# kondratevakate/mri-epilepsy-diagnosis

Measured on AMD Instinct MI355X. Metric: MRI volumes/sec (fwd+bwd) 3D U-Net @160x192x160, higher is better.
Workload: dtype f32; 1 GPU; unet.UNet(c0=8, 3 enc blocks, BN+PReLU, trilinear) fwd+softmax-Dice+bwd+AdamW, batch 2 x 1x160x192x160 fp32 per GPU (BASELINE configs[1]); global_batch=2, parallelism=dp1, launch=eager

## Files before the change

### include/mri3d.h

```cpp
#ifndef MRI3D_H
#define MRI3D_H

#include <stddef.h>
#include <stdint.h>

#ifdef __cplusplus
extern "C" {
#endif

typedef void* mri3d_stream_t;

enum { MRI3D_OK = 0, MRI3D_EINVAL = -1, MRI3D_ENOTSUP = -2, MRI3D_ELAUNCH = -3, MRI3D_EWORKSPACE = -4 };
enum { MRI3D_F32 = 0, MRI3D_BF16 = 1 };
enum { MRI3D_ACT_NONE = 0, MRI3D_ACT_RELU = 1, MRI3D_ACT_LEAKY = 2, MRI3D_ACT_PRELU = 3 };
enum { MRI3D_UP_NEAREST = 0, MRI3D_UP_TRILINEAR = 1 };
enum { MRI3D_PASS_FWD = 0, MRI3D_PASS_DGRAD = 1, MRI3D_PASS_WGRAD = 2 };

int mri3d_version(void);
const char* mri3d_last_error(void);

typedef struct Mri3dConvGeom {
    int32_t n;
    int32_t di, hi, wi, ci;
    int32_t dout, ho, wo, co;
    int32_t kd, kh, kw;
    int32_t sd, sh, sw;
    int32_t pd, ph, pw;
    int32_t dd, dh, dw;
    int32_t x_ld, y_ld;
    int32_t dtype;
} Mri3dConvGeom;

size_t mri3d_conv3d_workspace_bytes(const Mri3dConvGeom* g, int pass);

int mri3d_conv3d_fwd(const Mri3dConvGeom* g, const void* x, const void* w, const void* bias, void* y,
                     void* workspace, size_t ws_bytes, mri3d_stream_t stream);
int32_t mri3d_conv3d_fwd_stats_blocks(const Mri3dConvGeom* g);
int mri3d_conv3d_fwd_stats(const Mri3dConvGeom* g, const void* x, const void* w, const void* bias, void* y,
                           double* stat_partials, void* workspace, size_t ws_bytes, mri3d_stream_t stream);
int mri3d_conv3d_dgrad(const Mri3dConvGeom* g, const void* dy, const void* w, const void* bias, void* dx,
                       void* workspace, size_t ws_bytes, mri3d_stream_t stream);
int mri3d_conv3d_wgrad(const Mri3dConvGeom* g, const void* x, const void* dy, void* dw, void* dbias,
                       void* workspace, size_t ws_bytes, mri3d_stream_t stream);

int mri3d_conv3d_route(const Mri3dConvGeom* g, int32_t pass, int32_t stats, int32_t bias, int32_t split, int32_t second_ld,
                       int32_t align_x, int32_t align_y, char* name, size_t name_bytes);

int32_t mri3d_conv3d_cat_supported(const Mri3dConvGeom* g, int32_t split, int32_t second_ld, int32_t pass);
int32_t mri3d_conv3d_fwd_cat_stats_blocks(const Mri3dConvGeom* g, int32_t split, int32_t second_ld);
int mri3d_conv3d_fwd_cat(const Mri3dConvGeom* g, const void* x, const void* x2, int32_t split, int32_t x2_ld, const void* w,
                         const void* bias, void* y, double* stat_partials, void* workspace, size_t ws_bytes,
                         mri3d_stream_t stream);
int mri3d_conv3d_dgrad_cat(const Mri3dConvGeom* g, const void* dy, const void* w, void* dx, void* dx2, int32_t split,
                           int32_t dx2_ld, void* workspace, size_t ws_bytes, mri3d_stream_t stream);
int mri3d_conv3d_wgrad_cat(const Mri3dConvGeom* g, const void* x, const void* x2, int32_t split, int32_t x2_ld, const void* dy,
                           void* dw, void* dbias, void* workspace, size_t ws_bytes, mri3d_stream_t stream);

int32_t mri3d_conv3d_march_supported(const Mri3dConvGeom* g, int32_t pass);
int32_t mri3d_conv3d_march_stats_blocks(const Mri3dConvGeom* g);
int mri3d_conv3d_fwd_march(const Mri3dConvGeom* g, const void* x, const void* x2, int32_t split, int32_t x2_ld, const void* w,
                           const void* bias, void* y, double* stat_partials, void* workspace, size_t ws_bytes,
                           mri3d_stream_t stream);
int mri3d_conv3d_dgrad_march(const Mri3dConvGeom* g, const void* dy, const void* w, void* dx, void* dx2, int32_t split,
                             int32_t dx2_ld, void* workspace, size_t ws_bytes, mri3d_stream_t stream);

typedef struct Mri3dMarchPlanInfo {
    int32_t chunks, blocks, wgh, wgw, gch, gcw, nseg, seglen, nbuf, grid, whole_chunks, dispatcher;
    int64_t smem_bytes, wp_bytes;
} Mri3dMarchPlanInfo;
int32_t mri3d_conv3d_march_plan_query(const Mri3dConvGeom* g, int32_t pass, int32_t stats, Mri3dMarchPlanInfo* out);

int32_t mri3d_upconv3d_supported(const Mri3dConvGeom* g, int32_t scale);
size_t mri3d_upconv3d_workspace_bytes(const Mri3dConvGeom* g, int32_t scale);
int mri3d_upconv3d_fwd(const Mri3dConvGeom* g, int32_t scale, const void* x, const float* w, const float* bias, void* y,
                       mri3d_stream_t stream);
int mri3d_upconv3d_dgrad(const Mri3dConvGeom* g, int32_t scale, const void* dy, const float* w, void* dx, mri3d_stream_t stream);
int mri3d_upconv3d_wgrad(const Mri3dConvGeom* g, int32_t scale, const void* x, const void* dy, float* dw, float* dbias,
                         void* workspace, size_t ws_bytes, mri3d_stream_t stream);

int32_t mri3d_convpair_supported(const Mri3dConvGeom* first, const Mri3dConvGeom* second);
size_t mri3d_convpair_workspace_bytes(const Mri3dConvGeom* first, const Mri3dConvGeom* second);
int mri3d_convpair_wgrad_first(const Mri3dConvGeom* first, const Mri3dConvGeom* second, const void* x, const void* dy2, const float* w2,
                               float* dw1, float* dbias1, void* workspace, size_t ws_bytes, mri3d_stream_t stream);

typedef struct Mri3dFusedConvPlanInfo {
    int32_t hch, grid, gtrips, trips, per, passes, chunks;
    int64_t slabs, rows;
} Mri3dFusedConvPlanInfo;
int32_t mri3d_upconv3d_plan_query(const Mri3dConvGeom* g, int32_t scale, int32_t pass, Mri3dFusedConvPlanInfo* out);
int32_t mri3d_convpair_plan_query(const Mri3dConvGeom* first, const Mri3dConvGeom* second, Mri3dFusedConvPlanInfo* out);

typedef struct Mri3dNormGeom {
    int32_t n;
    int64_t vox;
    int32_t c;
    int32_t x_ld;
    int32_t y_ld;
    int32_t instance;
    int32_t act;
    int32_t alpha_n;
    float slope;
    float eps;
    int32_t group_c;
    int32_t dtype;
} Mri3dNormGeom;

size_t mri3d_norm_workspace_bytes(const Mri3dNormGeom* g);

enum { MRI3D_NORM_PASS_STATS = 0, MRI3D_NORM_PASS_FWD = 1, MRI3D_NORM_PASS_BWD = 2 };
typedef struct Mri3dNormPlanInfo {
    int32_t vec, CL, VT, cy, nblk, groups;
    int64_t gvox;
} Mri3dNormPlanInfo;
int32_t mri3d_norm_plan_query(const Mri3dNormGeom* g, int32_t pass, int32_t align, Mri3dNormPlanInfo* out);

int mri3d_norm_stats(const Mri3dNormGeom* g, const void* x, float* mean, float* invstd,
                     float* running_mean, float* running_var, float momentum,
                     void* workspace, size_t ws_bytes, mri3d_stream_t stream);
int mri3d_norm_stats_from_partials(const Mri3dNormGeom* g, const double* partials, int32_t nblk, const float* shift,
                                   float* mean, float* invstd, float* running_mean, float* running_var, float momentum,
                                   mri3d_stream_t stream);
int mri3d_norm_act_fwd(const Mri3dNormGeom* g, const void* x, const float* mean, const float* invstd,
                       const float* gamma, const float* beta, const float* alpha, void* y,
                       mri3d_stream_t stream);
int mri3d_norm_act_bwd(const Mri3dNormGeom* g, int training, const void* x, const void* dy,
                       const float* mean, const float* invstd, const float* gamma, const float* beta,
                       const float* alpha, void* dx, float* dgamma, float* dbeta, float* dalpha,
                       void* workspace, size_t ws_bytes, mri3d_stream_t stream);

int32_t mri3d_norm_act_pw_supported(const Mri3dNormGeom* g, int32_t co);
size_t mri3d_norm_act_pw_workspace_bytes(const Mri3dNormGeom* g, int32_t co);
int mri3d_norm_act_pw_fwd(const Mri3dNormGeom* g, int32_t co, const void* x, const float* mean, const float* invstd,
                          const float* gamma, const float* beta, const float* alpha, const float* w, const float* bias,
                          void* out, mri3d_stream_t stream);
int mri3d_norm_act_pw_bwd(const Mri3dNormGeom* g, int32_t co, int training, const void* x, const void* dout,
                          const float* mean, const float* invstd, const float* gamma, const float* beta, const float* alpha,
                          const float* w, void* dx, float* dgamma, float* dbeta, float* dalpha, float* dw, float* dbias,
                          void* workspace, size_t ws_bytes, mri3d_stream_t stream);

typedef struct Mri3dPoolGeom {
    int32_t n, di, hi, wi, dout, ho, wo, c;
    int32_t kd, kh, kw, sd, sh, sw, pd, ph, pw;
    int32_t x_ld, y_ld;
    int32_t dtype;
} Mri3dPoolGeom;
int mri3d_maxpool3d_fwd(const Mri3dPoolGeom* g, const void* x, void* y, uint8_t* idx, mri3d_stream_t stream);
int mri3d_maxpool3d_bwd(const Mri3dPoolGeom* g, const void* dy, const uint8_t* idx, void* dx, mri3d_stream_t stream);
int mri3d_maxpool3d_bwd_add(const Mri3dPoolGeom* g, const void* dy, const uint8_t* idx, const void* addend,
                            int32_t addend_ld, void* dx, mri3d_stream_t stream);
int mri3d_maxpool3d_route(const Mri3dPoolGeom* g, int32_t pass, int32_t addend_ld, int32_t align_tensors, int32_t align_idx,
                          char* name, size_t name_bytes);

int32_t mri3d_norm_act_pool_supported(const Mri3dNormGeom* g, const Mri3dPoolGeom* pg);
size_t mri3d_norm_act_pool_workspace_bytes(const Mri3dNormGeom* g, const Mri3dPoolGeom* pg);
int mri3d_norm_act_pool_fwd(const Mri3dNormGeom* g, const Mri3dPoolGeom* pg, const void* x, const float* mean,
                            const float* invstd, const float* gamma, const float* beta, const float* alpha, void* skip,
                            void* pooled, uint8_t* idx, mri3d_stream_t stream);
int mri3d_norm_act_pool_bwd(const Mri3dNormGeom* g, const Mri3dPoolGeom* pg, int training, const void* x, const void* dskip,
                            const void* dpool, const uint8_t* idx, const float* mean, const float* invstd, const float* gamma,
                            const float* beta, const float* alpha, void* dx, float* dgamma, float* dbeta, float* dalpha,
                            void* workspace, size_t ws_bytes, mri3d_stream_t stream);

typedef struct Mri3dUpGeom {
    int32_t n, di, hi, wi, dout, ho, wo, c;
    int32_t x_ld, y_ld;
    int32_t mode;
    int32_t align_corners;
    float rd, rh, rw;
    int32_t dtype;
} Mri3dUpGeom;
size_t mri3d_upsample3d_workspace_bytes(const Mri3dUpGeom* g);
int mri3d_upsample3d_fwd(const Mri3dUpGeom* g, const void* x, void* y, mri3d_stream_t stream);
int mri3d_upsample3d_bwd(const Mri3dUpGeom* g, const void* dy, void* dx, void* workspace, size_t ws_bytes,
                         mri3d_stream_t stream);
int mri3d_upsample3d_route(const Mri3dUpGeom* g, int32_t pass, int32_t align, char* name, size_t name_bytes);

typedef struct Mri3dResamplePlanInfo {
    int32_t vec, npv, hch, grid, segs, segl, tiles_h, tiles_w, passes, items, tables;
    int64_t lds_bytes;
} Mri3dResamplePlanInfo;
int32_t mri3d_maxpool3d_plan_query(const Mri3dPoolGeom* g, int32_t pass, int32_t addend_ld, int32_t align_tensors,
                                   int32_t align_idx, Mri3dResamplePlanInfo* out);
int32_t mri3d_upsample3d_plan_query(const Mri3dUpGeom* g, int32_t pass, int32_t align, Mri3dResamplePlanInfo* out);

typedef struct Mri3dDiceGeom {
    int32_t n;
    int64_t vox;
    int32_t c, ct;
    int32_t x_ld, t_ld;
    float eps;
    int32_t dtype;
} Mri3dDiceGeom;
size_t mri3d_softmax_dice_workspace_bytes(const Mri3dDiceGeom* g);
int mri3d_softmax_dice_fwd(const Mri3dDiceGeom* g, const void* logits, const void* target, float* loss,
                           float* stats, void* workspace, size_t ws_bytes, mri3d_stream_t stream);
int mri3d_softmax_dice_bwd(const Mri3dDiceGeom* g, const void* logits, const void* target, const float* stats,
                           const float* dloss, void* dlogits, mri3d_stream_t stream);

int mri3d_argmax_u8(const void* logits, uint8_t* out, int64_t nvox, int32_t c, int32_t ld, int32_t dtype,
                    mri3d_stream_t stream);

size_t mri3d_mask_overlap_workspace_bytes(void);
int mri3d_mask_overlap(const uint8_t* pred, const uint8_t* gt, int64_t nvox, int64_t* counts, void* workspace,
                       size_t ws_bytes, mri3d_stream_t stream);

enum { MRI3D_LABEL_U8 = 0, MRI3D_LABEL_I16 = 1, MRI3D_LABEL_I32 = 2, MRI3D_LABEL_F32 = 3 };

int mri3d_label_remap(const void* in, int32_t in_dtype, void* out, int32_t out_dtype, int64_t n, const uint8_t* lut,
                      int32_t lut_len, int32_t above, int32_t other, mri3d_stream_t stream);

typedef struct Mri3dDiceIndexGeom {
    int32_t n;
    int64_t vox;
    int32_t c;
    int32_t x_ld;
    float eps;
    int32_t dtype;
} Mri3dDiceIndexGeom;
size_t mri3d_softmax_dice_index_workspace_bytes(const Mri3dDiceIndexGeom* g);
int mri3d_softmax_dice_index_fwd(const Mri3dDiceIndexGeom* g, const void* logits, const uint8_t* labels, float* loss,
                                 float* stats, void* workspace, size_t ws_bytes, mri3d_stream_t stream);
int mri3d_softmax_dice_index_bwd(const Mri3dDiceIndexGeom* g, const void* logits, const uint8_t* labels,
                                 const float* stats, const float* dloss, void* dlogits, mri3d_stream_t stream);

size_t mri3d_confusion_workspace_bytes(int32_t c);
int mri3d_confusion_counts(const uint8_t* pred, const uint8_t* gt, int64_t nvox, int32_t c, int64_t* counts,
                           void* workspace, size_t ws_bytes, mri3d_stream_t stream);

size_t mri3d_order_stats_workspace_bytes(void);
int mri3d_order_stats_f32(const float* x, int64_t n, const int64_t* ranks, int32_t nranks, float* out, void* workspace,
                          size_t ws_bytes, mri3d_stream_t stream);
int mri3d_piecewise_linear_f32(const float* x, float* y, int64_t n, const double* edges, const double* slope,
                               const double* intercept, int32_t nseg, mri3d_stream_t stream);
size_t mri3d_znorm_workspace_bytes(void);
int mri3d_znorm_mean_mask_f32(const float* x, float* y, int64_t n, double* stats, void* workspace, size_t ws_bytes,
                              mri3d_stream_t stream);
int mri3d_crop_or_pad_f32(const float* x, float* y, int32_t outer, int32_t di, int32_t hi, int32_t wi, int32_t dout,
                          int32_t ho, int32_t wo, float fill, mri3d_stream_t stream);

size_t mri3d_intensity_workspace_bytes(int64_t n, int32_t batch, int32_t m);
int mri3d_kde_plan(int64_t n, int32_t batch, int32_t m, int32_t out[4]);
int mri3d_intensity_moments_f32(const float* x, const uint8_t* mask, int64_t n, int32_t batch, double* moments,
                                void* workspace, size_t ws_bytes, mri3d_stream_t stream);
int mri3d_kde_f32(const float* x, const uint8_t* mask, int64_t n, int32_t batch, const double* moments, const double* positions,
                  int32_t m, int32_t bw_rule, double bw_scalar, double* positions_out, double* density, void* workspace,
                  size_t ws_bytes, mri3d_stream_t stream);

size_t mri3d_surface_distance_workspace_bytes(int32_t d, int32_t h, int32_t w);
int mri3d_surface_distance(const uint8_t* gt, const uint8_t* pred, int32_t d, int32_t h, int32_t w,
                           const double* area_table, double* sums, void* workspace, size_t ws_bytes, mri3d_stream_t stream);
int mri3d_surface_elements(const uint8_t* gt, const uint8_t* pred, int32_t d, int32_t h, int32_t w, int32_t* d2_gt,
                           uint8_t* code_gt, int32_t* d2_pred, uint8_t* code_pred, int64_t capacity, uint64_t* counts,
                           void* workspace, size_t ws_bytes, mri3d_stream_t stream);

int mri3d_extract_patches(const void* volumes, int32_t elem_bytes, int32_t nvol, int32_t d, int32_t h, int32_t w,
                          const int32_t* loc_host, int32_t npatch, int32_t pd, int32_t ph, int32_t pw, void* out,
                          mri3d_stream_t stream);
int mri3d_aggregate_patches_u8(const uint8_t* patches, const int32_t* loc_host, int32_t npatch, int32_t pd, int32_t ph,
                               int32_t pw, int32_t bd, int32_t bh, int32_t bw, uint8_t* out, int32_t nvol, int32_t d,
                               int32_t h, int32_t w, mri3d_stream_t stream);
int mri3d_aggregate_patches_argmax(const void* logits, int32_t c, int32_t ld, int32_t dtype, const int32_t* loc_host,
                                   int32_t npatch, int32_t pd, int32_t ph, int32_t pw, int32_t bd, int32_t bh, int32_t bw,
                                   uint8_t* out, int32_t nvol, int32_t d, int32_t h, int32_t w, mri3d_stream_t stream);

int mri3d_strip_starts_f32(const float* gm, int32_t nx, int32_t ny, int32_t nz, int32_t h, int32_t* starts, mri3d_stream_t stream);
int mri3d_mirror_patches_f32(const float* volume, int32_t nx, int32_t ny, int32_t nz, const int32_t* table, const int32_t* order,
                             int64_t npatch, int32_t h, int32_t w, int32_t channels_last, float* out, mri3d_stream_t stream);
int mri3d_mirror_patch_labels_u8(const uint8_t* mask, int32_t nx, int32_t ny, int32_t nz, const int32_t* table, int64_t npatch,
                                 int32_t h, int32_t w, uint8_t* out, mri3d_stream_t stream);
int mri3d_patch_vote_u8(const uint8_t* map, int32_t strips, int32_t slices, uint8_t* out, mri3d_stream_t stream);
int mri3d_paint_patches_u8(const uint8_t* map, const int32_t* starts, int32_t nx, int32_t ny, int32_t nz, int32_t h, int32_t w,
                           uint8_t* out, mri3d_stream_t stream);

int mri3d_warp3d(const float* image, float* image_out, const void* label, void* label_out, int32_t label_bytes, int32_t s,
                 int32_t d, int32_t h, int32_t w, const float* affine, const float* grid, int32_t gd, int32_t gh, int32_t gw,
                 float pad_value, const float* pad_values, mri3d_stream_t stream);
int mri3d_bias_field_f32(const float* x, float* y, int32_t s, int32_t d, int32_t h, int32_t w, const float* coef_host,
                         int32_t order, mri3d_stream_t stream);
int mri3d_kspace_mix_f32(const float* images,
                         float* out,
                         int32_t s, int32_t n, int32_t d, int32_t h, int32_t w,
                         const float* coef,
                         mri3d_stream_t stream);

int mri3d_copy_channels(const void* src, void* dst, int64_t nvox, int32_t c, int32_t src_ld, int32_t dst_ld,
                        int32_t dtype, mri3d_stream_t stream);
int mri3d_add_channels(const void* a, const void* b, void* dst, int64_t nvox, int32_t c, int32_t a_ld,
                       int32_t b_ld, int32_t dst_ld, int32_t dtype, mri3d_stream_t stream);
int mri3d_convert_channels(const void* src, int32_t src_dtype, void* dst, int32_t dst_dtype, int64_t nvox, int32_t c,
                           int32_t src_ld, int32_t dst_ld, mri3d_stream_t stream);

int mri3d_bayes_weights_fwd(const float* mu, const float* logsigma, int64_t n, int32_t eval, float threshold, float* w_mean,
                            float* w_var, float* log_alpha, mri3d_stream_t stream);
int mri3d_bayes_weights_bwd(const float* mu, const float* logsigma, int64_t n, int32_t eval, float threshold,
                            const float* d_w_mean, const float* d_w_var, const float* d_log_alpha, float* dmu,
                            float* dlogsigma, mri3d_stream_t stream);
int mri3d_bayes_square(const void* x, void* x2, int64_t nvox, int32_t c, int32_t x_ld, int32_t x2_ld, int32_t dtype,
                       mri3d_stream_t stream);
int mri3d_bayes_sample_fwd(const void* mu_out, const void* var_out, const float* eps, void* y, int64_t nvox, int32_t c,
                           int32_t mu_ld, int32_t var_ld, int32_t eps_ld, int32_t y_ld, int32_t dtype, mri3d_stream_t stream);
int mri3d_bayes_sample_bwd(const void* dy, const void* var_out, const float* eps, void* dvar, int64_t nvox, int32_t c,
                           int32_t dy_ld, int32_t var_ld, int32_t eps_ld, int32_t dvar_ld, int32_t dtype,
                           mri3d_stream_t stream);
int mri3d_bayes_dx(const void* dx_mean, const void* dx_var, const void* x, void* dx, int64_t nvox, int32_t c,
                   int32_t dx_mean_ld, int32_t dx_var_ld, int32_t x_ld, int32_t dx_ld, int32_t dtype, mri3d_stream_t stream);

size_t mri3d_mc_state_bytes(int64_t nvox, int32_t c);
int mri3d_mc_accumulate(const void* logits, int64_t nvox, int32_t c, int32_t ld, int32_t dtype, int32_t reps,
                        int64_t rep_stride, int32_t first, void* state, size_t state_bytes, mri3d_stream_t stream);
int mri3d_mc_finalize(const void* state, size_t state_bytes, int64_t nvox, int32_t c, int32_t samples, float* mean_p,
                      float* variance, float* entropy, float* mutual_info, uint8_t* mask, mri3d_stream_t stream);

int mri3d_adam_step(float* p, const float* g, float* m, float* v, int64_t n, float lr, float beta1, float beta2,
                    float eps, float weight_decay, int32_t step, float grad_scale, int32_t decoupled,
                    mri3d_stream_t stream);

#ifdef __cplusplus
}
#endif
#endif
```

### mri_epilepsy_diagnosis_amd/_lib.py

```python
import ctypes
import os
from ctypes import POINTER, Structure, c_char_p, c_double, c_float, c_int32, c_int64, c_size_t, c_uint8, c_void_p

_HERE = os.path.dirname(os.path.abspath(__file__))
LIB_PATH = os.path.join(_HERE, "libmri3d_hip.so")

F32, BF16 = 0, 1
ACT_NONE, ACT_RELU, ACT_LEAKY, ACT_PRELU = 0, 1, 2, 3
UP_NEAREST, UP_TRILINEAR = 0, 1
PASS_FWD, PASS_DGRAD, PASS_WGRAD = 0, 1, 2
NORM_PASS_STATS, NORM_PASS_FWD, NORM_PASS_BWD = 0, 1, 2
LABEL_U8, LABEL_I16, LABEL_I32, LABEL_F32 = 0, 1, 2, 3
BW_SCOTT, BW_SILVERMAN, BW_FACTOR = 0, 1, 2


class ConvGeom(Structure):
    _fields_ = [(n, c_int32) for n in (
        "n", "di", "hi", "wi", "ci", "dout", "ho", "wo", "co", "kd", "kh", "kw", "sd", "sh", "sw",
        "pd", "ph", "pw", "dd", "dh", "dw", "x_ld", "y_ld", "dtype")]


class NormGeom(Structure):
    _fields_ = [("n", c_int32), ("vox", c_int64), ("c", c_int32), ("x_ld", c_int32), ("y_ld", c_int32),
                ("instance", c_int32), ("act", c_int32), ("alpha_n", c_int32), ("slope", c_float),
                ("eps", c_float), ("group_c", c_int32), ("dtype", c_int32)]


class NormPlanInfo(Structure):
    _fields_ = [(n, c_int32) for n in ("vec", "CL", "VT", "cy", "nblk", "groups")] + [("gvox", c_int64)]


class ResamplePlanInfo(Structure):
    _fields_ = [(n, c_int32) for n in ("vec", "npv", "hch", "grid", "segs", "segl", "tiles_h", "tiles_w", "passes", "items",
                                       "tables")] + [("lds_bytes", c_int64)]


class FusedConvPlanInfo(Structure):
    _fields_ = [(n, c_int32) for n in ("hch", "grid", "gtrips", "trips", "per", "passes", "chunks")] + \
               [("slabs", c_int64), ("rows", c_int64)]


class MarchPlanInfo(Structure):
    _fields_ = [(n, c_int32) for n in ("chunks", "blocks", "wgh", "wgw", "gch", "gcw", "nseg", "seglen", "nbuf", "grid",
                                       "whole_chunks", "dispatcher")] + [("smem_bytes", c_int64), ("wp_bytes", c_int64)]


class PoolGeom(Structure):
    _fields_ = [(n, c_int32) for n in (
        "n", "di", "hi", "wi", "dout", "ho", "wo", "c", "kd", "kh", "kw", "sd", "sh", "sw", "pd", "ph", "pw",
        "x_ld", "y_ld", "dtype")]


class UpGeom(Structure):
    _fields_ = [(n, c_int32) for n in ("n", "di", "hi", "wi", "dout", "ho", "wo", "c", "x_ld", "y_ld", "mode",
                                       "align_corners")] + \
               [("rd", c_float), ("rh", c_float), ("rw", c_float), ("dtype", c_int32)]


class DiceGeom(Structure):
    _fields_ = [("n", c_int32), ("vox", c_int64), ("c", c_int32), ("ct", c_int32), ("x_ld", c_int32),
                ("t_ld", c_int32), ("eps", c_float), ("dtype", c_int32)]


class DiceIndexGeom(Structure):
    _fields_ = [("n", c_int32), ("vox", c_int64), ("c", c_int32), ("x_ld", c_int32), ("eps", c_float), ("dtype", c_int32)]


_P = c_void_p
_FP = c_void_p

SIGNATURES = {
    "mri3d_version": (c_int32, []),
    "mri3d_last_error": (c_char_p, []),
    "mri3d_conv3d_workspace_bytes": (c_size_t, [POINTER(ConvGeom), c_int32]),
    "mri3d_conv3d_fwd": (c_int32, [POINTER(ConvGeom), _P, _P, _P, _P, _P, c_size_t, _P]),
    "mri3d_conv3d_fwd_stats_blocks": (c_int32, [POINTER(ConvGeom)]),
    "mri3d_conv3d_fwd_stats": (c_int32, [POINTER(ConvGeom), _P, _P, _P, _P, _P, _P, c_size_t, _P]),
    "mri3d_conv3d_dgrad": (c_int32, [POINTER(ConvGeom), _P, _P, _P, _P, _P, c_size_t, _P]),
    "mri3d_conv3d_wgrad": (c_int32, [POINTER(ConvGeom), _P, _P, _P, _P, _P, c_size_t, _P]),
    "mri3d_conv3d_route": (c_int32, [POINTER(ConvGeom), c_int32, c_int32, c_int32, c_int32, c_int32, c_int32, c_int32, c_char_p, c_size_t]),
    "mri3d_conv3d_cat_supported": (c_int32, [POINTER(ConvGeom), c_int32, c_int32, c_int32]),
    "mri3d_conv3d_fwd_cat_stats_blocks": (c_int32, [POINTER(ConvGeom), c_int32, c_int32]),
    "mri3d_conv3d_fwd_cat": (c_int32, [POINTER(ConvGeom), _P, _P, c_int32, c_int32, _P, _P, _P, _P, _P, c_size_t, _P]),
    "mri3d_conv3d_dgrad_cat": (c_int32, [POINTER(ConvGeom), _P, _P, _P, _P, c_int32, c_int32, _P, c_size_t, _P]),
    "mri3d_conv3d_wgrad_cat": (c_int32, [POINTER(ConvGeom), _P, _P, c_int32, c_int32, _P, _P, _P, _P, c_size_t, _P]),
    "mri3d_conv3d_march_supported": (c_int32, [POINTER(ConvGeom), c_int32]),
    "mri3d_conv3d_march_stats_blocks": (c_int32, [POINTER(ConvGeom)]),
    "mri3d_conv3d_march_plan_query": (c_int32, [POINTER(ConvGeom), c_int32, c_int32, POINTER(MarchPlanInfo)]),
    "mri3d_conv3d_fwd_march": (c_int32, [POINTER(ConvGeom), _P, _P, c_int32, c_int32, _P, _P, _P, _P, _P, c_size_t, _P]),
    "mri3d_conv3d_dgrad_march": (c_int32, [POINTER(ConvGeom), _P, _P, _P, _P, c_int32, c_int32, _P, c_size_t, _P]),
    "mri3d_upconv3d_supported": (c_int32, [POINTER(ConvGeom), c_int32]),
    "mri3d_upconv3d_workspace_bytes": (c_size_t, [POINTER(ConvGeom), c_int32]),
    "mri3d_upconv3d_fwd": (c_int32, [POINTER(ConvGeom), c_int32, _P, _FP, _FP, _P, _P]),
    "mri3d_upconv3d_dgrad": (c_int32, [POINTER(ConvGeom), c_int32, _P, _FP, _P, _P]),
    "mri3d_upconv3d_wgrad": (c_int32, [POINTER(ConvGeom), c_int32, _P, _P, _FP, _FP, _P, c_size_t, _P]),
    "mri3d_convpair_supported": (c_int32, [POINTER(ConvGeom), POINTER(ConvGeom)]),
    "mri3d_convpair_workspace_bytes": (c_size_t, [POINTER(ConvGeom), POINTER(ConvGeom)]),
    "mri3d_convpair_wgrad_first": (c_int32, [POINTER(ConvGeom), POINTER(ConvGeom), _P, _P, _FP, _FP, _FP, _P, c_size_t, _P]),
    "mri3d_upconv3d_plan_query": (c_int32, [POINTER(ConvGeom), c_int32, c_int32, POINTER(FusedConvPlanInfo)]),
    "mri3d_convpair_plan_query": (c_int32, [POINTER(ConvGeom), POINTER(ConvGeom), POINTER(FusedConvPlanInfo)]),
    "mri3d_norm_workspace_bytes": (c_size_t, [POINTER(NormGeom)]),
    "mri3d_norm_plan_query": (c_int32, [POINTER(NormGeom), c_int32, c_int32, POINTER(NormPlanInfo)]),
    "mri3d_norm_stats": (c_int32, [POINTER(NormGeom), _P, _FP, _FP, _FP, _FP, c_float, _P, c_size_t, _P]),
    "mri3d_norm_stats_from_partials": (c_int32, [POINTER(NormGeom), _P, c_int32, _FP, _FP, _FP, _FP, _FP, c_float, _P]),
    "mri3d_norm_act_fwd": (c_int32, [POINTER(NormGeom), _P, _FP, _FP, _FP, _FP, _FP, _P, _P]),
    "mri3d_norm_act_bwd": (c_int32, [POINTER(NormGeom), c_int32, _P, _P, _FP, _FP, _FP, _FP, _FP, _P, _FP, _FP, _FP,
                                     _P, c_size_t, _P]),
    "mri3d_norm_act_pw_supported": (c_int32, [POINTER(NormGeom), c_int32]),
    "mri3d_norm_act_pw_workspace_bytes": (c_size_t, [POINTER(NormGeom), c_int32]),
    "mri3d_norm_act_pw_fwd": (c_int32, [POINTER(NormGeom), c_int32, _P, _FP, _FP, _FP, _FP, _FP, _FP, _FP, _P, _P]),
    "mri3d_norm_act_pw_bwd": (c_int32, [POINTER(NormGeom), c_int32, c_int32, _P, _P, _FP, _FP, _FP, _FP, _FP, _FP, _P, _FP, _FP,
                                        _FP, _FP, _FP, _P, c_size_t, _P]),
    "mri3d_maxpool3d_fwd": (c_int32, [POINTER(PoolGeom), _P, _P, _P, _P]),
    "mri3d_maxpool3d_bwd": (c_int32, [POINTER(PoolGeom), _P, _P, _P, _P]),
    "mri3d_maxpool3d_bwd_add": (c_int32, [POINTER(PoolGeom), _P, _P, _P, c_int32, _P, _P]),
    "mri3d_maxpool3d_route": (c_int32, [POINTER(PoolGeom), c_int32, c_int32, c_int32, c_int32, c_char_p, c_size_t]),
    "mri3d_maxpool3d_plan_query": (c_int32, [POINTER(PoolGeom), c_int32, c_int32, c_int32, c_int32, POINTER(ResamplePlanInfo)]),
    "mri3d_norm_act_pool_supported": (c_int32, [POINTER(NormGeom), POINTER(PoolGeom)]),
    "mri3d_norm_act_pool_workspace_bytes": (c_size_t, [POINTER(NormGeom), POINTER(PoolGeom)]),
    "mri3d_norm_act_pool_fwd": (c_int32, [POINTER(NormGeom), POINTER(PoolGeom), _P, _FP, _FP, _FP, _FP, _FP, _P, _P, _P, _P]),
    "mri3d_norm_act_pool_bwd": (c_int32, [POINTER(NormGeom), POINTER(PoolGeom), c_int32, _P, _P, _P, _P, _FP, _FP, _FP, _FP,
                                          _FP, _P, _FP, _FP, _FP, _P, c_size_t, _P]),
    "mri3d_upsample3d_workspace_bytes":(c_size_t, [POINTER(UpGeom)]),
    "mri3d_upsample3d_fwd": (c_int32, [POINTER(UpGeom), _P, _P, _P]),
    "mri3d_upsample3d_bwd": (c_int32, [POINTER(UpGeom), _P, _P, _P, c_size_t, _P]),
    "mri3d_upsample3d_route": (c_int32, [POINTER(UpGeom), c_int32, c_int32, c_char_p, c_size_t]),
    "mri3d_upsample3d_plan_query": (c_int32, [POINTER(UpGeom), c_int32, c_int32, POINTER(ResamplePlanInfo)]),
    "mri3d_softmax_dice_workspace_bytes": (c_size_t, [POINTER(DiceGeom)]),
    "mri3d_softmax_dice_fwd": (c_int32, [POINTER(DiceGeom), _P, _P, _FP, _FP, _P, c_size_t, _P]),
    "mri3d_softmax_dice_bwd": (c_int32, [POINTER(DiceGeom), _P, _P, _FP, _FP, _P, _P]),
    "mri3d_argmax_u8": (c_int32, [_P, _P, c_int64, c_int32, c_int32, c_int32, _P]),
    "mri3d_mask_overlap_workspace_bytes": (c_size_t, []),
    "mri3d_mask_overlap": (c_int32, [_P, _P, c_int64, _P, _P, c_size_t, _P]),
    "mri3d_label_remap": (c_int32, [_P, c_int32, _P, c_int32, c_int64, _P, c_int32, c_int32, c_int32, _P]),
    "mri3d_softmax_dice_index_workspace_bytes": (c_size_t, [POINTER(DiceIndexGeom)]),
    "mri3d_softmax_dice_index_fwd": (c_int32, [POINTER(DiceIndexGeom), _P, _P, _FP, _FP, _P, c_size_t, _P]),
    "mri3d_softmax_dice_index_bwd": (c_int32, [POINTER(DiceIndexGeom), _P, _P, _FP, _FP, _P, _P]),
    "mri3d_confusion_workspace_bytes": (c_size_t, [c_int32]),
    "mri3d_confusion_counts": (c_int32, [_P, _P, c_int64, c_int32, _P, _P, c_size_t, _P]),
    "mri3d_order_stats_workspace_bytes": (c_size_t, []),
    "mri3d_order_stats_f32": (c_int32, [_P, c_int64, _P, c_int32, _P, _P, c_size_t, _P]),
    "mri3d_piecewise_linear_f32": (c_int32, [_P, _P, c_int64, _P, _P, _P, c_int32, _P]),
    "mri3d_znorm_workspace_bytes": (c_size_t, []),
    "mri3d_znorm_mean_mask_f32": (c_int32, [_P, _P, c_int64, _P, _P, c_size_t, _P]),
    "mri3d_crop_or_pad_f32": (c_int32, [_P, _P, c_int32, c_int32, c_int32, c_int32, c_int32, c_int32, c_int32, c_float, _P]),
    "mri3d_intensity_workspace_bytes": (c_size_t, [c_int64, c_int32, c_int32]),
    "mri3d_kde_plan": (c_int32, [c_int64, c_int32, c_int32, _P]),
    "mri3d_intensity_moments_f32": (c_int32, [_P, _P, c_int64, c_int32, _P, _P, c_size_t, _P]),
    "mri3d_kde_f32": (c_int32, [_P, _P, c_int64, c_int32, _P, _P, c_int32, c_int32, c_double, _P, _P, _P, c_size_t, _P]),
    "mri3d_surface_distance_workspace_bytes": (c_size_t, [c_int32, c_int32, c_int32]),
    "mri3d_surface_distance": (c_int32, [_P, _P, c_int32, c_int32, c_int32, _P, _P, _P, c_size_t, _P]),
    "mri3d_surface_elements": (c_int32, [_P, _P, c_int32, c_int32, c_int32, _P, _P, _P, _P, c_int64, _P, _P, c_size_t, _P]),
    "mri3d_extract_patches": (c_int32, [_P, c_int32, c_int32, c_int32, c_int32, c_int32, _P, c_int32, c_int32, c_int32,
                                        c_int32, _P, _P]),
    "mri3d_aggregate_patches_u8": (c_int32, [_P, _P, c_int32, c_int32, c_int32, c_int32, c_int32, c_int32, c_int32, _P,
                                             c_int32, c_int32, c_int32, c_int32, _P]),
    "mri3d_aggregate_patches_argmax": (c_int32, [_P, c_int32, c_int32, c_int32, _P, c_int32, c_int32, c_int32, c_int32,
                                                 c_int32, c_int32, c_int32, _P, c_int32, c_int32, c_int32, c_int32, _P]),
    "mri3d_strip_starts_f32": (c_int32, [_FP, c_int32, c_int32, c_int32, c_int32, _P, _P]),
    "mri3d_mirror_patches_f32": (c_int32, [_FP, c_int32, c_int32, c_int32, _P, _P, c_int64, c_int32, c_int32, c_int32, _FP, _P]),
    "mri3d_mirror_patch_labels_u8": (c_int32, [_P, c_int32, c_int32, c_int32, _P, c_int64, c_int32, c_int32, _P, _P]),
    "mri3d_patch_vote_u8": (c_int32, [_P, c_int32, c_int32, _P, _P]),
    "mri3d_paint_patches_u8": (c_int32, [_P, _P, c_int32, c_int32, c_int32, c_int32, c_int32, _P, _P]),
    "mri3d_warp3d": (c_int32, [_FP, _FP, _P, _P, c_int32, c_int32, c_int32, c_int32, c_int32, _FP, _FP, c_int32, c_int32,
                               c_int32, c_float, _FP, _P]),
    "mri3d_bias_field_f32": (c_int32, [_FP, _FP, c_int32, c_int32, c_int32, c_int32, _P, c_int32, _P]),
    "mri3d_kspace_mix_f32": (c_int32, [_FP, _FP, c_int32, c_int32, c_int32, c_int32, c_int32, _FP, _P]),
    "mri3d_copy_channels": (c_int32, [_P, _P, c_int64, c_int32, c_int32, c_int32, c_int32, _P]),
    "mri3d_add_channels": (c_int32, [_P, _P, _P, c_int64, c_int32, c_int32, c_int32, c_int32, c_int32, _P]),
    "mri3d_convert_channels": (c_int32, [_P, c_int32, _P, c_int32, c_int64, c_int32, c_int32, c_int32, _P]),
    "mri3d_bayes_weights_fwd": (c_int32, [_FP, _FP, c_int64, c_int32, c_float, _FP, _FP, _FP, _P]),
    "mri3d_bayes_weights_bwd": (c_int32, [_FP, _FP, c_int64, c_int32, c_float, _FP, _FP, _FP, _FP, _FP, _P]),
    "mri3d_bayes_square": (c_int32, [_P, _P, c_int64, c_int32, c_int32, c_int32, c_int32, _P]),
    "mri3d_bayes_sample_fwd": (c_int32, [_P, _P, _FP, _P, c_int64, c_int32, c_int32, c_int32, c_int32, c_int32, c_int32, _P]),
    "mri3d_bayes_sample_bwd": (c_int32, [_P, _P, _FP, _P, c_int64, c_int32, c_int32, c_int32, c_int32, c_int32, c_int32, _P]),
    "mri3d_bayes_dx": (c_int32, [_P, _P, _P, _P, c_int64, c_int32, c_int32, c_int32, c_int32, c_int32, c_int32, _P]),
    "mri3d_mc_state_bytes": (c_size_t, [c_int64, c_int32]),
    "mri3d_mc_accumulate": (c_int32, [_P, c_int64, c_int32, c_int32, c_int32, c_int32, c_int64, c_int32, _P, c_size_t, _P]),
    "mri3d_mc_finalize": (c_int32, [_P, c_size_t, c_int64, c_int32, c_int32, _FP, _FP, _FP, _FP, _P, _P]),
    "mri3d_adam_step": (c_int32, [_FP, _FP, _FP, _FP, c_int64, c_float, c_float, c_float, c_float, c_float, c_int32,
                                  c_float, c_int32, _P]),
}

_lib = None


class Mri3dError(RuntimeError):
    pass


def lib():
    global _lib
    if _lib is None:
        import torch
        if not os.path.exists(LIB_PATH):
            raise Mri3dError(
                "libmri3d_hip.so not found at %s — run `python -m mri_epilepsy_diagnosis_amd.build` "
                "(or __graft_entry__.build()).  There is no PyTorch fallback for device tensors." % LIB_PATH)
        h = ctypes.CDLL(LIB_PATH)
        for name, (res, args) in SIGNATURES.items():
            fn = getattr(h, name)
            fn.restype = res
            fn.argtypes = args
        _lib = h
    return _lib


def check(rc, what=""):
    if rc != 0:
        msg = lib().mri3d_last_error()
        raise Mri3dError("%s failed (rc=%d): %s" % (what, rc, msg.decode() if msg else "?"))
```

### mri_epilepsy_diagnosis_amd/csrc/api.hip

```cpp
#include "common.h"
#include "conv_backends.h"
#include <string.h>

namespace mri3d {

static thread_local char g_err[512] = "";

void set_error(const char* fmt, ...) {
    va_list ap;
    va_start(ap, fmt);
    vsnprintf(g_err, sizeof(g_err), fmt, ap);
    va_end(ap);
}

static int conv_check(const Mri3dConvGeom* g, const char* who, int first_ci = -1) {
    MRI3D_REQUIRE(g != nullptr, MRI3D_EINVAL, "%s: null geometry", who);
    MRI3D_REQUIRE(g->dtype == MRI3D_F32 || g->dtype == MRI3D_BF16, MRI3D_ENOTSUP, "%s: unknown dtype %d", who, g->dtype);
    MRI3D_REQUIRE(g->n > 0 && g->di > 0 && g->hi > 0 && g->wi > 0 && g->ci > 0 && g->dout > 0 && g->ho > 0 && g->wo > 0 &&
                      g->co > 0,
                  MRI3D_EINVAL, "%s: empty tensor", who);
    MRI3D_REQUIRE(g->kd > 0 && g->kh > 0 && g->kw > 0 && g->sd > 0 && g->sh > 0 && g->sw > 0 && g->dd > 0 && g->dh > 0 &&
                      g->dw > 0 && g->pd >= 0 && g->ph >= 0 && g->pw >= 0,
                  MRI3D_EINVAL, "%s: bad kernel/stride/padding/dilation", who);
    MRI3D_REQUIRE(g->x_ld >= (first_ci >= 0 ? first_ci : g->ci) && g->y_ld >= g->co, MRI3D_EINVAL, "%s: pitch smaller than channel count", who);
    int ed = (g->di + 2 * g->pd - g->dd * (g->kd - 1) - 1) / g->sd + 1;
    int eh = (g->hi + 2 * g->ph - g->dh * (g->kh - 1) - 1) / g->sh + 1;
    int ew = (g->wi + 2 * g->pw - g->dw * (g->kw - 1) - 1) / g->sw + 1;
    MRI3D_REQUIRE(ed == g->dout && eh == g->ho && ew == g->wo, MRI3D_EINVAL,
                  "%s: output dims (%d,%d,%d) do not match conv arithmetic (%d,%d,%d)", who, g->dout, g->ho, g->wo, ed, eh,
                  ew);
    return MRI3D_OK;
}

enum class ConvBackend { none, generic, pointwise, mfma };

static ConvBackend conv_backend(const Mri3dConvGeom& g, int pass, bool stats, int split, int second_ld, int align_mfma, int align_pw) {
    const bool mfma_aligned = align_mfma >= 16;
    const bool pw_aligned = align_pw >= (g.dtype == MRI3D_BF16 ? 8 : 16);
    if (split > 0) {
        if (!(conv_mfma_cat_supported(g, split, second_ld, pass) && mfma_aligned)) return ConvBackend::none;
        return (stats && conv_mfma_fwd_stat_blocks(g, split, second_ld) <= 0) ? ConvBackend::none : ConvBackend::mfma;
    }
    if (stats)
        return (pass == MRI3D_PASS_FWD && conv_mfma_supported(g, MRI3D_PASS_FWD) && conv_mfma_fwd_stat_blocks(g) > 0 && mfma_aligned)
                   ? ConvBackend::mfma : ConvBackend::none;
    if (pass == MRI3D_PASS_FWD) {
        if (conv_mfma_supported(g, pass) && mfma_aligned) return ConvBackend::mfma;
        if (conv_pointwise_supported(g, pass) && pw_aligned) return ConvBackend::pointwise;
        return ConvBackend::generic;
    }
    if (conv_pointwise_supported(g, pass) && pw_aligned) return ConvBackend::pointwise;
    if (conv_mfma_supported(g, pass) && mfma_aligned) return ConvBackend::mfma;
    return ConvBackend::generic;
}

}

using namespace mri3d;

extern "C" int mri3d_version(void) { return 100; }
extern "C" const char* mri3d_last_error(void) { return g_err; }

extern "C" size_t mri3d_conv3d_workspace_bytes(const Mri3dConvGeom* g, int pass) {
    if (!g) return 0;
    size_t a = conv_generic_workspace_bytes(*g, pass);
    size_t b = conv_mfma_supported(*g, pass) ? conv_mfma_workspace_bytes(*g, pass) : 0;
    size_t c = conv_pointwise_supported(*g, pass) ? conv_pointwise_workspace_bytes(*g, pass) : 0;
    a = a > b ? a : b;
    return align_up(a > c ? a : c, 256);
}

extern "C" int mri3d_conv3d_fwd(const Mri3dConvGeom* g, const void* x, const void* w, const void* bias, void* y,
                                void* workspace, size_t ws_bytes, mri3d_stream_t stream) {
    int rc = conv_check(g, "conv3d_fwd");
    if (rc) return rc;
    MRI3D_REQUIRE(x && w && y, MRI3D_EINVAL, "conv3d_fwd: null pointer");
    hipStream_t s = static_cast<hipStream_t>(stream);
    switch (conv_backend(*g, MRI3D_PASS_FWD, false, 0, 0, ptr_align(x, y, workspace), ptr_align(x))) {
    case ConvBackend::mfma: return conv_mfma_fwd(*g, x, (const float*)w, (const float*)bias, y, workspace, ws_bytes, s);
    case ConvBackend::pointwise: return conv_pointwise_fwd(*g, x, (const float*)w, (const float*)bias, y, s);
    default: return conv_generic_fwd(*g, x, (const float*)w, (const float*)bias, y, workspace, ws_bytes, s);
    }
}

extern "C" int32_t mri3d_conv3d_fwd_stats_blocks(const Mri3dConvGeom* g) {
    if (!g || conv_check(g, "conv3d_fwd_stats_blocks") != MRI3D_OK) return 0;
    return conv_mfma_supported(*g, MRI3D_PASS_FWD) ? conv_mfma_fwd_stat_blocks(*g) : 0;
}

extern "C" int mri3d_conv3d_fwd_stats(const Mri3dConvGeom* g, const void* x, const void* w, const void* bias, void* y,
                                      double* stat_partials, void* workspace, size_t ws_bytes, mri3d_stream_t stream) {
    int rc = conv_check(g, "conv3d_fwd_stats");
    if (rc) return rc;
    MRI3D_REQUIRE(x && w && y && stat_partials, MRI3D_EINVAL, "conv3d_fwd_stats: null pointer");
    MRI3D_REQUIRE(conv_backend(*g, MRI3D_PASS_FWD, true, 0, 0, ptr_align(x, y, workspace), ptr_align(x)) == ConvBackend::mfma,
                  MRI3D_ENOTSUP, "conv3d_fwd_stats: geometry not served by the MFMA forward kernel (query mri3d_conv3d_fwd_stats_blocks)");
    return conv_mfma_fwd_stats(*g, x, (const float*)w, (const float*)bias, y, stat_partials, workspace, ws_bytes,
                               static_cast<hipStream_t>(stream));
}

extern "C" int mri3d_conv3d_dgrad(const Mri3dConvGeom* g, const void* dy, const void* w, const void* bias, void* dx,
                                  void* workspace, size_t ws_bytes, mri3d_stream_t stream) {
    int rc = conv_check(g, "conv3d_dgrad");
    if (rc) return rc;
    MRI3D_REQUIRE(dy && w && dx, MRI3D_EINVAL, "conv3d_dgrad: null pointer");
    hipStream_t s = static_cast<hipStream_t>(stream);
    switch (conv_backend(*g, MRI3D_PASS_DGRAD, false, 0, 0, ptr_align(dy, dx, workspace), ptr_align(dx))) {
    case ConvBackend::pointwise: return conv_pointwise_dgrad(*g, dy, (const float*)w, (const float*)bias, dx, s);
    case ConvBackend::mfma: return conv_mfma_dgrad(*g, dy, (const float*)w, (const float*)bias, dx, workspace, ws_bytes, s);
    default: return conv_generic_dgrad(*g, dy, (const float*)w, (const float*)bias, dx, workspace, ws_bytes, s);
    }
}

extern "C" int32_t mri3d_conv3d_cat_supported(const Mri3dConvGeom* g, int32_t split, int32_t second_ld, int32_t pass) {
    if (!g || split <= 0 || conv_check(g, "conv3d_cat_supported", split) != MRI3D_OK) return 0;
    return conv_mfma_cat_supported(*g, split, second_ld, pass) ? 1 : 0;
}

extern "C" int32_t mri3d_conv3d_fwd_cat_stats_blocks(const Mri3dConvGeom* g, int32_t split, int32_t second_ld) {
    if (!g || split <= 0 || conv_check(g, "conv3d_fwd_cat_stats_blocks", split) != MRI3D_OK) return 0;
    return conv_mfma_cat_supported(*g, split, second_ld, MRI3D_PASS_FWD) ? conv_mfma_fwd_stat_blocks(*g, split, second_ld) : 0;
}

extern "C" int mri3d_conv3d_fwd_cat(const Mri3dConvGeom* g, const void* x, const void* x2, int32_t split, int32_t x2_ld,
                                    const void* w, const void* bias, void* y, double* stat_partials, void* workspace,
                                    size_t ws_bytes, mri3d_stream_t stream) {
    int rc = conv_check(g, "conv3d_fwd_cat", split);
    if (rc) return rc;
    MRI3D_REQUIRE(x && x2 && w && y, MRI3D_EINVAL, "conv3d_fwd_cat: null pointer");
    MRI3D_REQUIRE(conv_backend(*g, MRI3D_PASS_FWD, false, split, x2_ld, ptr_align(x, y, workspace, x2), 0) == ConvBackend::mfma,
                  MRI3D_ENOTSUP, "conv3d_fwd_cat: geometry / alignment not served (query mri3d_conv3d_cat_supported)");
    MRI3D_REQUIRE(stat_partials == nullptr || conv_mfma_fwd_stat_blocks(*g, split, x2_ld) > 0, MRI3D_ENOTSUP,
                  "conv3d_fwd_cat: no fused statistics for this geometry (query mri3d_conv3d_fwd_cat_stats_blocks)");
    return conv_mfma_fwd_cat(*g, x, x2, split, x2_ld, (const float*)w, (const float*)bias, y, stat_partials, workspace, ws_bytes,
                             static_cast<hipStream_t>(stream));
}

extern "C" int mri3d_conv3d_dgrad_cat(const Mri3dConvGeom* g, const void* dy, const void* w, void* dx, void* dx2, int32_t split,
                                      int32_t dx2_ld, void* workspace, size_t ws_bytes, mri3d_stream_t stream) {
    int rc = conv_check(g, "conv3d_dgrad_cat", split);
    if (rc) return rc;
    MRI3D_REQUIRE(dy && w && dx && dx2, MRI3D_EINVAL, "conv3d_dgrad_cat: null pointer");
    MRI3D_REQUIRE(conv_backend(*g, MRI3D_PASS_DGRAD, false, split, dx2_ld, ptr_align(dy, dx, workspace, dx2), 0) == ConvBackend::mfma,
                  MRI3D_ENOTSUP, "conv3d_dgrad_cat: geometry / alignment not served (query mri3d_conv3d_cat_supported)");
    return conv_mfma_dgrad_cat(*g, dy, (const float*)w, dx, dx2, split, dx2_ld, workspace, ws_bytes, static_cast<hipStream_t>(stream));
}

extern "C" int mri3d_conv3d_wgrad_cat(const Mri3dConvGeom* g, const void* x, const void* x2, int32_t split, int32_t x2_ld,
                                      const void* dy, void* dw, void* dbias, void* workspace, size_t ws_bytes,
                                      mri3d_stream_t stream) {
    int rc = conv_check(g, "conv3d_wgrad_cat", split);
    if (rc) return rc;
    MRI3D_REQUIRE(x && x2 && dy && dw, MRI3D_EINVAL, "conv3d_wgrad_cat: null pointer");
    MRI3D_REQUIRE(conv_backend(*g, MRI3D_PASS_WGRAD, false, split, x2_ld, ptr_align(x, dy, workspace, x2), 0) == ConvBackend::mfma,
                  MRI3D_ENOTSUP, "conv3d_wgrad_cat: geometry / alignment not served (query mri3d_conv3d_cat_supported)");
    return conv_mfma_wgrad_cat(*g, x, x2, split, x2_ld, dy, (float*)dw, (float*)dbias, workspace, ws_bytes,
                               static_cast<hipStream_t>(stream));
}

extern "C" int32_t mri3d_conv3d_march_supported(const Mri3dConvGeom* g, int32_t pass) {
    if (!g || (pass != MRI3D_PASS_FWD && pass != MRI3D_PASS_DGRAD) || conv_check(g, "conv3d_march_supported") != MRI3D_OK) return 0;
    return conv_march_needs(*g, pass == MRI3D_PASS_DGRAD, false, true).grid > 0 ? 1 : 0;
}

extern "C" int32_t mri3d_conv3d_march_stats_blocks(const Mri3dConvGeom* g) {
    if (!g || conv_check(g, "conv3d_march_stats_blocks") != MRI3D_OK) return 0;
    return conv_march_needs(*g, false, true, true).grid;
}

extern "C" int32_t mri3d_conv3d_march_plan_query(const Mri3dConvGeom* g, int32_t pass, int32_t stats, Mri3dMarchPlanInfo* out) {
    MRI3D_REQUIRE(g && out, MRI3D_EINVAL, "conv3d_march_plan_query: null pointer");
    int rc = conv_check(g, "conv3d_march_plan_query");
    if (rc) return rc;
    MRI3D_REQUIRE(pass == MRI3D_PASS_FWD || pass == MRI3D_PASS_DGRAD, MRI3D_EINVAL, "conv3d_march_plan_query: pass %d", pass);
    MRI3D_REQUIRE(!stats || pass == MRI3D_PASS_FWD, MRI3D_EINVAL, "conv3d_march_plan_query: statistics outside the forward");
    Mri3dMarchPlanInfo info;
    MRI3D_REQUIRE(conv_march_plan_info(*g, pass == MRI3D_PASS_DGRAD, stats != 0, info), MRI3D_ENOTSUP,
                  "conv3d_march_plan_query: geometry not served (see mri3d_conv3d_march_supported; statistics: at most 8 output blocks)");
    *out = info;
    return MRI3D_OK;
}

extern "C" int mri3d_conv3d_fwd_march(const Mri3dConvGeom* g, const void* x, const void* x2, int32_t split, int32_t x2_ld,
                                      const void* w, const void* bias, void* y, double* stat_partials, void* workspace,
                                      size_t ws_bytes, mri3d_stream_t stream) {
    int rc = conv_check(g, "conv3d_fwd_march", x2 ? split : -1);
    if (rc) return rc;
    MRI3D_REQUIRE(x && w && y, MRI3D_EINVAL, "conv3d_fwd_march: null pointer");
    MRI3D_REQUIRE(x2 == nullptr || (split > 0 && split < g->ci && x2_ld >= g->ci - split), MRI3D_EINVAL, "conv3d_fwd_march: bad split");
    return conv_march_run(*g, false, true, x, (const float*)w, (const float*)bias, y, workspace, ws_bytes,
                          static_cast<hipStream_t>(stream), stat_partials, ConvSplit{x2, split, x2_ld});
}

extern "C" int mri3d_conv3d_dgrad_march(const Mri3dConvGeom* g, const void* dy, const void* w, void* dx, void* dx2, int32_t split,
                                        int32_t dx2_ld, void* workspace, size_t ws_bytes, mri3d_stream_t stream) {
    int rc = conv_check(g, "conv3d_dgrad_march", dx2 ? split : -1);
    if (rc) return rc;
    MRI3D_REQUIRE(dy && w && dx, MRI3D_EINVAL, "conv3d_dgrad_march: null pointer");
    MRI3D_REQUIRE(dx2 == nullptr || (split > 0 && split < g->ci && dx2_ld >= g->ci - split), MRI3D_EINVAL, "conv3d_dgrad_march: bad split");
    return conv_march_run(*g, true, true, dy, (const float*)w, nullptr, dx, workspace, ws_bytes, static_cast<hipStream_t>(stream),
                          nullptr, ConvSplit{dx2, split, dx2_ld});
}

extern "C" int mri3d_conv3d_wgrad(const Mri3dConvGeom* g, const void* x, const void* dy, void* dw, void* dbias,
                                  void* workspace, size_t ws_bytes, mri3d_stream_t stream) {
    int rc = conv_check(g, "conv3d_wgrad");
    if (rc) return rc;
    MRI3D_REQUIRE(x && dy && dw, MRI3D_EINVAL, "conv3d_wgrad: null pointer");
    hipStream_t s = static_cast<hipStream_t>(stream);
    switch (conv_backend(*g, MRI3D_PASS_WGRAD, false, 0, 0, ptr_align(x, dy, workspace), ptr_align(x))) {
    case ConvBackend::pointwise: return conv_pointwise_wgrad(*g, x, dy, (float*)dw, (float*)dbias, workspace, ws_bytes, s);
    case ConvBackend::mfma: return conv_mfma_wgrad(*g, x, dy, (float*)dw, (float*)dbias, workspace, ws_bytes, s);
    default: return conv_generic_wgrad(*g, x, dy, (float*)dw, (float*)dbias, workspace, ws_bytes, s);
    }
}

extern "C" int mri3d_conv3d_route(const Mri3dConvGeom* g, int32_t pass, int32_t stats, int32_t bias, int32_t split, int32_t second_ld,
                                  int32_t align_x, int32_t align_y, char* name, size_t name_bytes) {
    int rc = conv_check(g, "conv3d_route", split > 0 ? split : -1);
    if (rc) return rc;
    MRI3D_REQUIRE(name != nullptr && name_bytes >= 32, MRI3D_EINVAL, "conv3d_route: name buffer of at least 32 bytes required");
    MRI3D_REQUIRE(pass == MRI3D_PASS_FWD || pass == MRI3D_PASS_DGRAD || pass == MRI3D_PASS_WGRAD, MRI3D_EINVAL, "conv3d_route: unknown pass %d", pass);
    MRI3D_REQUIRE(split >= 0 && (!stats || pass == MRI3D_PASS_FWD), MRI3D_EINVAL, "conv3d_route: negative split, or statistics outside the forward");
    const ConvSplit sp{nullptr, split, second_ld};
    const bool with_bias = bias != 0 && pass != MRI3D_PASS_WGRAD && !(split > 0 && pass == MRI3D_PASS_DGRAD);
    switch (conv_backend(*g, pass, stats != 0, split, second_ld, align_x < align_y ? align_x : align_y, align_x)) {
    case ConvBackend::none: snprintf(name, name_bytes, "none"); break;
    case ConvBackend::generic:
        MRI3D_REQUIRE(conv_generic_route_name(*g, pass, with_bias, align_x, align_y, name, name_bytes), MRI3D_EINVAL,
                      "conv3d_route: name buffer too small");
        break;
    case ConvBackend::pointwise:
        MRI3D_REQUIRE(conv_pointwise_route_name(*g, pass, with_bias, align_x, align_y, name, name_bytes), MRI3D_EINVAL,
                      "conv3d_route: name buffer too small");
        break;
    case ConvBackend::mfma:
        MRI3D_REQUIRE(conv_mfma_route_name(*g, pass, stats != 0, with_bias, sp, name, name_bytes), MRI3D_ENOTSUP,
                      "conv3d_route: the MFMA file names no kernel for a pass it supports");
        break;
    }
    return MRI3D_OK;
}
```

### mri_epilepsy_diagnosis_amd/csrc/conv_backends.h

```cpp
#pragma once
#include "common.h"

namespace mri3d {

struct ConvSplit {
    const void* second = nullptr;
    int split = 0, second_ld = 0;
};

size_t conv_generic_workspace_bytes(const Mri3dConvGeom& g, int pass);
int conv_generic_fwd(const Mri3dConvGeom& g, const void* x, const float* w, const float* bias, void* y, void* ws,
                     size_t ws_bytes, hipStream_t s);
int conv_generic_dgrad(const Mri3dConvGeom& g, const void* dy, const float* w, const float* bias, void* dx, void* ws,
                       size_t ws_bytes, hipStream_t s);
int conv_generic_wgrad(const Mri3dConvGeom& g, const void* x, const void* dy, float* dw, float* dbias, void* ws,
                       size_t ws_bytes, hipStream_t s);
bool conv_generic_route_name(const Mri3dConvGeom& g, int pass, bool bias, int ax, int ay, char* name, size_t name_bytes);

bool conv_mfma_supported(const Mri3dConvGeom& g, int pass);
size_t conv_mfma_workspace_bytes(const Mri3dConvGeom& g, int pass);
int conv_mfma_fwd(const Mri3dConvGeom& g, const void* x, const float* w, const float* bias, void* y, void* ws,
                  size_t ws_bytes, hipStream_t s);
int conv_mfma_dgrad(const Mri3dConvGeom& g, const void* dy, const float* w, const float* bias, void* dx, void* ws,
                    size_t ws_bytes, hipStream_t s);
int conv_mfma_fwd_stat_blocks(const Mri3dConvGeom& g, int split = 0, int second_ld = 0);
bool conv_mfma_cat_supported(const Mri3dConvGeom& g, int split, int second_ld, int pass);
int conv_mfma_fwd_cat(const Mri3dConvGeom& g, const void* x, const void* x2, int split, int x2_ld, const float* w, const float* bias,
                      void* y, double* stat_part, void* ws, size_t ws_bytes, hipStream_t s);
int conv_mfma_dgrad_cat(const Mri3dConvGeom& g, const void* dy, const float* w, void* dx, void* dx2, int split, int dx2_ld, void* ws,
                        size_t ws_bytes, hipStream_t s);
int conv_mfma_fwd_stats(const Mri3dConvGeom& g, const void* x, const float* w, const float* bias, void* y, double* stat_part,
                        void* ws, size_t ws_bytes, hipStream_t s);
bool conv_mfma_route_name(const Mri3dConvGeom& g, int pass, bool stats, bool bias, const ConvSplit& sp, char* name, size_t name_bytes);

bool conv_mfma_wgrad_supported(const Mri3dConvGeom& g, int split = 0, int second_ld = 0);
size_t conv_mfma_wgrad_workspace_bytes(const Mri3dConvGeom& g);
bool conv_mfma_wgrad_route_name(const Mri3dConvGeom& g, char* name, size_t name_bytes);
int conv_mfma_wgrad(const Mri3dConvGeom& g, const void* x, const void* dy, float* dw, float* dbias, void* ws,
                    size_t ws_bytes, hipStream_t s);
int conv_mfma_wgrad_cat(const Mri3dConvGeom& g, const void* x, const void* x2, int split, int x2_ld, const void* dy, float* dw,
                        float* dbias, void* ws, size_t ws_bytes, hipStream_t s);

struct MarchNeeds { int grid; size_t wp_bytes; };
MarchNeeds conv_march_needs(const Mri3dConvGeom& g, bool dgrad, bool stats, bool force);
bool conv_march_plan_info(const Mri3dConvGeom& g, bool dgrad, bool stats, Mri3dMarchPlanInfo& out);
int conv_march_run(const Mri3dConvGeom& g, bool dgrad, bool force, const void* in_v, const float* w, const float* bias, void* out_v,
                   void* ws, size_t ws_bytes, hipStream_t s, double* stat_part, const ConvSplit& sp);

bool conv_pointwise_supported(const Mri3dConvGeom& g, int pass);
size_t conv_pointwise_workspace_bytes(const Mri3dConvGeom& g, int pass);
int conv_pointwise_fwd(const Mri3dConvGeom& g, const void* x, const float* w, const float* bias, void* y, hipStream_t s);
int conv_pointwise_dgrad(const Mri3dConvGeom& g, const void* dy, const float* w, const float* bias, void* dx,
                         hipStream_t s);
int conv_pointwise_wgrad(const Mri3dConvGeom& g, const void* x, const void* dy, float* dw, float* dbias, void* ws,
                         size_t ws_bytes, hipStream_t s);
bool conv_pointwise_route_name(const Mri3dConvGeom& g, int pass, bool bias, int ax, int ay, char* name, size_t name_bytes);

}
```

### mri_epilepsy_diagnosis_amd/csrc/conv_generic.hip

```cpp
#include "common.h"
#include "conv_backends.h"

namespace mri3d {

__device__ __forceinline__ float wave_sum_dpp(float v) {
    v += __builtin_bit_cast(float, __builtin_amdgcn_update_dpp(0, __builtin_bit_cast(int, v), 0xB1, 0xF, 0xF, true));
    v += __builtin_bit_cast(float, __builtin_amdgcn_update_dpp(0, __builtin_bit_cast(int, v), 0x4E, 0xF, 0xF, true));
    v += __builtin_bit_cast(float, __builtin_amdgcn_update_dpp(0, __builtin_bit_cast(int, v), 0x141, 0xF, 0xF, true));
    v += __builtin_bit_cast(float, __builtin_amdgcn_update_dpp(0, __builtin_bit_cast(int, v), 0x140, 0xF, 0xF, true));
    const int vi = __builtin_bit_cast(int, v);
    const float r0 = __builtin_bit_cast(float, __builtin_amdgcn_readlane(vi, 0));
    const float r1 = __builtin_bit_cast(float, __builtin_amdgcn_readlane(vi, 16));
    const float r2 = __builtin_bit_cast(float, __builtin_amdgcn_readlane(vi, 32));
    const float r3 = __builtin_bit_cast(float, __builtin_amdgcn_readlane(vi, 48));
    return (r0 + r1) + (r2 + r3);
}

__global__ void repack_w_kernel(const float* __restrict__ w, float* __restrict__ wp, int Co, int Ci, int taps, int P, int dgrad) {
    const int M = dgrad ? Co : Ci, N = dgrad ? Ci : Co;
    int total = taps * M * P;
    for (int i = blockIdx.x * blockDim.x + threadIdx.x; i < total; i += gridDim.x * blockDim.x) {
        int p = i % P;
        int m = (i / P) % M;
        int tap = i / (P * M);
// ... 754 lines not shown
        };
        for (unsigned e = vl; e < inner; e += VL) {
            float4 gv;
            float xv[NTAPS][CIV];
            unsigned okm;
            fetch(e, gv, xv, okm);
            consume(gv, xv, okm);
        }
    }
    for (int t = 0; t < taps; ++t) {
        __syncthreads();
#pragma unroll
        for (int a = 0; a < CIV; ++a)
#pragma unroll
            for (int b = 0; b < 4; ++b) {
                float val = 0.f;
#pragma unroll
                for (int tt = 0; tt < NTAPS; ++tt)
                    if (tt == t) val = acc[tt][a][b];
                red[tid * 16 + a * 4 + b] = val;
            }
        __syncthreads();
        for (int o = tid; o < PV * (CIV * 4); o += 256) {
            const int ab = o % (CIV * 4), q = o / (CIV * 4);
            double sdbl = 0.0;
            for (int l = 0; l < VL; ++l) sdbl += (double)red[(l * PV + q) * 16 + ab];
            const int ci = (q % QI) * CIV + ab / 4, co = (q / QI) * 4 + ab % 4;
            if (ci < g.ci && co < g.co) part[(((size_t)blockIdx.x * taps + t) * CiP + ci) * CoP + co] = (float)sdbl;
        }
    }
    if (bias_part != nullptr) {
        __syncthreads();
#pragma unroll
        for (int b = 0; b < 4; ++b) red[tid * 4 + b] = (iq == 0) ? bsum[b] : 0.f;
        __syncthreads();
        if (tid < g.co) {
            double sdbl = 0.0;
            for (int l = 0; l < VL; ++l) sdbl += (double)red[((l * PV) + (tid / 4) * QI) * 4 + (tid % 4)];
            bias_part[(size_t)blockIdx.x * g.co + tid] = (float)sdbl;
        }
    }
}

template <typename T, int CI>
__global__ void __launch_bounds__(256)
conv_wgrad_co1_kernel(Mri3dConvGeom g, const T* __restrict__ x, const T* __restrict__ dy, float* __restrict__ part,
                      float* __restrict__ bias_part) {
    __shared__ float red[4][kSmTaps * CI + 1];
    const int taps = g.kd * g.kh * g.kw;
    const int tid = threadIdx.x;
    float acc[kSmTaps][CI], bsum = 0.f;
#pragma unroll
    for (int t = 0; t < kSmTaps; ++t)
#pragma unroll
        for (int c = 0; c < CI; ++c) acc[t][c] = 0.f;
    const int64_t per_n = (int64_t)g.dout * g.ho * g.wo;
    const int64_t nvox = (int64_t)g.n * per_n;
    for (int64_t v = (int64_t)blockIdx.x * 256 + tid; v < nvox; v += (int64_t)gridDim.x * 256) {
        const int n = (int)(v / per_n);
        unsigned r = (unsigned)(v - (int64_t)n * per_n);
        const int ow = r % g.wo;
        r /= g.wo;
        const int oh = r % g.ho, od = r / g.ho;
        const float gv = ldf(dy + v * g.y_ld);
        bsum += gv;
        const T* xn = x + (int64_t)n * g.di * g.hi * g.wi * g.x_ld;
#pragma unroll
        for (int t = 0; t < kSmTaps; ++t) {
            if (t < taps) {
                const int kw = t % g.kw, kh = (t / g.kw) % g.kh, kd = t / (g.kw * g.kh);
                const int id = od * g.sd - g.pd + kd * g.dd, ih = oh * g.sh - g.ph + kh * g.dh, iw = ow * g.sw - g.pw + kw * g.dw;
                const bool ok = (unsigned)id < (unsigned)g.di && (unsigned)ih < (unsigned)g.hi && (unsigned)iw < (unsigned)g.wi;
                const T* xp = xn + (((int64_t)min(max(id, 0), g.di - 1) * g.hi + min(max(ih, 0), g.hi - 1)) * g.wi +
                                    min(max(iw, 0), g.wi - 1)) * g.x_ld;
                const float gm = ok ? gv : 0.f;
                if constexpr (CI == 1) {
                    acc[t][0] = fmaf(ldf(xp), gm, acc[t][0]);
                } else {
#pragma unroll
                    for (int c = 0; c < CI; c += 4) {
                        const float4 q = ldf4(xp + c);
                        acc[t][c] = fmaf(q.x, gm, acc[t][c]);
                        acc[t][c + 1] = fmaf(q.y, gm, acc[t][c + 1]);
                        acc[t][c + 2] = fmaf(q.z, gm, acc[t][c + 2]);
                        acc[t][c + 3] = fmaf(q.w, gm, acc[t][c + 3]);
                    }
                }
            }
        }
    }
    const int lane = tid & 63, wave = tid >> 6;
#pragma unroll
    for (int t = 0; t < kSmTaps; ++t)
#pragma unroll
        for (int c = 0; c < CI; ++c) {
            const float vsum = wave_sum_dpp(acc[t][c]);
            if (lane == 0) red[wave][t * CI + c] = vsum;
        }
    {
        const float vsum = wave_sum_dpp(bsum);
        if (lane == 0) red[wave][kSmTaps * CI] = vsum;
    }
    __syncthreads();
    if (tid < taps * CI)
        part[(size_t)blockIdx.x * taps * CI + tid] = (red[0][tid] + red[1][tid]) + (red[2][tid] + red[3][tid]);
    else if (tid == kSmTaps * CI && bias_part)
        bias_part[blockIdx.x] = (red[0][tid] + red[1][tid]) + (red[2][tid] + red[3][tid]);
}

constexpr int kCo1Blocks = 1024;

static bool wgrad_co1_ok(const Mri3dConvGeom& g) {
    static const int off = tuning_knob("MRI3D_CO1_OFF", 0);
    return !off && g.co == 1 && g.kd * g.kh * g.kw <= kSmTaps && (g.ci == 1 || ((g.ci == 4 || g.ci == 8 || g.ci == 16) && g.x_ld % 4 == 0)) &&
           (int64_t)g.dout * g.ho * g.wo < 0x7fffffffLL;
}

constexpr int C1D = 4, C1H = 8, C1WQ = 8;

template <int CO> struct Cin1 { static constexpr int VPT = CO <= 8 ? 4 : 2; };
typedef float f32x2 __attribute__((ext_vector_type(2)));

__device__ __forceinline__ void decode_tile(int t, int tilesD, int tilesH, int tilesW, int TW, int& n, int& d0, int& h0, int& w0) {
    w0 = (t % tilesW) * TW;
    t /= tilesW;
    h0 = (t % tilesH) * C1H;
    t /= tilesH;
    d0 = (t % tilesD) * C1D;
    n = t / tilesD;
}

template <typename T, int TW, int ND, int NTHR = 256>
__device__ __forceinline__ void cin1_stage(float* xs, const T* __restrict__ xn, const Mri3dConvGeom& g, int dlo, int h0,
                                           int w0, int tid) {
    constexpr int PW = TW + 4, NE = ND * (C1H + 2) * (TW + 2);
    for (int e = tid; e < NE; e += NTHR) {
        const int fw = e % (TW + 2), r = e / (TW + 2);
        const int fh = r % (C1H + 2), fd = r / (C1H + 2);
        const int id = dlo + fd, ih = h0 - 1 + fh, iw = w0 - 1 + fw;
        const bool ok = (unsigned)id < (unsigned)g.di && (unsigned)ih < (unsigned)g.hi && (unsigned)iw < (unsigned)g.wi;
        const int cd = min(max(id, 0), g.di - 1), ch = min(max(ih, 0), g.hi - 1), cw = min(max(iw, 0), g.wi - 1);
        const float v = ldf(xn + (((int64_t)cd * g.hi + ch) * g.wi + cw) * g.x_ld);
        xs[(fd * (C1H + 2) + fh) * PW + fw] = ok ? v : 0.f;
    }
}

template <typename T, int CO>
__global__ void __launch_bounds__(256)
conv_cin1_fwd_kernel(Mri3dConvGeom g, const T* __restrict__ x, const float* __restrict__ wp, const float* __restrict__ bias,
                     T* __restrict__ y, int tilesD, int tilesH, int tilesW, int ntiles) {
    constexpr int VPT = Cin1<CO>::VPT, TW = C1WQ * VPT, PW = TW + 4;
    __shared__ __attribute__((aligned(16))) float xs[(C1D + 2) * (C1H + 2) * PW];
    __shared__ __attribute__((aligned(16))) float wsh[27 * CO];
    const int tid = threadIdx.x;
    for (int e = tid; e < 27 * CO; e += 256) wsh[e] = wp[e];
    const int wq = tid % C1WQ, hl = (tid / C1WQ) % C1H, dl = tid / (C1WQ * C1H);
    float bv[CO];
#pragma unroll
    for (int c = 0; c < CO; ++c) bv[c] = bias ? bias[c] : 0.f;
    for (int tile = blockIdx.x; tile < ntiles; tile += gridDim.x) {
        int n, d0, h0, w0;
        decode_tile(tile, tilesD, tilesH, tilesW, TW, n, d0, h0, w0);
        __syncthreads();
        cin1_stage<T, TW, C1D + 2>(xs, x + (int64_t)n * g.di * g.hi * g.wi * g.x_ld, g, d0 - 1, h0, w0, tid);
        __syncthreads();
        f32x2 acc[VPT][CO / 2];
#pragma unroll
        for (int v = 0; v < VPT; ++v)
#pragma unroll
            for (int c = 0; c < CO / 2; ++c) acc[v][c] = f32x2{bv[2 * c], bv[2 * c + 1]};
#pragma unroll
        for (int kd = 0; kd < 3; ++kd)
#pragma unroll
            for (int kh = 0; kh < 3; ++kh) {
                const float* row = xs + ((dl + kd) * (C1H + 2) + hl + kh) * PW + wq * VPT;
                float r[VPT + 2];
#pragma unroll
                for (int i = 0; i < VPT + 2; ++i) r[i] = row[i];
                int woff = (kd * 3 + kh) * 3 * CO;
                asm volatile("" : "+v"(woff));
                __builtin_amdgcn_sched_barrier(0);
                const float* wrow = wsh + woff;
#pragma unroll
                for (int kw = 0; kw < 3; ++kw) {
                    const float* wt = wrow + kw * CO;
#pragma unroll
                    for (int c = 0; c < CO / 2; ++c) {
                        const f32x2 wv = f32x2{wt[2 * c], wt[2 * c + 1]};
#pragma unroll
                        for (int v = 0; v < VPT; ++v)
                            acc[v][c] = __builtin_elementwise_fma(f32x2{r[v + kw], r[v + kw]}, wv, acc[v][c]);
                    }
                }
            }
#pragma unroll
        for (int v = 0; v < VPT; ++v)
#pragma unroll
            for (int c = 0; c < CO / 2; ++c) asm volatile("" : "+v"(acc[v][c]));
        const int od = d0 + dl, oh = h0 + hl;
        if (od < g.dout && oh < g.ho) {
            T* yo = y + ((((int64_t)n * g.dout + od) * g.ho + oh) * g.wo + w0 + wq * VPT) * g.y_ld;
#pragma unroll
            for (int v = 0; v < VPT; ++v)
                if (w0 + wq * VPT + v < g.wo) {
#pragma unroll
                    for (int c = 0; c < CO; c += 4)
                        stf4(yo + (int64_t)v * g.y_ld + c,
                             make_float4(acc[v][c / 2].x, acc[v][c / 2].y, acc[v][c / 2 + 1].x, acc[v][c / 2 + 1].y));
                }
        }
    }
}

template <typename T, int CO>
__global__ void __launch_bounds__(768)
conv_cin1_wgrad_kernel(Mri3dConvGeom g, const T* __restrict__ x, const T* __restrict__ dy, float* __restrict__ part,
                       float* __restrict__ bias_part, int tilesD, int tilesH, int tilesW, int ntiles, int nshares) {
    constexpr int VPT = Cin1<CO>::VPT, TW = C1WQ * VPT, PW = TW + 4, NA = 9 * CO + CO;
    __shared__ __attribute__((aligned(16))) float xs[(C1D + 2) * (C1H + 2) * PW];
    __shared__ float red[12][NA];
    const int kd = __builtin_amdgcn_readfirstlane((int)threadIdx.x >> 8);
    const int tid = threadIdx.x & 255;
    const int per_xcd = gridDim.x / 8;
    const int share = (blockIdx.x % 8) * per_xcd + blockIdx.x / 8;
    const int wq = tid % C1WQ, hl = (tid / C1WQ) % C1H, dl = tid / (C1WQ * C1H);
    f32x2 acc[3][3][CO / 2];
    float bsum[CO];
#pragma unroll
    for (int a = 0; a < 3; ++a)
#pragma unroll
        for (int b = 0; b < 3; ++b)
#pragma unroll
            for (int c = 0; c < CO / 2; ++c) acc[a][b][c] = f32x2{0.f, 0.f};
#pragma unroll
    for (int c = 0; c < CO; ++c) bsum[c] = 0.f;
    for (int tile = share; tile < ntiles; tile += nshares) {
        int n, d0, h0, w0;
        decode_tile(tile, tilesD, tilesH, tilesW, TW, n, d0, h0, w0);
        __syncthreads();
        cin1_stage<T, TW, C1D + 2, 768>(xs, x + (int64_t)n * g.di * g.hi * g.wi * g.x_ld, g, d0 - 1, h0, w0, (int)threadIdx.x);
        const int od = d0 + dl, oh = h0 + hl;
        f32x2 gy[VPT][CO / 2];
#pragma unroll
        for (int v = 0; v < VPT; ++v) {
            const int ow = w0 + wq * VPT + v;
            const bool ok = od < g.dout && oh < g.ho && ow < g.wo;
            const T* dp = dy + ((((int64_t)n * g.dout + min(od, g.dout - 1)) * g.ho + min(oh, g.ho - 1)) * g.wo +
                                min(ow, g.wo - 1)) * g.y_ld;
#pragma unroll
            for (int c = 0; c < CO; c += 4) {
                const float4 q = ldf4(dp + c);
                gy[v][c / 2] = f32x2{ok ? q.x : 0.f, ok ? q.y : 0.f};
                gy[v][c / 2 + 1] = f32x2{ok ? q.z : 0.f, ok ? q.w : 0.f};
            }
        }
        __syncthreads();
#pragma unroll
        for (int kh = 0; kh < 3; ++kh) {
            const float* row = xs + ((dl + kd) * (C1H + 2) + hl + kh) * PW + wq * VPT;
            float r[VPT + 2];
#pragma unroll
            for (int i = 0; i < VPT + 2; ++i) r[i] = row[i];
#pragma unroll
            for (int kw = 0; kw < 3; ++kw)
#pragma unroll
                for (int v = 0; v < VPT; ++v)
#pragma unroll
                    for (int c = 0; c < CO / 2; ++c)
                        acc[kh][kw][c] = __builtin_elementwise_fma(f32x2{r[v + kw], r[v + kw]}, gy[v][c], acc[kh][kw][c]);
        }
        if (kd == 1) {
#pragma unroll
            for (int v = 0; v < VPT; ++v)
#pragma unroll
                for (int c = 0; c < CO / 2; ++c) { bsum[2 * c] += gy[v][c].x; bsum[2 * c + 1] += gy[v][c].y; }
        }
    }
    const int lane = tid & 63, wave = (int)threadIdx.x >> 6;
#pragma unroll
    for (int a = 0; a < 3; ++a)
#pragma unroll
        for (int b = 0; b < 3; ++b)
#pragma unroll
            for (int c = 0; c < CO; ++c) {
                const float vsum = wave_sum_dpp((c & 1) ? acc[a][b][c / 2].y : acc[a][b][c / 2].x);
                if (lane == 0) red[wave][(a * 3 + b) * CO + c] = vsum;
            }
#pragma unroll
    for (int c = 0; c < CO; ++c) {
        const float vsum = wave_sum_dpp(bsum[c]);
        if (lane == 0) red[wave][9 * CO + c] = vsum;
    }
    __syncthreads();
    const int w0_ = 4 * kd;
    if (tid < 9 * CO) {
        const float t4 = (red[w0_][tid] + red[w0_ + 1][tid]) + (red[w0_ + 2][tid] + red[w0_ + 3][tid]);
        part[((size_t)share * 27 + kd * 9 + tid / CO) * CO + tid % CO] = t4;
    } else if (tid < NA && kd == 1 && bias_part) {
        const int c = tid - 9 * CO;
        bias_part[(size_t)share * CO + c] = (red[w0_][tid] + red[w0_ + 1][tid]) + (red[w0_ + 2][tid] + red[w0_ + 3][tid]);
    }
}

template <typename T>
__global__ void __launch_bounds__(256)
conv_c1c1_stencil_kernel(Mri3dConvGeom g, const T* __restrict__ x, int x_ld, const float* __restrict__ w, const float* __restrict__ bias,
                         int flip, T* __restrict__ y, int y_ld, int tilesD, int tilesH, int tilesW, int ntiles) {
    constexpr int VPT = 4, TW = C1WQ * VPT, PW = TW + 4;
    __shared__ __attribute__((aligned(16))) float xs[(C1D + 2) * (C1H + 2) * PW];
    const int tid = threadIdx.x;
    const int wq = tid % C1WQ, hl = (tid / C1WQ) % C1H, dl = tid / (C1WQ * C1H);
    float wt[27];
#pragma unroll
    for (int t = 0; t < 27; ++t) wt[t] = w[flip ? 26 - t : t];
    const float b0 = bias ? bias[0] : 0.f;
    Mri3dConvGeom gs = g;
    gs.x_ld = x_ld;
    for (int tile = blockIdx.x; tile < ntiles; tile += gridDim.x) {
        int n, d0, h0, w0;
        decode_tile(tile, tilesD, tilesH, tilesW, TW, n, d0, h0, w0);
        __syncthreads();
        cin1_stage<T, TW, C1D + 2>(xs, x + (int64_t)n * g.di * g.hi * g.wi * x_ld, gs, d0 - 1, h0, w0, tid);
        __syncthreads();
        float acc[VPT];
#pragma unroll
        for (int v = 0; v < VPT; ++v) acc[v] = b0;
#pragma unroll
        for (int kd = 0; kd < 3; ++kd)
#pragma unroll
            for (int kh = 0; kh < 3; ++kh) {
                const float* row = xs + ((dl + kd) * (C1H + 2) + hl + kh) * PW + wq * VPT;
                float r[VPT + 2];
#pragma unroll
                for (int i = 0; i < VPT + 2; ++i) r[i] = row[i];
#pragma unroll
                for (int kw = 0; kw < 3; ++kw)
#pragma unroll
                    for (int v = 0; v < VPT; ++v) acc[v] = fmaf(r[v + kw], wt[(kd * 3 + kh) * 3 + kw], acc[v]);
            }
#pragma unroll
        for (int v = 0; v < VPT; ++v) asm volatile("" : "+v"(acc[v]));
        const int od = d0 + dl, oh = h0 + hl;
        if (od < g.di && oh < g.hi) {
            T* yo = y + ((((int64_t)n * g.di + od) * g.hi + oh) * g.wi + w0 + wq * VPT) * y_ld;
#pragma unroll
            for (int v = 0; v < VPT; ++v)
                if (w0 + wq * VPT + v < g.wi) stf(yo + (int64_t)v * y_ld, acc[v]);
        }
    }
}

template <typename T>
__global__ void __launch_bounds__(256)
conv_c1c1_wgrad_kernel(Mri3dConvGeom g, const T* __restrict__ x, const T* __restrict__ dy, float* __restrict__ part,
                       float* __restrict__ bias_part, int tilesD, int tilesH, int tilesW, int ntiles) {
    constexpr int VPT = 4, TW = C1WQ * VPT, PW = TW + 4;
    __shared__ __attribute__((aligned(16))) float xs[(C1D + 2) * (C1H + 2) * PW];
    __shared__ float red[4][28];
    const int tid = threadIdx.x;
    const int wq = tid % C1WQ, hl = (tid / C1WQ) % C1H, dl = tid / (C1WQ * C1H);
    float acc[27], bsum = 0.f;
#pragma unroll
    for (int t = 0; t < 27; ++t) acc[t] = 0.f;
    for (int tile = blockIdx.x; tile < ntiles; tile += gridDim.x) {
        int n, d0, h0, w0;
        decode_tile(tile, tilesD, tilesH, tilesW, TW, n, d0, h0, w0);
        __syncthreads();
        cin1_stage<T, TW, C1D + 2>(xs, x + (int64_t)n * g.di * g.hi * g.wi * g.x_ld, g, d0 - 1, h0, w0, tid);
        const int od = d0 + dl, oh = h0 + hl;
        float gy[VPT];
#pragma unroll
        for (int v = 0; v < VPT; ++v) {
            const int ow = w0 + wq * VPT + v;
            const bool ok = od < g.dout && oh < g.ho && ow < g.wo;
            const float q = ldf(dy + ((((int64_t)n * g.dout + min(od, g.dout - 1)) * g.ho + min(oh, g.ho - 1)) * g.wo +
                                      min(ow, g.wo - 1)) * g.y_ld);
            gy[v] = ok ? q : 0.f;
            bsum += gy[v];
        }
        __syncthreads();
#pragma unroll
        for (int kd = 0; kd < 3; ++kd)
#pragma unroll
            for (int kh = 0; kh < 3; ++kh) {
                const float* row = xs + ((dl + kd) * (C1H + 2) + hl + kh) * PW + wq * VPT;
                float r[VPT + 2];
#pragma unroll
                for (int i = 0; i < VPT + 2; ++i) r[i] = row[i];
#pragma unroll
                for (int kw = 0; kw < 3; ++kw)
#pragma unroll
                    for (int v = 0; v < VPT; ++v) acc[(kd * 3 + kh) * 3 + kw] = fmaf(r[v + kw], gy[v], acc[(kd * 3 + kh) * 3 + kw]);
            }
    }
    const int lane = tid & 63, wave = tid >> 6;
#pragma unroll
    for (int t = 0; t < 27; ++t) {
        const float vsum = wave_sum_dpp(acc[t]);
        if (lane == 0) red[wave][t] = vsum;
    }
    {
        const float vsum = wave_sum_dpp(bsum);
        if (lane == 0) red[wave][27] = vsum;
    }
    __syncthreads();
    if (tid < 27) part[(size_t)blockIdx.x * 27 + tid] = (red[0][tid] + red[1][tid]) + (red[2][tid] + red[3][tid]);
    else if (tid == 27 && bias_part) bias_part[blockIdx.x] = (red[0][27] + red[1][27]) + (red[2][27] + red[3][27]);
}

constexpr int kC1C1Blocks = 1024;

constexpr int kC1TBlocks = 1024;

template <int NT>
__global__ void __launch_bounds__(256)
conv_c1_taps_kernel(Mri3dConvGeom g, const float* __restrict__ src, const float* __restrict__ w, const float* __restrict__ bias,
                    float* __restrict__ dst, int sign, int sD, int sH, int sW, int oD, int oH, int oW) {
    const int taps = g.kd * g.kh * g.kw;
    const unsigned W4 = (unsigned)oW >> 2;
    const unsigned nitems = (unsigned)g.n * oD * oH * W4;
    const float b0 = bias != nullptr ? bias[0] : 0.f;
    for (unsigned item = blockIdx.x * blockDim.x + threadIdx.x; item < nitems; item += gridDim.x * blockDim.x) {
        const unsigned q = item % W4;
        unsigned r = item / W4;
        const int oh = (int)(r % (unsigned)oH);
        r /= (unsigned)oH;
        const int od = (int)(r % (unsigned)oD), n = (int)(r / (unsigned)oD);
        const int ow = 4 * (int)q;
        const float* sn = src + (int64_t)n * sD * sH * sW;
        float4 xv[NT];
        unsigned vm[NT];
#pragma unroll
        for (int t = 0; t < NT; ++t) {
            const int tt = t < taps ? t : 0;
            const int kw = tt % g.kw, kh = (tt / g.kw) % g.kh, kd = tt / (g.kw * g.kh);
            const int sd_ = od + sign * (kd * g.dd - g.pd), sh_ = oh + sign * (kh * g.dh - g.ph), sw_ = ow + sign * (kw * g.dw - g.pw);
            const bool rowok = t < taps && (unsigned)sd_ < (unsigned)sD && (unsigned)sh_ < (unsigned)sH;
            unsigned m = 0;
#pragma unroll
            for (int j = 0; j < 4; ++j) m |= (rowok && (unsigned)(sw_ + j) < (unsigned)sW) ? (1u << j) : 0u;
            vm[t] = m;
            const float* p = sn + ((int64_t)(rowok ? sd_ : 0) * sH + (rowok ? sh_ : 0)) * sW;
            if (m == 15u) {
                xv[t] = *reinterpret_cast<const float4*>(p + sw_);
            } else {
                xv[t].x = (m & 1u) ? p[sw_] : 0.f;
                xv[t].y = (m & 2u) ? p[sw_ + 1] : 0.f;
                xv[t].z = (m & 4u) ? p[sw_ + 2] : 0.f;
                xv[t].w = (m & 8u) ? p[sw_ + 3] : 0.f;
            }
        }
        float4 acc = make_float4(b0, b0, b0, b0);
#pragma unroll
        for (int t = 0; t < NT; ++t) {
            if (t < taps) {
                const float wt = w[t];
                acc.x = fmaf(xv[t].x, wt, acc.x);
                acc.y = fmaf(xv[t].y, wt, acc.y);
                acc.z = fmaf(xv[t].z, wt, acc.z);
                acc.w = fmaf(xv[t].w, wt, acc.w);
            }
        }
        *reinterpret_cast<float4*>(dst + (((int64_t)n * oD + od) * oH + oh) * oW + ow) = acc;
    }
}

template <int NT>
__global__ void __launch_bounds__(256)
conv_c1_taps_wgrad_kernel(Mri3dConvGeom g, const float* __restrict__ x, const float* __restrict__ dy, float* __restrict__ part,
                          float* __restrict__ bias_part) {
    __shared__ double red[4][NT + 1];
    const int taps = g.kd * g.kh * g.kw;
    const unsigned W4 = (unsigned)g.wo >> 2;
    const unsigned nitems = (unsigned)g.n * g.dout * g.ho * W4;
    float acc[NT + 1];
#pragma unroll
    for (int t = 0; t <= NT; ++t) acc[t] = 0.f;
    for (unsigned item = blockIdx.x * blockDim.x + threadIdx.x; item < nitems; item += gridDim.x * blockDim.x) {
        const unsigned q = item % W4;
        unsigned r = item / W4;
        const int oh = (int)(r % (unsigned)g.ho);
        r /= (unsigned)g.ho;
        const int od = (int)(r % (unsigned)g.dout), n = (int)(r / (unsigned)g.dout);
        const int ow = 4 * (int)q;
        const float4 gv = *reinterpret_cast<const float4*>(dy + (((int64_t)n * g.dout + od) * g.ho + oh) * g.wo + ow);
        acc[NT] += (gv.x + gv.y) + (gv.z + gv.w);
        const float* xn = x + (int64_t)n * g.di * g.hi * g.wi;
#pragma unroll
        for (int t = 0; t < NT; ++t) {
            const int tt = t < taps ? t : 0;
            const int kw = tt % g.kw, kh = (tt / g.kw) % g.kh, kd = tt / (g.kw * g.kh);
            const int id = od - g.pd + kd * g.dd, ih = oh - g.ph + kh * g.dh, iw = ow - g.pw + kw * g.dw;
            const bool rowok = t < taps && (unsigned)id < (unsigned)g.di && (unsigned)ih < (unsigned)g.hi;
            const float* p = xn + ((int64_t)(rowok ? id : 0) * g.hi + (rowok ? ih : 0)) * g.wi;
            float4 xv;
            if (rowok && iw >= 0 && iw + 3 < g.wi) {
                xv = *reinterpret_cast<const float4*>(p + iw);
            } else {
                xv.x = (rowok && (unsigned)iw < (unsigned)g.wi) ? p[iw] : 0.f;
                xv.y = (rowok && (unsigned)(iw + 1) < (unsigned)g.wi) ? p[iw + 1] : 0.f;
                xv.z = (rowok && (unsigned)(iw + 2) < (unsigned)g.wi) ? p[iw + 2] : 0.f;
                xv.w = (rowok && (unsigned)(iw + 3) < (unsigned)g.wi) ? p[iw + 3] : 0.f;
            }
            acc[t] = fmaf(xv.x, gv.x, fmaf(xv.y, gv.y, fmaf(xv.z, gv.z, fmaf(xv.w, gv.w, acc[t]))));
        }
    }
    const int lane = threadIdx.x & 63, wv = threadIdx.x >> 6;
#pragma unroll
    for (int t = 0; t <= NT; ++t) {
        float v = acc[t];
#pragma unroll
        for (int o = 32; o >= 1; o >>= 1) v += __shfl_xor(v, o, 64);
        if (lane == 0) red[wv][t] = (double)v;
    }
    __syncthreads();
    if (threadIdx.x <= NT) {
        const double sdbl = (red[0][threadIdx.x] + red[1][threadIdx.x]) + (red[2][threadIdx.x] + red[3][threadIdx.x]);
        if ((int)threadIdx.x < taps) part[(size_t)blockIdx.x * taps + threadIdx.x] = (float)sdbl;
        if (threadIdx.x == NT && bias_part != nullptr) bias_part[blockIdx.x] = (float)sdbl;
    }
}

static bool c1_taps_ok(const Mri3dConvGeom& g) {
    return g.dtype == MRI3D_F32 && g.ci == 1 && g.co == 1 && g.kd * g.kh * g.kw <= kSmTaps && g.sd == 1 && g.sh == 1 && g.sw == 1 &&
           g.x_ld == 1 && g.y_ld == 1 && g.wo % 4 == 0 && g.wi % 4 == 0 && !(g.kd == 3 && g.kh == 3 && g.kw == 3) &&
           (int64_t)g.n * g.dout * g.ho * g.wo < 0x7fffffffLL && (int64_t)g.n * g.di * g.hi * g.wi < 0x7fffffffLL;
}

static void launch_c1_taps(const Mri3dConvGeom& g, int nt, const float* src, const float* w, const float* bias, float* dst, int sign,
                           hipStream_t s) {
    const int sD = sign > 0 ? g.di : g.dout, sH = sign > 0 ? g.hi : g.ho, sW = sign > 0 ? g.wi : g.wo;
    const int oD = sign > 0 ? g.dout : g.di, oH = sign > 0 ? g.ho : g.hi, oW = sign > 0 ? g.wo : g.wi;
    const int64_t items = (int64_t)g.n * oD * oH * (oW / 4);
    const int grid = (int)std::max<int64_t>(1, std::min<int64_t>(cdiv64(items, 256), 8192));
    if (nt == 3)
        hipLaunchKernelGGL(conv_c1_taps_kernel<3>, dim3(grid), dim3(256), 0, s, g, src, w, bias, dst, sign, sD, sH, sW, oD, oH, oW);
    else
        hipLaunchKernelGGL(conv_c1_taps_kernel<kSmTaps>, dim3(grid), dim3(256), 0, s, g, src, w, bias, dst, sign, sD, sH, sW, oD, oH, oW);
}

struct C1Tiles { int tilesD, tilesH, tilesW; int64_t ntiles; };
static C1Tiles c1_tiles(int n, int D, int H, int W, int vpt) {
    C1Tiles t;
    t.tilesD = cdiv(D, C1D), t.tilesH = cdiv(H, C1H), t.tilesW = cdiv(W, C1WQ * vpt);
    t.ntiles = (int64_t)n * t.tilesD * t.tilesH * t.tilesW;
    return t;
}

static bool c1c1_ok(const Mri3dConvGeom& g) {
    static const int off = tuning_knob("MRI3D_C1C1_OFF", 0);
    return !off && g.ci == 1 && g.co == 1 && g.kd == 3 && g.kh == 3 && g.kw == 3 && g.sd == 1 && g.sh == 1 && g.sw == 1 &&
           g.dd == 1 && g.dh == 1 && g.dw == 1 && g.pd == 1 && g.ph == 1 && g.pw == 1 &&
           c1_tiles(g.n, g.dout, g.ho, g.wo, 4).ntiles < 0x7fffffffLL;
}

template <typename T>
static void launch_c1c1_stencil(const Mri3dConvGeom& g, const T* src, int src_ld, const float* w, const float* bias, int flip,
                                T* dst, int dst_ld, hipStream_t s) {
    const C1Tiles t = c1_tiles(g.n, g.di, g.hi, g.wi, 4);
    hipLaunchKernelGGL(conv_c1c1_stencil_kernel<T>, dim3(std::min((int)t.ntiles, 256 * 8)), dim3(256), 0, s, g, src, src_ld, w, bias, flip,
                       dst, dst_ld, t.tilesD, t.tilesH, t.tilesW, (int)t.ntiles);
}

static const int g_cin1_off = tuning_knob("MRI3D_CIN1_OFF", 0);
constexpr int kCin1Shares = 256;

static bool cin1_ok(const Mri3dConvGeom& g) {
    return !g_cin1_off && g.ci == 1 && (g.co == 8 || g.co == 16) && g.kd == 3 && g.kh == 3 && g.kw == 3 && g.sd == 1 &&
           g.sh == 1 && g.sw == 1 && g.dd == 1 && g.dh == 1 && g.dw == 1 && g.pd == 1 && g.ph == 1 && g.pw == 1 &&
           g.y_ld % 4 == 0 && c1_tiles(g.n, g.dout, g.ho, g.wo, 2).ntiles < 0x7fffffffLL;
}
static C1Tiles cin1_tiles(const Mri3dConvGeom& g) { return c1_tiles(g.n, g.dout, g.ho, g.wo, g.co <= 8 ? 4 : 2); }

static bool wgrad_small_ok(const Mri3dConvGeom& g) {
    const int taps = g.kd * g.kh * g.kw;
    return taps <= kSmTaps && g.ci <= 64 && g.co <= 64 && (int64_t)g.dout * g.ho * g.wo < 0x7fffffffLL;
}

static bool wgrad_quads_ok(const Mri3dConvGeom& g) {
    const int taps = g.kd * g.kh * g.kw;
    const int pv = (g.ci / 4) * (g.co / 4);
    if (g.ci == 1)
        return taps <= kSmTaps && g.co % 4 == 0 && g.co >= 4 && g.co <= 64 && 256 % (g.co / 4) == 0 && g.y_ld % 4 == 0 &&
               (int64_t)g.ho * g.wo < 0x7fffffffLL && (int64_t)g.n * g.dout * g.ho < 0x7fffffffLL && !cin1_ok(g);
    return taps <= kSmTaps && g.ci % 4 == 0 && g.co % 4 == 0 && g.ci >= 4 && g.co >= 4 && pv <= 64 && 256 % pv == 0 &&
           g.x_ld % 4 == 0 && g.y_ld % 4 == 0 && (int64_t)g.ho * g.wo < 0x7fffffffLL &&
           (int64_t)g.n * g.dout * g.ho < 0x7fffffffLL;
}

static int pick_tile(int c) { return c >= 16 ? 16 : (c > 4 ? 8 : (c > 2 ? 4 : 2)); }
static int pad_to_tile(int c) { return cdiv(c, pick_tile(c)) * pick_tile(c); }
static size_t packed_w_bytes(const Mri3dConvGeom& g, int pass) {
    const int taps = g.kd * g.kh * g.kw;
    return pass == MRI3D_PASS_FWD ? (size_t)taps * g.ci * pad_to_tile(g.co) * sizeof(float)
                                  : (size_t)taps * g.co * pad_to_tile(g.ci) * sizeof(float);
}

enum class GenKernel { c1c1, c1taps, cin1, taps, gather, strided_taps, strided, co1, quads, small, lds };
struct GenericPlan {
    GenKernel kernel = GenKernel::gather;
    int tl = 0;
    int nt = 0;
    int cv = 0;
    int vec = 0;
    int civ = 0;
    int co_inst = 0;
// ... 97 lines not shown
    int gx = 2048 / (taps * q.gz);
    if (gx < 8) gx = 8;
    if (gx > 256) gx = 256;
    if (gx > nchunks) gx = (int)nchunks;
    if (gx < 1) gx = 1;
    p.slots = gx;
    q.smem = (size_t)kWgCH * (q.Ci4 + q.Co4) * 4 * sizeof(float) + kWgCH * sizeof(int64_t) +
             (q.vsplit > 1 ? 256 * 16 * sizeof(float) : 0);
}

static GenericPlan generic_wgrad_plan(const Mri3dConvGeom& g, int ax, int ay) {
    GenericPlan p;
    const int taps = g.kd * g.kh * g.kw;
    p.CiP = g.ci, p.CoP = g.co;
    size_t slot_floats = 0;
    if (c1c1_ok(g)) {
        p.kernel = GenKernel::c1c1, p.slots = kC1C1Blocks;
    } else if (c1_taps_ok(g) && align16(ay)) {
        p.kernel = GenKernel::c1taps, p.nt = taps <= 3 ? 3 : kSmTaps, p.slots = kC1TBlocks, slot_floats = kSmTaps;
    } else if (cin1_ok(g) && align_vec4(g.dtype, ay)) {
        p.kernel = GenKernel::cin1, p.co_inst = g.co == 8 ? 8 : 16, p.slots = kCin1Shares;
    } else if (wgrad_co1_ok(g) && align_vec4(g.dtype, ax)) {
        p.kernel = GenKernel::co1, p.ci_inst = (g.ci == 1 || g.ci == 4 || g.ci == 8) ? g.ci : 16;
        p.slots = kCo1Blocks, slot_floats = kSmTaps * 16;
    } else if (wgrad_quads_ok(g) && align_vec4(g.dtype, ay) && (g.ci == 1 || align_vec4(g.dtype, ax))) {
        p.kernel = GenKernel::quads, wgrad_quads_plan(g, p);
    } else if (wgrad_small_ok(g)) {
        p.kernel = GenKernel::small, wgrad_small_plan(g, p);
    } else {
        p.kernel = GenKernel::lds, wgrad_lds_plan(g, p);
    }
    p.part_floats = (size_t)p.slots * (slot_floats ? slot_floats : (size_t)taps * p.CiP * p.CoP);
    p.bias_floats = (size_t)p.slots * g.co;
    p.ws_bytes = (p.part_floats + p.bias_floats) * sizeof(float);
    return p;
}

bool conv_generic_route_name(const Mri3dConvGeom& g, int pass, bool bias, int ax, int ay, char* name, size_t name_bytes) {
    const GenericPlan p = pass == MRI3D_PASS_FWD ? generic_fwd_plan(g, ax, ay)
                                                 : (pass == MRI3D_PASS_DGRAD ? generic_dgrad_plan(g, ax, ay) : generic_wgrad_plan(g, ax, ay));
    const char* b = (bias && pass == MRI3D_PASS_DGRAD) ? " bias" : "";
    int len = 0;
    switch (p.kernel) {
    case GenKernel::c1c1: len = snprintf(name, name_bytes, "generic c1c1%s", b); break;
    case GenKernel::c1taps: len = snprintf(name, name_bytes, "generic c1taps nt%d%s", p.nt, b); break;
    case GenKernel::cin1: len = snprintf(name, name_bytes, "generic cin1 co%d", p.co_inst); break;
    case GenKernel::taps: len = snprintf(name, name_bytes, "generic taps tl%d nt%d cv%d%s", p.tl, p.nt, p.cv, b); break;
    case GenKernel::gather: len = snprintf(name, name_bytes, "generic gather tl%d vec%d%s", p.tl, p.vec, b); break;
    case GenKernel::strided_taps: len = snprintf(name, name_bytes, "generic staps tl%d nt%d%s", p.tl, p.nt, b); break;
    case GenKernel::strided: len = snprintf(name, name_bytes, "generic strided tl%d vec%d%s", p.tl, p.vec, b); break;
    case GenKernel::co1: len = snprintf(name, name_bytes, "generic co1 ci%d", p.ci_inst); break;
    case GenKernel::quads: len = snprintf(name, name_bytes, "generic quads nt%d civ%d", p.nt, p.civ); break;
    case GenKernel::small: len = snprintf(name, name_bytes, "generic small"); break;
    case GenKernel::lds: len = snprintf(name, name_bytes, "generic lds"); break;
    }
    return len > 0 && (size_t)len < name_bytes;
}

size_t conv_generic_workspace_bytes(const Mri3dConvGeom& g, int pass) {
    if (pass != MRI3D_PASS_WGRAD) return packed_w_bytes(g, pass);
    size_t a = 0;
    for (int ax : {16, 8, 4})
        for (int ay : {16, 8, 4}) a = std::max(a, generic_wgrad_plan(g, ax, ay).ws_bytes);
    return a;
}

template <int TL>
static void launch_fwd(const Mri3dConvGeom& g, const GenericPlan& p, const void* x, const float* wp, const float* bias, void* y,
                       hipStream_t s) {
    const int CoP = p.cp;
    int64_t nvox = (int64_t)g.n * g.dout * g.ho * g.wo;
    dim3 grid((unsigned)std::min<int64_t>(cdiv64(nvox, 256), 8192), CoP / TL);
    if (p.kernel == GenKernel::taps) {
        const int hch = (int)std::max<int64_t>(1, std::min<int64_t>(g.ho, (int64_t)2048 / std::max(g.wo, 1)));
        const int64_t slabs = (int64_t)g.n * g.dout * cdiv(g.ho, hch);
        dim3 tgrid((unsigned)std::min<int64_t>(slabs, 4096), CoP / TL);
#define MRI3D_FT(NTv, CVv) hipLaunchKernelGGL((conv_fwd_taps_kernel<T, TL, NTv, CVv>), tgrid, dim3(256), 0, s, g, (const T*)x, wp, bias, (T*)y, CoP, hch)
        MRI3D_DISPATCH_DTYPE(g.dtype, T, {
            if (p.cv == 4) { if (p.nt == 3) MRI3D_FT(3, 4); else if (p.nt == 4) MRI3D_FT(4, 4); else if (p.nt == 6) MRI3D_FT(6, 4); else MRI3D_FT(8, 4); }
            else { if (p.nt == 3) MRI3D_FT(3, 1); else if (p.nt == 6) MRI3D_FT(6, 1); else MRI3D_FT(8, 1); }
        });
#undef MRI3D_FT
        return;
    }
    MRI3D_DISPATCH_DTYPE(g.dtype, T, {
        if (p.vec)
            hipLaunchKernelGGL((conv_fwd_generic_kernel<T, TL, true>), grid, dim3(256), 0, s, g, (const T*)x, wp, bias, (T*)y, CoP);
        else
            hipLaunchKernelGGL((conv_fwd_generic_kernel<T, TL, false>), grid, dim3(256), 0, s, g, (const T*)x, wp, bias, (T*)y, CoP);
    });
}

int conv_generic_fwd(const Mri3dConvGeom& g, const void* x, const float* w, const float* bias, void* y, void* ws,
                     size_t ws_bytes, hipStream_t s) {
    const GenericPlan p = generic_fwd_plan(g, ptr_align(x), ptr_align(y));
    if (p.kernel == GenKernel::c1c1) {
        MRI3D_DISPATCH_DTYPE(g.dtype, T, { launch_c1c1_stencil<T>(g, (const T*)x, g.x_ld, w, bias, 0, (T*)y, g.y_ld, s); });
        return check_launch("conv3d_fwd(1->1 stencil)");
    }
    if (p.kernel == GenKernel::c1taps) {
        launch_c1_taps(g, p.nt, (const float*)x, w, bias, (float*)y, 1, s);
        return check_launch("conv3d_fwd(1->1 taps)");
    }
    MRI3D_REQUIRE(ws != nullptr && ws_bytes >= p.ws_bytes, MRI3D_EWORKSPACE, "conv3d_fwd: workspace %zu < %zu", ws_bytes, p.ws_bytes);
    float* wp = static_cast<float*>(ws);
    const int taps = g.kd * g.kh * g.kw;
    if (p.kernel == GenKernel::cin1) {
        hipLaunchKernelGGL(repack_w_kernel, dim3(1), dim3(256), 0, s, w, wp, g.co, 1, 27, g.co, 0);
        const C1Tiles t = cin1_tiles(g);
        const int grid = std::min((int)t.ntiles, 256 * 8);
        MRI3D_DISPATCH_DTYPE(g.dtype, T, {
            if (p.co_inst == 8)
                hipLaunchKernelGGL((conv_cin1_fwd_kernel<T, 8>), dim3(grid), dim3(256), 0, s, g, (const T*)x, wp, bias, (T*)y,
                                   t.tilesD, t.tilesH, t.tilesW, (int)t.ntiles);
            else
                hipLaunchKernelGGL((conv_cin1_fwd_kernel<T, 16>), dim3(grid), dim3(256), 0, s, g, (const T*)x, wp, bias, (T*)y,
                                   t.tilesD, t.tilesH, t.tilesW, (int)t.ntiles);
        });
        return check_launch("conv3d_fwd(cin1)");
    }
    const int TL = p.tl, CoP = p.cp;
    int total = taps * g.ci * CoP;
    hipLaunchKernelGGL(repack_w_kernel, dim3(std::min(cdiv(total, 256), 1024)), dim3(256), 0, s, w, wp, g.co, g.ci, taps, CoP, 0);
    switch (TL) {
        case 16: launch_fwd<16>(g, p, x, wp, bias, y, s); break;
        case 8: launch_fwd<8>(g, p, x, wp, bias, y, s); break;
        case 4: launch_fwd<4>(g, p, x, wp, bias, y, s); break;
        default: launch_fwd<2>(g, p, x, wp, bias, y, s); break;
    }
    return check_launch("conv3d_fwd(generic)");
}

template <int TL>
static void launch_dgrad(const Mri3dConvGeom& g, const GenericPlan& p, const void* dy, const float* wp, const float* bias, void* dx,
                         hipStream_t s) {
    const int CiP = p.cp;
    int64_t nvox = (int64_t)g.n * g.di * g.hi * g.wi;
    dim3 grid((unsigned)std::min<int64_t>(cdiv64(nvox, 256), 8192), CiP / TL);
    if (p.kernel == GenKernel::taps) {
        const int hch = (int)std::max<int64_t>(1, std::min<int64_t>(g.hi, (int64_t)2048 / std::max(g.wi, 1)));
        const int64_t slabs = (int64_t)g.n * g.di * cdiv(g.hi, hch);
        dim3 tgrid((unsigned)std::min<int64_t>(slabs, 4096), CiP / TL);
#define MRI3D_DT(NTv, CVv) hipLaunchKernelGGL((conv_dgrad_taps_kernel<T, TL, NTv, CVv>), tgrid, dim3(256), 0, s, g, (const T*)dy, wp, bias, (T*)dx, CiP, hch)
        MRI3D_DISPATCH_DTYPE(g.dtype, T, {
            if (p.cv == 4) { if (p.nt == 3) MRI3D_DT(3, 4); else if (p.nt == 4) MRI3D_DT(4, 4); else if (p.nt == 6) MRI3D_DT(6, 4); else MRI3D_DT(8, 4); }
            else { if (p.nt == 3) MRI3D_DT(3, 1); else MRI3D_DT(8, 1); }
        });
#undef MRI3D_DT
        return;
    }
    if (p.kernel == GenKernel::strided_taps || p.kernel == GenKernel::strided) {
        dim3 sgrid((unsigned)((int64_t)g.n * g.di * g.hi * g.sw), CiP / TL);
        if (p.kernel == GenKernel::strided_taps) {
            MRI3D_DISPATCH_DTYPE(g.dtype, T, {
                if (p.nt == 3)
                    hipLaunchKernelGGL((conv_dgrad_strided_taps_kernel<T, TL, 3>), sgrid, dim3(64), 0, s, g, (const T*)dy, wp, bias, (T*)dx, CiP);
                else if (p.nt == 4)
                    hipLaunchKernelGGL((conv_dgrad_strided_taps_kernel<T, TL, 4>), sgrid, dim3(64), 0, s, g, (const T*)dy, wp, bias, (T*)dx, CiP);
                else
                    hipLaunchKernelGGL((conv_dgrad_strided_taps_kernel<T, TL, 8>), sgrid, dim3(64), 0, s, g, (const T*)dy, wp, bias, (T*)dx, CiP);
            });
            return;
        }
        MRI3D_DISPATCH_DTYPE(g.dtype, T, {
            if (p.vec)
                hipLaunchKernelGGL((conv_dgrad_strided_kernel<T, TL, true>), sgrid, dim3(64), 0, s, g, (const T*)dy, wp, bias, (T*)dx, CiP);
            else
                hipLaunchKernelGGL((conv_dgrad_strided_kernel<T, TL, false>), sgrid, dim3(64), 0, s, g, (const T*)dy, wp, bias, (T*)dx, CiP);
        });
        return;
    }
    MRI3D_DISPATCH_DTYPE(g.dtype, T, {
        if (p.vec)
            hipLaunchKernelGGL((conv_dgrad_generic_kernel<T, TL, true>), grid, dim3(256), 0, s, g, (const T*)dy, wp, bias, (T*)dx, CiP);
        else
            hipLaunchKernelGGL((conv_dgrad_generic_kernel<T, TL, false>), grid, dim3(256), 0, s, g, (const T*)dy, wp, bias, (T*)dx, CiP);
    });
}

int conv_generic_dgrad(const Mri3dConvGeom& g, const void* dy, const float* w, const float* bias, void* dx, void* ws,
                       size_t ws_bytes, hipStream_t s) {
    const GenericPlan p = generic_dgrad_plan(g, ptr_align(dx), ptr_align(dy));
    if (p.kernel == GenKernel::c1c1) {
        MRI3D_DISPATCH_DTYPE(g.dtype, T, { launch_c1c1_stencil<T>(g, (const T*)dy, g.y_ld, w, bias, 1, (T*)dx, g.x_ld, s); });
        return check_launch("conv3d_dgrad(1->1 stencil)");
    }
    if (p.kernel == GenKernel::c1taps) {
        launch_c1_taps(g, p.nt, (const float*)dy, w, bias, (float*)dx, -1, s);
        return check_launch("conv3d_dgrad(1->1 taps)");
    }
    const int taps = g.kd * g.kh * g.kw;
    const int TL = p.tl, CiP = p.cp;
    MRI3D_REQUIRE(ws != nullptr && ws_bytes >= p.ws_bytes, MRI3D_EWORKSPACE, "conv3d_dgrad: workspace %zu < %zu", ws_bytes, p.ws_bytes);
    float* wp = static_cast<float*>(ws);
    int total = taps * g.co * CiP;
    hipLaunchKernelGGL(repack_w_kernel, dim3(std::min(cdiv(total, 256), 1024)), dim3(256), 0, s, w, wp, g.co, g.ci, taps, CiP, 1);
    switch (TL) {
        case 16: launch_dgrad<16>(g, p, dy, wp, bias, dx, s); break;
        case 8: launch_dgrad<8>(g, p, dy, wp, bias, dx, s); break;
        case 4: launch_dgrad<4>(g, p, dy, wp, bias, dx, s); break;
        default: launch_dgrad<2>(g, p, dy, wp, bias, dx, s); break;
    }
    return check_launch("conv3d_dgrad(generic)");
}

int conv_generic_wgrad(const Mri3dConvGeom& g, const void* x, const void* dy, float* dw, float* dbias, void* ws,
                       size_t ws_bytes, hipStream_t s) {
    const GenericPlan p = generic_wgrad_plan(g, ptr_align(x), ptr_align(dy));
    MRI3D_REQUIRE(ws != nullptr && ws_bytes >= p.ws_bytes, MRI3D_EWORKSPACE, "conv3d_wgrad: workspace %zu < %zu", ws_bytes, p.ws_bytes);
    float* part = static_cast<float*>(ws);
    float* bias_part = dbias ? part + p.part_floats : nullptr;
    const int taps = g.kd * g.kh * g.kw;
    const int64_t nvox = (int64_t)g.n * g.dout * g.ho * g.wo;
    int nb = p.slots;
    const char* what = "conv3d_wgrad(generic)";
    switch (p.kernel) {
    case GenKernel::c1c1: {
        const C1Tiles t = c1_tiles(g.n, g.dout, g.ho, g.wo, 4);
        nb = std::min((int)t.ntiles, kC1C1Blocks), what = "conv3d_wgrad(1->1 stencil)";
        MRI3D_DISPATCH_DTYPE(g.dtype, T, {
            hipLaunchKernelGGL(conv_c1c1_wgrad_kernel<T>, dim3(nb), dim3(256), 0, s, g, (const T*)x, (const T*)dy, part, bias_part,
                               t.tilesD, t.tilesH, t.tilesW, (int)t.ntiles);
        });
        break;
    }
    case GenKernel::c1taps: {
        const int64_t items = (int64_t)g.n * g.dout * g.ho * (g.wo / 4);
        nb = (int)std::max<int64_t>(1, std::min<int64_t>(cdiv64(items, 256 * 4), kC1TBlocks)), what = "conv3d_wgrad(1->1 taps)";
        if (p.nt == 3)
            hipLaunchKernelGGL(conv_c1_taps_wgrad_kernel<3>, dim3(nb), dim3(256), 0, s, g, (const float*)x, (const float*)dy, part, bias_part);
        else
            hipLaunchKernelGGL(conv_c1_taps_wgrad_kernel<kSmTaps>, dim3(nb), dim3(256), 0, s, g, (const float*)x, (const float*)dy, part, bias_part);
        break;
    }
    case GenKernel::cin1: {
        const C1Tiles t = cin1_tiles(g);
        what = "conv3d_wgrad(cin1)";
        MRI3D_DISPATCH_DTYPE(g.dtype, T, {
            if (p.co_inst == 8)
                hipLaunchKernelGGL((conv_cin1_wgrad_kernel<T, 8>), dim3(nb), dim3(768), 0, s, g, (const T*)x,
                                   (const T*)dy, part, bias_part, t.tilesD, t.tilesH, t.tilesW, (int)t.ntiles, nb);
            else
                hipLaunchKernelGGL((conv_cin1_wgrad_kernel<T, 16>), dim3(nb), dim3(768), 0, s, g, (const T*)x,
                                   (const T*)dy, part, bias_part, t.tilesD, t.tilesH, t.tilesW, (int)t.ntiles, nb);
        });
        break;
    }
    case GenKernel::co1: {
        nb = (int)std::min<int64_t>(cdiv64(nvox, 256), kCo1Blocks), what = "conv3d_wgrad(co1)";
#define MRI3D_CO1(CIv) hipLaunchKernelGGL((conv_wgrad_co1_kernel<T, CIv>), dim3(nb), dim3(256), 0, s, g, (const T*)x, (const T*)dy, part, bias_part)
        MRI3D_DISPATCH_DTYPE(g.dtype, T, {
            switch (p.ci_inst) {
                case 1: MRI3D_CO1(1); break;
                case 4: MRI3D_CO1(4); break;
                case 8: MRI3D_CO1(8); break;
                default: MRI3D_CO1(16); break;
            }
        });
#undef MRI3D_CO1
        break;
    }
    case GenKernel::quads: {
        what = "conv3d_wgrad(quads)";
#define MRI3D_WGQ(NTv, CIVv)                                                                                           \
    hipLaunchKernelGGL((conv_wgrad_quads_kernel<T, NTv, CIVv>), dim3(nb), dim3(256), 0, s, g, (const T*)x, (const T*)dy,  \
                       part, bias_part, p.quads.QI, p.quads.QO, p.quads.hch, p.CiP, p.CoP)
        MRI3D_DISPATCH_DTYPE(g.dtype, T, {
            if (p.civ == 1) MRI3D_WGQ(8, 1);
            else if (p.nt == 4) MRI3D_WGQ(4, 4);
            else if (p.nt == 6) MRI3D_WGQ(6, 4);
            else MRI3D_WGQ(8, 4);
        });
#undef MRI3D_WGQ
        break;
    }
    case GenKernel::small: {
        what = "conv3d_wgrad(small)";
        MRI3D_DISPATCH_DTYPE(g.dtype, T, {
            hipLaunchKernelGGL(conv_wgrad_small_kernel<T>, dim3(nb, p.small.gy, p.small.gz), dim3(256), 0, s, g, (const T*)x,
                               (const T*)dy, part, bias_part, p.small.CiL, p.CiP, p.CoP);
        });
        break;
    }
    case GenKernel::lds: {
        const auto& q = p.lds;
        MRI3D_REQUIRE(q.smem <= 160 * 1024, MRI3D_ENOTSUP, "conv3d_wgrad: Ci=%d Co=%d needs %zu B of LDS", g.ci, g.co, q.smem);
        MRI3D_DISPATCH_DTYPE(g.dtype, T, {
            static const hipError_t attr_ = hipFuncSetAttribute(reinterpret_cast<const void*>(conv_wgrad_generic_kernel<T>),
                                                                hipFuncAttributeMaxDynamicSharedMemorySize, 160 * 1024);
            (void)attr_;
            hipLaunchKernelGGL(conv_wgrad_generic_kernel<T>, dim3(nb, taps, q.gz), dim3(256), q.smem, s, g, (const T*)x,
                               (const T*)dy, part, bias_part, q.Ci4, q.Co4, q.nitems, q.vsplit);
        });
        break;
    }
    case GenKernel::taps: case GenKernel::gather: case GenKernel::strided_taps: case GenKernel::strided:
        MRI3D_REQUIRE(false, MRI3D_EINVAL, "conv3d_wgrad: no weight-gradient kernel in the plan");
    }
    hipLaunchKernelGGL(wgrad_reduce_kernel, dim3(cdiv(g.co * g.ci * taps + g.co, 8)), dim3(256), 0, s, part, bias_part, dw, dbias, nb,
                       taps, g.ci, g.co, p.CiP, p.CoP);
    return check_launch(what);
}

}
```

### mri_epilepsy_diagnosis_amd/nn.py

```python
import math

import torch
import torch.nn as tnn

from . import ops


class Conv3d(tnn.Conv3d):
    def forward(self, x):
        if self.padding_mode != "zeros" or self.groups != 1 or isinstance(self.padding, str):
            raise NotImplementedError("mri3d Conv3d supports padding_mode='zeros', groups=1, numeric padding")
        return ops.conv3d(x, self.weight, self.bias, self.stride, self.padding, self.dilation)


class ConvTranspose3d(tnn.ConvTranspose3d):
    def forward(self, x, output_size=None):
        if output_size is not None or self.groups != 1 or self.padding_mode != "zeros":
            raise NotImplementedError("mri3d ConvTranspose3d supports groups=1, zero padding, no output_size")
        return ops.conv_transpose3d(x, self.weight, self.bias, self.stride, self.padding, self.output_padding,
                                    self.dilation)


class BayesConv3d(tnn.Module):

    def __init__(self, in_channels, out_channels, kernel_size, stride=1, padding=0, dilation=1, groups=1, bias=True,
                 zero_mean=False, threshold=3):
        super().__init__()
        if in_channels % groups != 0 or out_channels % groups != 0:
            raise ValueError("in_channels and out_channels must be divisible by groups")
        self.in_channels, self.out_channels, self.groups = in_channels, out_channels, groups
        self.kernel_size, self.stride, self.dilation = ops._triple(kernel_size), ops._triple(stride), ops._triple(dilation)
        self.padding = padding if isinstance(padding, str) else ops._triple(padding)
        self.zero_mean, self.threshold = zero_mean, threshold
        self.noise = None
        self.log_alpha = None
        shape = (out_channels, in_channels // groups) + self.kernel_size
        self.mu_weight = tnn.Parameter(torch.empty(shape))
        self.logsigma_weight = tnn.Parameter(torch.empty(shape))
        if bias:
            self.mu_bias = tnn.Parameter(torch.empty(out_channels))
            self.logsigma_bias = tnn.Parameter(torch.empty(out_channels))
        else:
            self.register_parameter("mu_bias", None)
            self.register_parameter("logsigma_bias", None)
        self.reset_parameters()
        if zero_mean:
            self.mu_weight = tnn.Parameter(torch.zeros_like(self.mu_weight))

    def reset_parameters(self):
        with torch.no_grad():
            self.mu_weight.normal_(0, 0.02)
            self.logsigma_weight.fill_(-5)
            if self.mu_bias is not None:
                fan_in = self.mu_weight[0].numel()
                bound = 1 / math.sqrt(fan_in)
                self.mu_bias.uniform_(-bound, bound)
                self.logsigma_bias.uniform_(-bound, bound)

    def output_shape(self, x):
        return (x.shape[0], self.out_channels) + tuple(
            (i + 2 * p - d * (k - 1) - 1) // s + 1
            for i, p, d, k, s in zip(x.shape[2:], self.padding, self.dilation, self.kernel_size, self.stride))

    def extra_repr(self):
        return "%d, %d, kernel_size=%s, stride=%s, padding=%s%s" % (self.in_channels, self.out_channels, self.kernel_size, self.stride,
                                                                    self.padding, "" if self.mu_bias is not None else ", bias=False")

    def forward(self, x):
        if self.groups != 1 or isinstance(self.padding, str):
            raise NotImplementedError("mri3d BayesConv3d supports groups=1, numeric padding")
        eps = self.noise(self.output_shape(x), x.device) if self.noise is not None else None
        y, self.log_alpha = ops.bayes_conv3d(x, self.mu_weight, self.logsigma_weight, self.mu_bias, self.logsigma_bias, self.stride,
                                             self.padding, self.dilation, self.training, self.threshold, eps)
        return y


def _act_spec(act):
    if act is None or isinstance(act, tnn.Identity):
        return None, None, 0.0
    if isinstance(act, tnn.PReLU):
        return "prelu", act.weight, 0.0
    if isinstance(act, tnn.LeakyReLU):
        return "leaky_relu", None, float(act.negative_slope)
    if isinstance(act, tnn.ReLU):
        return "relu", None, 0.0
    raise NotImplementedError("unsupported activation module %r" % (act,))


def _batchnorm_spec(norm, alpha):
    use_batch = norm.training or norm.running_mean is None
    mode = "running" if not use_batch else ("sync" if norm.training and ops.sync_batchnorm_reducer() is not None else "batch")
    running = (norm.running_mean, norm.running_var) if norm.track_running_stats else (None, None)
    return mode, (norm.weight, norm.bias, alpha, *running, mode, norm.momentum, norm.eps)


def _count_batch(norm):
    if norm is not None and norm.training and norm.track_running_stats and norm.num_batches_tracked is not None:
        norm.num_batches_tracked.add_(1)


def fused_norm_act(norm, act, x, out=None):
    kind, alpha, slope = _act_spec(act)
    if norm is None:
        if kind is None and out is None:
            return x
        return ops.norm_act(x, None, None, alpha, None, None, "none", 0.1, 0.0, kind, slope, out)
    if isinstance(norm, tnn.modules.batchnorm._BatchNorm):
        _count_batch(norm)
        return ops.norm_act(x, *_batchnorm_spec(norm, alpha)[1], kind, slope, out)
    if isinstance(norm, tnn.modules.instancenorm._InstanceNorm):
        if norm.track_running_stats:
            raise NotImplementedError("InstanceNorm3d(track_running_stats=True) is not supported")
        return ops.norm_act(x, norm.weight, norm.bias, alpha, None, None, "instance", 0.1, norm.eps, kind, slope, out)
    if isinstance(norm, tnn.GroupNorm):
        return ops.norm_act(x, norm.weight, norm.bias, alpha, None, None, "group", 0.1, norm.eps, kind, slope, out,
                            norm.num_channels // norm.num_groups)
    raise NotImplementedError("unsupported normalisation module %r" % (norm,))


def _plain_pointwise(head):
    return (isinstance(head, Conv3d) and tuple(head.kernel_size) == (1, 1, 1) and tuple(head.stride) == (1, 1, 1)
            and tuple(head.dilation) == (1, 1, 1) and head.groups == 1 and head.padding_mode == "zeros"
            and not isinstance(head.padding, str) and tuple(head.padding) == (0, 0, 0))


def _local_stats_spec(norm, act):
    kind, alpha, slope = _act_spec(act)
    if norm is None:
        return "none", (None, None, alpha, None, None, "none", 0.1, 0.0), kind, alpha, slope
    if not isinstance(norm, tnn.modules.batchnorm._BatchNorm) or norm.momentum is None:
        return None
    mode, args = _batchnorm_spec(norm, alpha)
    return None if mode == "sync" else (mode, args, kind, alpha, slope)


def _fused_tail(norm, act, supported, asked, run, given):
    spec = _local_stats_spec(norm, act)
    if spec is None:
        return None
    mode, args, kind, alpha, slope = spec
    if not supported(*asked, mode, kind, alpha):
        return None
    _count_batch(norm)
    return run(*given, *args, act=kind, slope=slope)


def fused_norm_act_head(norm, act, x, head):
    if not _plain_pointwise(head):
        return None
    cast = ops.autocast_dtype()
    if cast is not None and x.dtype != cast:
        return None
    return _fused_tail(norm, act, ops.norm_act_pointwise_supported, (x, head.weight), ops.norm_act_pointwise,
                       (x, head.weight, head.bias))


def fused_norm_act_pool(norm, act, x, pool):
    if (not isinstance(pool, tnn.MaxPool3d) or pool.ceil_mode or pool.return_indices or pool.dilation not in (1, (1, 1, 1))
            or not x.is_cuda):
        return None
    if x.dtype != torch.float32:
        return None
    return _fused_tail(norm, act, ops.norm_act_pool_supported, (x, pool.kernel_size, pool.stride, pool.padding), ops.norm_act_pool,
                       (x,))


def conv_norm_act(conv, norm, act, x, out=None, head=None, pool=None):
    wants = (isinstance(norm, tnn.modules.batchnorm._BatchNorm) and (norm.training or norm.running_mean is None)
             and ops.sync_batchnorm_reducer() is None and isinstance(conv, Conv3d) and conv.padding_mode == "zeros"
             and conv.groups == 1 and not isinstance(conv.padding, str))
    if isinstance(x, (tuple, list)):
        xa, xb = x
        plain = (isinstance(conv, Conv3d) and conv.padding_mode == "zeros" and conv.groups == 1 and not isinstance(conv.padding, str)
                 and tuple(conv.stride) == (1, 1, 1) and tuple(conv.dilation) == (1, 1, 1))
        if plain:
            y = ops.conv3d_cat(xa, xb, conv.weight, conv.bias, conv.padding, bn_stats=wants)
        else:
            y = conv(ops.cat_channels([xa, xb]))
    elif wants:
        y = ops.conv3d(x, conv.weight, conv.bias, conv.stride, conv.padding, conv.dilation, bn_stats=True)
    else:
        y = conv(x)
    if head is not None:
        logits = fused_norm_act_head(norm, act, y, head) if out is None else None
        return logits if logits is not None else head(fused_norm_act(norm, act, y, out))
    if pool is not None:
        both = fused_norm_act_pool(norm, act, y, pool) if out is None else None
        return both if both is not None else pool.forward_with_skip(fused_norm_act(norm, act, y, out))
    return fused_norm_act(norm, act, y, out)


class GroupNorm(tnn.GroupNorm):
    def forward(self, x):
        return fused_norm_act(self, None, x)


class BatchNorm3d(tnn.BatchNorm3d):
    def forward(self, x):
        return fused_norm_act(self, None, x)


class InstanceNorm3d(tnn.InstanceNorm3d):
    def forward(self, x):
        return fused_norm_act(self, None, x)


class PReLU(tnn.PReLU):
    def forward(self, x):
        if x.dim() != 5:
            return super().forward(x)
        return fused_norm_act(None, self, x)


class ReLU(tnn.ReLU):
    def forward(self, x):
        if x.dim() != 5:
            return super().forward(x)
        return fused_norm_act(None, self, x)


class LeakyReLU(tnn.LeakyReLU):
    def forward(self, x):
        if x.dim() != 5:
            return super().forward(x)
        return fused_norm_act(None, self, x)


class MaxPool3d(tnn.MaxPool3d):
    def forward(self, x):
        if self.ceil_mode or self.return_indices or self.dilation not in (1, (1, 1, 1)):
            raise NotImplementedError("mri3d MaxPool3d supports floor mode, dilation 1, no indices")
        return ops.max_pool3d(x, self.kernel_size, self.stride, self.padding)

    def forward_with_skip(self, x):
        if self.ceil_mode or self.return_indices or self.dilation not in (1, (1, 1, 1)):
            raise NotImplementedError("mri3d MaxPool3d supports floor mode, dilation 1, no indices")
        return ops.max_pool3d_skip(x, self.kernel_size, self.stride, self.padding)


def _pair(v):
    return (v, v) if isinstance(v, int) else tuple(v)


def _as_slice(x, who):
    if x.dim() == 4:
        return x.unsqueeze(2), True
    if x.dim() == 5 and x.shape[2] == 1:
        return x, False
    raise RuntimeError("mri3d %s expects (N, C, H, W) or (N, C, 1, H, W), got shape %s" % (who, tuple(x.shape)))


class Conv2d(tnn.Conv2d):
    def forward(self, x):
        if self.padding_mode != "zeros" or self.groups != 1 or isinstance(self.padding, str):
            raise NotImplementedError("mri3d Conv2d supports padding_mode='zeros', groups=1, numeric padding")
        x, four = _as_slice(x, "Conv2d")
        y = ops.conv3d(x, self.weight.unsqueeze(2), self.bias, (1,) + _pair(self.stride), (0,) + _pair(self.padding),
                       (1,) + _pair(self.dilation))
        return y.squeeze(2) if four else y


class BatchNorm2d(tnn.BatchNorm2d):
    def forward(self, x):
        x, four = _as_slice(x, "BatchNorm2d")
        y = fused_norm_act(self, None, x)
        return y.squeeze(2) if four else y


class MaxPool2d(tnn.MaxPool2d):
    def forward(self, x):
        if self.ceil_mode or self.return_indices or self.dilation not in (1, (1, 1)):
            raise NotImplementedError("mri3d MaxPool2d supports floor mode, dilation 1, no indices")
        x, four = _as_slice(x, "MaxPool2d")
        stride = self.kernel_size if self.stride is None else self.stride
        y = ops.max_pool3d(x, (1,) + _pair(self.kernel_size), (1,) + _pair(stride), (0,) + _pair(self.padding))
        return y.squeeze(2) if four else y


class Upsample(tnn.Upsample):
    def forward(self, x):
        return ops.upsample3d(x, self.size, self.scale_factor, self.mode, self.align_corners)


class Dropout3d(tnn.Dropout3d):
    def forward(self, x):
        return ops.dropout3d(x, self.p, self.training)


class Flatten(tnn.Module):

    def forward(self, x):
        return x.contiguous(memory_format=torch.contiguous_format).view(x.size(0), -1)


_NORMS = (tnn.modules.batchnorm._BatchNorm, tnn.modules.instancenorm._InstanceNorm)
_ACTS = (tnn.PReLU, tnn.ReLU, tnn.LeakyReLU)


def run_fused(modules, x):
    mods = list(modules)
    i = 0
    while i < len(mods):
        m = mods[i]
        five_d = torch.is_tensor(x) and x.dim() == 5
        if (five_d and i == 0 and isinstance(m, Conv3d) and len(mods) > 2 and isinstance(mods[1], Conv3d) and isinstance(mods[2], Conv3d)
                and ops.conv3d_pair_supported(x, m, mods[1])):
            x = ops.conv3d_pair(x, m, mods[1])
            i += 2
            continue
        if five_d and isinstance(m, Conv3d) and i + 1 < len(mods) and isinstance(mods[i + 1], tnn.BatchNorm3d):
            nxt2 = mods[i + 2] if i + 2 < len(mods) else None
            if isinstance(nxt2, _ACTS):
                x = conv_norm_act(m, mods[i + 1], nxt2, x)
                i += 3
            else:
                x = conv_norm_act(m, mods[i + 1], None, x)
                i += 2
            continue
        if five_d and isinstance(m, (tnn.BatchNorm3d, tnn.InstanceNorm3d, tnn.GroupNorm)):
            nxt = mods[i + 1] if i + 1 < len(mods) else None
            if isinstance(nxt, _ACTS):
                x = fused_norm_act(m, nxt, x)
                i += 2
                continue
            x = fused_norm_act(m, None, x)
        elif five_d and isinstance(m, _ACTS):
            x = fused_norm_act(None, m, x)
        else:
            x = m(x)
        i += 1
    return x


class FusedSequential(tnn.Sequential):
    def forward(self, x):
        return run_fused(self, x)
```

### mri_epilepsy_diagnosis_amd/ops.py

```python
import collections
import ctypes
import math

import torch

from . import _lib
from ._lib import (ACT_LEAKY, ACT_NONE, ACT_PRELU, ACT_RELU, BF16, F32, NORM_PASS_BWD, NORM_PASS_FWD, NORM_PASS_STATS, PASS_DGRAD,
                   PASS_FWD, PASS_WGRAD, UP_NEAREST, UP_TRILINEAR, ConvGeom, DiceGeom, NormGeom, NormPlanInfo, PoolGeom, UpGeom,
                   check)

CL3D = torch.channels_last_3d



def _require_device(*ts):
    for t in ts:
        if t is None:
            continue
        if not t.is_cuda:
            raise RuntimeError(
                "mri_epilepsy_diagnosis_amd ops run only on a ROCm device tensor (got %s); there is no CPU fallback"
                % t.device)
        if t.dtype not in (torch.float32, torch.bfloat16):
            raise RuntimeError("mri_epilepsy_diagnosis_amd ops: only float32 / bfloat16 tensors are supported, got %s"
# ... 353 lines not shown
    check(_lib.lib().mri3d_norm_plan_query(ctypes.byref(g), pass_, align, ctypes.byref(info)), "norm_plan_query")
    return (info.vec, info.CL, info.VT, info.cy, info.nblk, info.groups, info.gvox)


def _stuffed_wgrad_ok(g):
    return ((g.kd, g.kh, g.kw) == (3, 3, 3) and (g.sd, g.sh, g.sw) == (2, 2, 2) and (g.pd, g.ph, g.pw) == (1, 1, 1)
            and (g.dd, g.dh, g.dw) == (1, 1, 1) and g.ci % 8 == 0 and g.co % 4 == 0 and g.x_ld % 4 == 0)


_ONE = (1, 1, 1)
_ConvPasses = collections.namedtuple("_ConvPasses", "fwd dgrad wgrad stuffed layer")


def _conv_passes(xshape, wshape, stride, padding, dilation, dtype=F32, x_ld=None, dy_ld=None, dx_ld=None):
    fwd = _conv_geom(xshape, wshape, stride, padding, dilation, x_ld=x_ld, dtype=dtype)
    dgrad = _conv_geom(xshape, wshape, stride, padding, dilation, x_ld=dx_ld, y_ld=dy_ld, dtype=dtype)
    wgrad = _conv_geom(xshape, wshape, stride, padding, dilation, x_ld=fwd.x_ld, y_ld=dy_ld, dtype=dtype)
    stuffed = _conv_geom(xshape, wshape, _ONE, _ONE, _ONE, x_ld=fwd.x_ld, dtype=dtype) if _stuffed_wgrad_ok(fwd) else None
    return _ConvPasses(fwd, dgrad, wgrad, stuffed, (tuple(xshape), tuple(wshape), stride, padding, dilation, dtype, x_ld, dx_ld))


def _for_gradient_pitch(p, dy_ld):
    return p if dy_ld == p.wgrad.y_ld else _conv_passes(*p.layer[:7], dy_ld=dy_ld, dx_ld=p.layer[7])


def _cat_passes(xa, xb, wshape, a_ld, dy_ld=None):
    ca = xa.shape[1]
    return _conv_passes((xa.shape[0], ca + xb.shape[1]) + tuple(xa.shape[2:]), wshape, _ONE, _ONE, _ONE, _dt(xa), a_ld, dy_ld, dx_ld=ca)


def _upconv_passes(xshape, wshape, scale, padding, dtype, x_ld, dy_ld=None):
    n, c, d, h, w = xshape
    return _conv_passes((n, c, d * scale, h * scale, w * scale), wshape, _ONE, padding, _ONE, dtype, x_ld, dy_ld)


def _pair_passes(xshape, x_ld, dtype, w1shape, conv1, w2shape, conv2):
    g1 = _conv_passes(xshape, w1shape, _triple(conv1.stride), _triple(conv1.padding), _ONE, dtype, x_ld).fwd
    return g1, _conv_passes((g1.n, g1.co, g1.dout, g1.ho, g1.wo), w2shape, _triple(conv2.stride), _triple(conv2.padding), _ONE, dtype)


def _transpose_geom(xshape, wshape, stride, padding, output_padding, dilation, dtype):
    out = tuple((i - 1) * s - 2 * p + d * (k - 1) + op + 1 for i, s, p, d, k, op in zip(xshape[2:], stride, padding, dilation, wshape[2:], output_padding))
    g = _conv_geom((xshape[0], wshape[1]) + out, wshape, stride, padding, dilation, dtype=dtype)
    if (g.dout, g.ho, g.wo) != tuple(xshape[2:]):
        raise RuntimeError("conv_transpose3d: inconsistent output_padding")
    return g


def conv3d_routes(xshape, wshape, stride=1, padding=0, dilation=1, dtype=F32, x_ld=None, dy_ld=None, bias=True, bn_stats=False,
                  x_align=16, dy_align=16):
    p = _conv_passes(xshape, wshape, _triple(stride), _triple(padding), _triple(dilation), dtype, x_ld, dy_ld)
    fwd = conv_route(p.fwd, PASS_FWD, bn_stats, bias, x_align=x_align, y_align=16) if bn_stats else "none"
    if fwd == "none":
        fwd = conv_route(p.fwd, PASS_FWD, False, bias, x_align=x_align, y_align=16)
    gw, wy_align = (p.wgrad, dy_align) if p.stuffed is None else (p.stuffed, 16)
    return {"fwd": fwd, "dgrad": conv_route(p.dgrad, PASS_DGRAD, x_align=16, y_align=dy_align),
            "wgrad": conv_route(gw, PASS_WGRAD, x_align=x_align, y_align=wy_align)}


def conv_transpose3d_routes(xshape, wshape, stride=1, padding=0, output_padding=0, dilation=1, dtype=F32, bias=True, x_align=16,
                            dy_align=16):
    g = _transpose_geom(xshape, wshape, _triple(stride), _triple(padding), _triple(output_padding), _triple(dilation), dtype)
    return {"fwd": conv_route(g, PASS_DGRAD, False, bias, x_align=16, y_align=x_align),
            "dgrad": conv_route(g, PASS_FWD, x_align=dy_align, y_align=16),
            "wgrad": conv_route(g, PASS_WGRAD, x_align=dy_align, y_align=x_align)}


def _carg(a):
    return _ptr(a) if a is None or torch.is_tensor(a) else ctypes.byref(a) if isinstance(a, ctypes.Structure) else a


def _launch(fn, tag, work, ws_bytes, device, *args):
    tail = ()
    if ws_bytes is not None:
        ws = _workspace(ws_bytes, device)
        tail = (_ptr(ws), ws.numel())
    with _timed(tag, work):
        rc = fn(*map(_carg, args), *tail, _stream())
        if rc != 0:
            check(rc, fn.__name__[len("mri3d_"):])


def _conv_launch(fn, pass_, g, device, *args, suffix=""):
    kind = ("fwd", "dgrad", "wgrad")[pass_]
    _launch(fn, lambda: _conv_tag(kind, g) + suffix, lambda: _conv_work(g, kind),
            _lib.lib().mri3d_conv3d_workspace_bytes(ctypes.byref(g), pass_), device, g, *args)


def _conv_fwd(g, x, w, b, part=None):
    y = _new((g.n, g.co, g.dout, g.ho, g.wo), x)
    if part is None:
        _conv_launch(_lib.lib().mri3d_conv3d_fwd, PASS_FWD, g, x.device, x, w, b, y)
    else:
        _conv_launch(_lib.lib().mri3d_conv3d_fwd_stats, PASS_FWD, g, x.device, x, w, b, y, part, suffix=" +bn-stats")
    return y


def _conv_dgrad(g, dy, w, b, like):
    dx = _new((g.n, g.ci, g.di, g.hi, g.wi), like)
    _conv_launch(_lib.lib().mri3d_conv3d_dgrad, PASS_DGRAD, g, dy.device, dy, w, b, dx)
    return dx


class GradSink:

    __slots__ = ("view", "fresh")

    def __init__(self, view):
        self.view, self.fresh = view, True


_sinks_suspended = 0


class suspend_grad_sinks:

    def __enter__(self):
        global _sinks_suspended
        _sinks_suspended += 1
        return self

    def __exit__(self, *exc):
        global _sinks_suspended
        _sinks_suspended -= 1
        return False


def _live_sink(param):
    if _sinks_suspended:
        return None
    sink = getattr(param, "_mri3d_grad_sink", None) if param is not None else None
    if sink is None or param.grad is None or param.grad.data_ptr() != sink.view.data_ptr() or sink.view.shape != param.shape:
        return None
    return sink


def _sink_take(param):
    sink = _live_sink(param)
    if sink is None or not sink.fresh:
        return None
    sink.fresh = False
    return sink.view


def _sink_done(param, grad, out):
    if grad is None or out is not None:
        return None
    sink = _live_sink(param)
    if sink is None or sink.view.shape != grad.shape:
        return grad
    sink.view.add_(grad)
    return None


def _grad_slots(ctx, saved, first=1, params=None, all_written=False):
    params = ctx.params if params is None else params
    want = [t is not None and ctx.needs_input_grad[first + i] for i, t in enumerate(saved)]
    sinks = [_sink_take(p) if wt else None for p, wt in zip(params, want)]
    grads = [(sk if sk is not None else torch.empty_like(t, memory_format=torch.contiguous_format))
             if wt or (all_written and t is not None) else None for sk, t, wt in zip(sinks, saved, want)]
    return sinks, grads


def _grad_slots_done(ctx, grads, sinks, first=1, params=None):
    params = ctx.params if params is None else params
    return tuple(_sink_done(p, gr, sk) if ctx.needs_input_grad[first + i] else None for i, (p, gr, sk) in enumerate(zip(params, grads, sinks)))


def _conv_param_grads(ctx, first, params, wgrad):
    if not any(p is not None and ctx.needs_input_grad[first + i] for i, p in enumerate(params)):
        return None, None
    sinks, grads = _grad_slots(ctx, params, first, params, all_written=True)
    wgrad(*grads)
    return _grad_slots_done(ctx, grads, sinks, first, params)


def _conv_wgrad(g, x, dy, w_like, want_bias, dw_out=None, db_out=None, split=None):
    L = _lib.lib()
    dw = dw_out if dw_out is not None else torch.empty_like(w_like, memory_format=torch.contiguous_format)
    db = (db_out if db_out is not None else torch.empty(g.co, dtype=w_like.dtype, device=w_like.device)) if want_bias else None
    if split is None:
        _conv_launch(L.mri3d_conv3d_wgrad, PASS_WGRAD, g, x.device, x, dy, dw, db)
    else:
        _conv_launch(L.mri3d_conv3d_wgrad_cat, PASS_WGRAD, g, x.device, x, *split, dy, dw, db, suffix=" cat")
    return dw, db


def _stuffed_wgrad(p, x, dy):
    if p.stuffed is None or dy.dtype != x.dtype:
        return p.wgrad, dy
    g = p.fwd
    dyw = torch.empty((g.n, g.co, g.di, g.hi, g.wi), dtype=dy.dtype, device=dy.device, memory_format=CL3D).zero_()
    dyw[:, :, ::2, ::2, ::2].copy_(dy)
    return p.stuffed, dyw


def _autocast_in(x):
    return convert(x, _autocast_dtype) if _autocast_dtype is not None and x.dtype != _autocast_dtype else x


def _stats_partials(holder, blocks, g, x, bias):
    if blocks <= 0:
        return None
    part = torch.empty(blocks * g.co * 2, dtype=torch.float64, device=x.device)
    holder.append((part, blocks, bias.detach() if bias is not None else None))
    return part


def _apply_with_bn_stats(fn, bn_stats, *args):
    holder = [] if bn_stats else None
    y = fn.apply(*args, holder)
    if holder:
        y._mri3d_bn_stats = holder[0]
    return y


class _Conv3dFn(torch.autograd.Function):
    @staticmethod
    def forward(ctx, x, weight, bias, stride, padding, dilation, stats_holder=None):
        _require_device(x)
        _require_param(weight, bias)
        x, x_ld = _nd(x)
        w = weight.contiguous()
        p = _conv_passes(x.shape, w.shape, stride, padding, dilation, _dt(x), x_ld)
        g = p.fwd
        part = _stats_partials(stats_holder, _lib.lib().mri3d_conv3d_fwd_stats_blocks(ctypes.byref(g)), g, x, bias) if stats_holder is not None else None
        y = _conv_fwd(g, x, w, bias, part)
        ctx.save_for_backward(x, w)
        ctx.passes, ctx.params = p, (weight, bias)
        return y

    @staticmethod
    def backward(ctx, dy):
        x, w = ctx.saved_tensors
        dy, y_ld = _nd(dy)
        p = _for_gradient_pitch(ctx.passes, y_ld)
        dx = _conv_dgrad(p.dgrad, dy, w, None, x) if ctx.needs_input_grad[0] else None

        def wgrad(dw, db):
            gw, dyw = _stuffed_wgrad(p, x, dy)
            _conv_wgrad(gw, x, dyw, w, db is not None, dw, db)
        return (dx, *_conv_param_grads(ctx, 1, ctx.params, wgrad), None, None, None, None)


class _Conv3dCatFn(torch.autograd.Function):

    @staticmethod
    def forward(ctx, xa, xb, weight, bias, stats_holder=None):
        _require_device(xa, xb)
        _require_param(weight, bias)
        L = _lib.lib()
        xa, a_ld = _nd(xa)
        xb, b_ld = _nd(xb)
        w = weight.contiguous()
        p = _cat_passes(xa, xb, w.shape, a_ld)
        g, ca = p.fwd, xa.shape[1]
        y = _new((g.n, g.co, g.dout, g.ho, g.wo), xa)
        ws_bytes = L.mri3d_conv3d_workspace_bytes(ctypes.byref(g), PASS_FWD)
        part = None
        if stats_holder is not None:
            part = _stats_partials(stats_holder, L.mri3d_conv3d_fwd_cat_stats_blocks(ctypes.byref(g), ca, b_ld), g, xa, bias)
        _launch(L.mri3d_conv3d_fwd_cat, lambda: _conv_tag("fwd", g) + " cat" + (" +bn-stats" if part is not None else ""),
                lambda: _conv_work(g, "fwd"), ws_bytes, xa.device, g, xa, xb, ca, b_ld, w, bias, y, part)
        ctx.save_for_backward(xa, xb, w)
        ctx.passes, ctx.b_ld, ctx.params = p, b_ld, (weight, bias)
        return y

    @staticmethod
    def backward(ctx, dy):
        xa, xb, w = ctx.saved_tensors
        dy, y_ld = _nd(dy)
        p = _for_gradient_pitch(ctx.passes, y_ld)
        ca, cb = xa.shape[1], xb.shape[1]
        dxa = dxb = None
        if ctx.needs_input_grad[0] or ctx.needs_input_grad[1]:
            dxa, dxb = _new(xa.shape, xa), _new(xb.shape, xb)
            _conv_launch(_lib.lib().mri3d_conv3d_dgrad_cat, PASS_DGRAD, p.dgrad, dy.device, dy, w, dxa, dxb, ca, cb, suffix=" cat")
        dw, db = _conv_param_grads(ctx, 2, ctx.params, lambda dw, db: _conv_wgrad(p.wgrad, xa, dy, w, db is not None, dw, db,
                                                                                 split=(xb, ca, ctx.b_ld)))
        return dxa, dxb, dw, db, None


def conv3d_cat(xa, xb, weight, bias=None, padding=1, bn_stats=False):
    xa, xb = _autocast_in(xa), _autocast_in(xb)
    ok = (xa.is_cuda and xa.dim() == 5 and xb.shape[0] == xa.shape[0] and xb.shape[2:] == xa.shape[2:] and xa.dtype == xb.dtype
          and tuple(weight.shape[2:]) == (3, 3, 3) and _triple(padding) == (1, 1, 1) and weight.shape[1] == xa.shape[1] + xb.shape[1])
    if ok:
        L = _lib.lib()
        a_nd, a_ld = _nd(xa)
        b_nd, b_ld = _nd(xb)
        ca, cb = xa.shape[1], xb.shape[1]
        p = _cat_passes(a_nd, b_nd, weight.shape, a_ld)
        ok = (a_nd.data_ptr() % 16 == 0 and b_nd.data_ptr() % 16 == 0
              and L.mri3d_conv3d_cat_supported(ctypes.byref(p.fwd), ca, b_ld, PASS_FWD)
              and L.mri3d_conv3d_cat_supported(ctypes.byref(p.fwd), ca, b_ld, PASS_WGRAD)
              and L.mri3d_conv3d_cat_supported(ctypes.byref(p.dgrad), ca, cb, PASS_DGRAD))
    if not ok:
        return conv3d(cat_channels([xa, xb]), weight, bias, 1, padding, 1, bn_stats=bn_stats)
    return _apply_with_bn_stats(_Conv3dCatFn, bn_stats, xa, xb, weight, bias)


def conv3d(x, weight, bias=None, stride=1, padding=0, dilation=1, bn_stats=False):
    return _apply_with_bn_stats(_Conv3dFn, bn_stats, _autocast_in(x), weight, bias, _triple(stride), _triple(padding), _triple(dilation))




class _BayesWeightsFn(torch.autograd.Function):

    @staticmethod
    def forward(ctx, mu, logsigma, evaluate, threshold):
        _require_param(mu, logsigma)
        if mu.shape != logsigma.shape:
            raise RuntimeError("bayes_conv3d: mu_weight %s and logsigma_weight %s differ in shape" % (tuple(mu.shape), tuple(logsigma.shape)))
        mu, logsigma = mu.contiguous(), logsigma.contiguous()
        w_var, log_alpha = torch.empty_like(mu), torch.empty_like(mu)
        w_mean = torch.empty_like(mu) if evaluate else None
        check(_lib.lib().mri3d_bayes_weights_fwd(_ptr(mu), _ptr(logsigma), mu.numel(), int(evaluate), float(threshold), _ptr(w_mean),
                                                 _ptr(w_var), _ptr(log_alpha), _stream()), "bayes_weights_fwd")
        ctx.save_for_backward(mu, logsigma)
        ctx.evaluate, ctx.threshold = bool(evaluate), float(threshold)
        ctx.set_materialize_grads(False)
        return (w_mean, w_var, log_alpha) if evaluate else (w_var, log_alpha)

    @staticmethod
    def backward(ctx, *grads):
        mu, logsigma = ctx.saved_tensors
        d_w_mean, d_w_var, d_log_alpha = grads if ctx.evaluate else (None,) + grads
        d_w_mean, d_w_var, d_log_alpha = (None if g is None else g.contiguous() for g in (d_w_mean, d_w_var, d_log_alpha))
        dmu, dls = torch.empty_like(mu), torch.empty_like(mu)
        check(_lib.lib().mri3d_bayes_weights_bwd(_ptr(mu), _ptr(logsigma), mu.numel(), int(ctx.evaluate), ctx.threshold, _ptr(d_w_mean),
                                                 _ptr(d_w_var), _ptr(d_log_alpha), _ptr(dmu), _ptr(dls), _stream()),
              "bayes_weights_bwd")
        return dmu, dls, None, None


def _stream_work(n_tensors, like, eps_numel=0):
    return {"flops": 0.0, "bytes": _esz(like) * n_tensors * like.numel() + 4.0 * eps_numel}


def _bayes_square(x, x_ld):
    n, c, d, h, w = x.shape
    x2 = _new(x.shape, x)
    _launch(_lib.lib().mri3d_bayes_square, lambda: "bayes_square %d @%dx%dx%d n%d" % (c, d, h, w, n), lambda: _stream_work(2, x), None, None,
            x, x2, n * d * h * w, c, x_ld, c, _dt(x))
    return x2


class _BayesConv3dFn(torch.autograd.Function):

    @staticmethod
    def forward(ctx, x, w_mean, w_var, mu_bias, logsigma_bias, eps, stride, padding, dilation):
        _require_device(x)
        _require_param(w_mean, w_var, mu_bias, logsigma_bias, eps)
        L = _lib.lib()
        x, x_ld = _nd(x)
        w_mean, w_var = w_mean.contiguous(), w_var.contiguous()
        pm = _conv_passes(x.shape, w_mean.shape, stride, padding, dilation, _dt(x), x_ld)
        pv = _conv_passes(x.shape, w_var.shape, stride, padding, dilation, _dt(x))
        g = pm.fwd
        y = _conv_fwd(g, x, w_mean, mu_bias)
        var_bias = logsigma_bias * logsigma_bias if logsigma_bias is not None else None
        var_out = _conv_fwd(pv.fwd, _bayes_square(x, x_ld), w_var, var_bias)
        if tuple(eps.shape) != tuple(y.shape):
            raise RuntimeError("bayes_conv3d: eps has shape %s, the output %s" % (tuple(eps.shape), tuple(y.shape)))
        eps, eps_ld = _nd(eps)
        nvox = g.n * g.dout * g.ho * g.wo
        _launch(L.mri3d_bayes_sample_fwd, lambda: "bayes_sample_fwd %d @%dx%dx%d n%d" % (g.co, g.dout, g.ho, g.wo, g.n),
                lambda: _stream_work(3, y, eps.numel()), None, None, y, var_out, eps, y, nvox, g.co, g.co, g.co, eps_ld, g.co, g.dtype)
        ctx.save_for_backward(x, w_mean, w_var, var_out, eps, logsigma_bias)
        ctx.passes, ctx.eps_ld, ctx.has_bias = (pm, pv), eps_ld, mu_bias is not None
        return y

    @staticmethod
    def backward(ctx, dy):
        L = _lib.lib()
        x, w_mean, w_var, var_out, eps, logsigma_bias = ctx.saved_tensors
        dy, y_ld = _nd(dy)
        pm, pv = _for_gradient_pitch(ctx.passes[0], y_ld), ctx.passes[1]
        g = pm.fwd
        nvox = g.n * g.dout * g.ho * g.wo
        dvar = _new(dy.shape, dy)
        _launch(L.mri3d_bayes_sample_bwd, lambda: "bayes_sample_bwd %d @%dx%dx%d n%d" % (g.co, g.dout, g.ho, g.wo, g.n),
                lambda: _stream_work(3, dy, eps.numel()), None, None, dy, var_out, eps, dvar, nvox, g.co, y_ld, g.co, ctx.eps_ld, g.co, g.dtype)
        dx = dw_mean = dw_var = dmb = dlb = None
        if ctx.needs_input_grad[0]:
            dx = _conv_dgrad(pm.dgrad, dy, w_mean, None, x)
            dx_var = _conv_dgrad(pv.dgrad, dvar, w_var, None, x)
            _launch(L.mri3d_bayes_dx, lambda: "bayes_dx %d @%dx%dx%d n%d" % (g.ci, g.di, g.hi, g.wi, g.n), lambda: _stream_work(4, x), None, None,
                    dx, dx_var, x, dx, g.n * g.di * g.hi * g.wi, g.ci, g.ci, g.ci, g.x_ld, g.ci, g.dtype)
        want_b = ctx.has_bias and (ctx.needs_input_grad[3] or ctx.needs_input_grad[4])
        if ctx.needs_input_grad[1] or ctx.needs_input_grad[2] or want_b:
            gw, dyw = _stuffed_wgrad(pm, x, dy)
            dw_mean, dmb = _conv_wgrad(gw, x, dyw, w_mean, ctx.has_bias)
            gw2, dvw = _stuffed_wgrad(pv, x, dvar)
            dw_var, dvb = _conv_wgrad(gw2, _bayes_square(x, g.x_ld), dvw, w_var, ctx.has_bias)
            if ctx.has_bias:
                dlb = 2.0 * logsigma_bias * dvb
        return dx, dw_mean, dw_var, dmb, dlb, None, None, None, None


def bayes_conv3d(x, mu_weight, logsigma_weight, mu_bias=None, logsigma_bias=None, stride=1, padding=0, dilation=1, training=True,
                 threshold=3, eps=None, groups=1):
    if groups != 1:
        raise NotImplementedError("bayes_conv3d: groups != 1 is not supported")
    if isinstance(padding, str):
        raise NotImplementedError("bayes_conv3d: string padding is not supported")
    if (mu_bias is None) != (logsigma_bias is None):
        raise RuntimeError("bayes_conv3d: mu_bias and logsigma_bias come together")
    _require_device(x)
    x = _autocast_in(x)
    stride, padding, dilation = _triple(stride), _triple(padding), _triple(dilation)
    g = _conv_geom(x.shape, mu_weight.shape, stride, padding, dilation)
    if training:
        w_mean = mu_weight
        w_var, log_alpha = _BayesWeightsFn.apply(mu_weight, logsigma_weight, False, threshold)
    else:
        w_mean, w_var, log_alpha = _BayesWeightsFn.apply(mu_weight, logsigma_weight, True, threshold)
    if eps is None:
        eps = torch.empty((g.n, g.dout, g.ho, g.wo, g.co), dtype=torch.float32, device=x.device).normal_().permute(0, 4, 1, 2, 3)
    y = _BayesConv3dFn.apply(x, w_mean, w_var, mu_bias, logsigma_bias, eps.detach(), stride, padding, dilation)
    return y, log_alpha


class _ConvPairFn(torch.autograd.Function):

    @staticmethod
    def forward(ctx, x, w1, b1, w2, b2, conv1, conv2):
        _require_device(x)
        _require_param(w1, b1)
        _require_param(w2, b2)
        x, x_ld = _nd(x)
        w1c, w2c = w1.contiguous(), w2.contiguous()
        g1, p2 = _pair_passes(x.shape, x_ld, _dt(x), w1c.shape, conv1, w2c.shape, conv2)
        a1 = _conv_fwd(g1, x, w1c, b1)
        y = _conv_fwd(p2.fwd, a1, w2c, b2)
        ctx.save_for_backward(x, a1, w2c)
        ctx.passes, ctx.params = (g1, p2), (w1, b1, w2, b2)
        return y

    @staticmethod
    def backward(ctx, dy):
        L = _lib.lib()
        x, a1, w2c = ctx.saved_tensors
        w1, b1, w2, b2 = ctx.params
        dy, y_ld = _nd(dy)
        g1, gw2 = ctx.passes[0], _for_gradient_pitch(ctx.passes[1], y_ld).wgrad
        dw2, db2 = _conv_param_grads(ctx, 3, (w2, b2), lambda dw, db: _conv_wgrad(gw2, a1, dy, w2c, db is not None, dw, db))

        def wgrad_first(dw, db):
            _launch(L.mri3d_convpair_wgrad_first, lambda: _conv_tag("wgrad", g1) + " through " + _conv_tag("dgrad", gw2),
                    lambda: {"flops": _conv_work(g1, "wgrad")["flops"] + _conv_work(gw2, "dgrad")["flops"],
                             "bytes": _esz(dy) * (x.numel() + dy.numel())},
                    L.mri3d_convpair_workspace_bytes(ctypes.byref(g1), ctypes.byref(gw2)), x.device, g1, gw2, x, dy, w2c, dw, db)
        dw1, db1 = _conv_param_grads(ctx, 1, (w1, b1), wgrad_first)
        return None, dw1, db1, dw2, db2, None, None


def conv3d_pair_supported(x, conv1, conv2):
    if not (torch.is_tensor(x) and x.dim() == 5 and x.is_cuda) or x.requires_grad or _autocast_dtype is not None:
        return False
    if _triple(conv1.dilation) != (1, 1, 1) or _triple(conv2.dilation) != (1, 1, 1) or conv1.weight.shape[1] != x.shape[1]:
        return False
    try:
        g1, p2 = _pair_passes(x.shape, _pitch_of(x) or x.shape[1], _dt(x), conv1.weight.shape, conv1, conv2.weight.shape, conv2)
    except RuntimeError:
        return False
    return bool(_lib.lib().mri3d_convpair_supported(ctypes.byref(g1), ctypes.byref(p2.fwd)))


def conv3d_pair(x, conv1, conv2):
    if conv3d_pair_supported(x, conv1, conv2):
        return _ConvPairFn.apply(x, conv1.weight, conv1.bias, conv2.weight, conv2.bias, conv1, conv2)
    y = conv3d(x, conv1.weight, conv1.bias, conv1.stride, conv1.padding, conv1.dilation)
    return conv3d(y, conv2.weight, conv2.bias, conv2.stride, conv2.padding, conv2.dilation)


def _channel_sum(t):
    L = _lib.lib()
    n, c, d, h, w = t.shape
    g = NormGeom(n, d * h * w, c, c, c, 0, ACT_NONE, 1, 0.0, 0.0, 0, _dt(t))
    mean = torch.empty(c, dtype=torch.float32, device=t.device)
    invstd = torch.empty(c, dtype=torch.float32, device=t.device)
    ws = _workspace(L.mri3d_norm_workspace_bytes(ctypes.byref(g)), t.device)
    check(L.mri3d_norm_stats(ctypes.byref(g), _ptr(t), _ptr(mean), _ptr(invstd), None, None, 0.0, _ptr(ws), ws.numel(),
                             _stream()), "norm_stats")
    return mean * float(n * d * h * w)


class _ConvTranspose3dFn(torch.autograd.Function):

    @staticmethod
    def forward(ctx, x, weight, bias, stride, padding, output_padding, dilation):
        _require_device(x)
        _require_param(weight, bias)
        x = _cl(x)
        w = weight.contiguous()
        if w.shape[0] != x.shape[1]:
            raise RuntimeError("conv_transpose3d: weight expects %d input channels, got %d" % (w.shape[0], x.shape[1]))
        g = _transpose_geom(x.shape, w.shape, stride, padding, output_padding, dilation, _dt(x))
        y = _conv_dgrad(g, x, w, bias, x)
        ctx.save_for_backward(x, w)
        ctx.geom, ctx.has_bias = g, bias is not None
        return y

    @staticmethod
    def backward(ctx, dy):
        x, w = ctx.saved_tensors
        g = ctx.geom
        dy = _cl(dy)
        dx = dw = db = None
        if ctx.needs_input_grad[0]:
            dx = _conv_fwd(g, dy, w, None)
        if ctx.needs_input_grad[1]:
            dw, _ = _conv_wgrad(g, dy, x, w, False)
        if ctx.has_bias and ctx.needs_input_grad[2]:
            db = _channel_sum(dy)
        return dx, dw, db, None, None, None, None


def conv_transpose3d(x, weight, bias=None, stride=1, padding=0, output_padding=0, dilation=1):
    return _ConvTranspose3dFn.apply(_autocast_in(x), weight, bias, _triple(stride), _triple(padding), _triple(output_padding),
                                    _triple(dilation))



_ACT_CODES = {None: ACT_NONE, "none": ACT_NONE, "relu": ACT_RELU, "leaky_relu": ACT_LEAKY, "prelu": ACT_PRELU}

_sync_bn_reducer = None


def set_sync_batchnorm(reducer):
    global _sync_bn_reducer
    prev, _sync_bn_reducer = _sync_bn_reducer, reducer
    return prev


def sync_batchnorm_reducer():
    return _sync_bn_reducer


def _sync_statistics(reducer, g, x, running_mean, running_var, momentum, eps):
    c = g.c
    mean_l, invstd_l = _norm_statistics("norm_act", g, x, 1, "batch", None, None, momentum, eps, None)
    cnt_l = float(g.n * g.vox)
    shift = running_mean.detach().double() if running_mean is not None else torch.zeros(c, dtype=torch.float64, device=x.device)
    m64 = mean_l.double() - shift
    var_l = (1.0 / invstd_l.double() ** 2 - float(eps)).clamp_(min=0.0)
    pack = torch.cat([torch.full((1,), cnt_l, dtype=torch.float64, device=x.device), cnt_l * m64,
                      cnt_l * (var_l + m64 * m64)])
    pack = reducer.all_reduce(pack)
    cnt = pack[0]
    gm_s = pack[1:1 + c] / cnt
    gmean = gm_s + shift
    gvar = (pack[1 + c:] / cnt - gm_s * gm_s).clamp_(min=0.0)
    mean = gmean.to(torch.float32).contiguous()
    invstd = torch.rsqrt(gvar + float(eps)).to(torch.float32).contiguous()
    if running_mean is not None:
        with torch.no_grad():
            unb = gvar * (cnt / torch.clamp(cnt - 1.0, min=1.0))
            running_mean.mul_(1.0 - momentum).add_(momentum * gmean.to(running_mean.dtype))
            running_var.mul_(1.0 - momentum).add_(momentum * unb.to(running_var.dtype))
    return mean, invstd, cnt


def _sync_correct_dx(reducer, g, x, mean, invstd, gamma, dbeta, dgamma, cnt, dx):
    L = _lib.lib()
    tot = reducer.all_reduce(torch.cat([dbeta.double(), dgamma.double()]))
    gam = gamma.double() if gamma is not None else torch.ones(g.c, dtype=torch.float64, device=x.device)
    a0 = (-gam * invstd.double() * tot[:g.c] / cnt).to(torch.float32).contiguous()
    b1 = (-gam * invstd.double() ** 2 * tot[g.c:] / cnt).to(torch.float32).contiguous()
    ones = torch.ones(g.c, dtype=torch.float32, device=x.device)
    corr = _new(x.shape, x)
    ga = NormGeom(g.n, g.vox, g.c, g.c, g.c, 0, ACT_NONE, 1, 0.0, 0.0, 0, g.dtype)
    check(L.mri3d_norm_act_fwd(ctypes.byref(ga), _ptr(x), _ptr(mean), _ptr(ones), _ptr(b1), _ptr(a0), None, _ptr(corr),
                               _stream()), "norm_act_fwd")
    check(L.mri3d_add_channels(_ptr(dx), _ptr(corr), _ptr(dx), g.n * g.vox, g.c, g.c, g.c, g.c, g.dtype, _stream()),
          "add_channels")


def _norm_geom(x, x_ld, y_ld, act_code, alpha, slope, eps, instance=0, group_c=0):
    n, c, d, h, w = x.shape
    alpha_n = 1 if act_code != ACT_PRELU else (alpha.numel() if alpha is not None else 0)
    return NormGeom(n, d * h * w, c, x_ld, y_ld, instance, act_code, alpha_n, float(slope), float(eps), group_c, _dt(x))


def _repitched(g, x_ld, y_ld, dtype=None):
    g = type(g).from_buffer_copy(g)
    g.x_ld, g.y_ld = x_ld, y_ld
    if dtype is not None:
        g.dtype = dtype
    return g


def _norm_statistics(who, g, x, groups, mode, running_mean, running_var, momentum, eps, fused_stats):
    if mode == "none":
        return None, None
    if mode == "running":
        return (running_mean.detach().to(torch.float32).contiguous(),
                torch.rsqrt(running_var.detach().to(torch.float32) + eps).contiguous())
    if mode != "batch":
        raise RuntimeError("%s: statistics mode %r is not served" % (who, mode))
    L = _lib.lib()
    c = g.c
    g = _repitched(g, g.x_ld, g.x_ld)
    mean = torch.empty(groups * c, dtype=torch.float32, device=x.device)
# ... 936 lines not shown
```

### mri_epilepsy_diagnosis_amd/unet/unet.py

```python
import torch
import torch.nn as tnn

from .. import nn as mnn
from .. import ops

_UPSAMPLING = {"nearest": "nearest", "linear": "trilinear", "trilinear": "trilinear"}


class ConvolutionalBlock(tnn.Module):
    def __init__(self, dimensions, in_channels, out_channels, normalization=None, kernel_size=3, activation="ReLU",
                 preactivation=False, padding=0, padding_mode="zeros", dilation=None, dropout=0):
        super().__init__()
        if dimensions != 3:
            raise NotImplementedError("only the 3-D U-Net of the reference is implemented")
        if preactivation or padding_mode != "zeros" or dropout:
            raise NotImplementedError("preactivation / non-zero padding_mode / dropout are not used by the reference")
        dilation = 1 if dilation is None else dilation
        if padding:
            total = kernel_size + 2 * (dilation - 1) - 1
            padding = total // 2
        conv = mnn.Conv3d(in_channels, out_channels, kernel_size, padding=padding, dilation=dilation)
        norm = None
        if normalization is not None:
            norm = {"batch": mnn.BatchNorm3d, "instance": mnn.InstanceNorm3d}[normalization.lower()](out_channels)
        act = None
        if activation is not None:
            act = {"PReLU": mnn.PReLU, "ReLU": mnn.ReLU, "LeakyReLU": mnn.LeakyReLU}[activation]()
        self.conv_layer = conv
        self.norm_layer = norm
        self.activation_layer = act
        self.dropout_layer = None
        self.block = tnn.Sequential(*[m for m in (conv, norm, act) if m is not None])

    def forward(self, x, out=None, head=None, pool=None):
        return mnn.conv_norm_act(self.conv_layer, self.norm_layer, self.activation_layer, x, out, head, pool)


class EncodingBlock(tnn.Module):
    def __init__(self, in_channels, out_channels_first, dimensions, normalization, pooling_type, preactivation=False,
                 is_first_block=False, residual=False, padding=0, padding_mode="zeros", activation="ReLU",
                 dilation=None, dropout=0):
        super().__init__()
        if residual:
            raise NotImplementedError("residual encoding blocks are not used by the reference")
        self.conv1 = ConvolutionalBlock(dimensions, in_channels, out_channels_first,
                                        normalization=None if is_first_block else normalization,
                                        padding=padding, activation=activation, dilation=dilation)
        out_channels_second = 2 * out_channels_first
        self.conv2 = ConvolutionalBlock(dimensions, out_channels_first, out_channels_second, normalization=normalization,
                                        padding=padding, activation=activation, dilation=dilation)
        self.downsample = None
        if pooling_type is not None:
            if pooling_type != "max":
                raise NotImplementedError("only max pooling is used by the reference")
            self.downsample = mnn.MaxPool3d(kernel_size=2)

    def forward(self, x, skip_out=None, head=None, fused_pool=True):
        if self.downsample is None:
            return self.conv2(self.conv1(x), skip_out, head)
        if fused_pool and skip_out is None and isinstance(self.downsample, mnn.MaxPool3d):
            return self.conv2(self.conv1(x), pool=self.downsample)
        x = self.conv2(self.conv1(x), skip_out)
        return self.downsample.forward_with_skip(x)

    @property
    def out_channels(self):
        return self.conv2.conv_layer.out_channels


class Encoder(tnn.Module):
    def __init__(self, in_channels, out_channels_first, dimensions, pooling_type, num_encoding_blocks, normalization,
                 padding=0, activation="ReLU", initial_dilation=None):
        super().__init__()
        self.encoding_blocks = tnn.ModuleList()
        self.dilation = initial_dilation
        first = True
        for _ in range(num_encoding_blocks):
            blk = EncodingBlock(in_channels, out_channels_first, dimensions, normalization, pooling_type,
                                is_first_block=first, padding=padding, activation=activation, dilation=self.dilation)
            first = False
            self.encoding_blocks.append(blk)
            in_channels = 2 * out_channels_first
            out_channels_first = in_channels
            if self.dilation is not None:
                self.dilation *= 2

    def forward(self, x, cat_bufs=None, fused_pool=True):
        skips = []
        for i, blk in enumerate(self.encoding_blocks):
            x, skip = blk(x, None if cat_bufs is None else (cat_bufs[i], 0), fused_pool=fused_pool)
            skips.append(skip)
        return skips, x

    @property
    def out_channels(self):
        return self.encoding_blocks[-1].out_channels


class DecodingBlock(tnn.Module):
    def __init__(self, in_channels_skip_connection, dimensions, upsampling_type, normalization, padding=0,
                 activation="ReLU", dilation=None):
        super().__init__()
        if upsampling_type == "conv":
            c = 2 * in_channels_skip_connection
            self.upsample = mnn.ConvTranspose3d(c, c, kernel_size=2, stride=2)
        else:
            mode = _UPSAMPLING[upsampling_type]
            self.upsample = mnn.Upsample(scale_factor=2, mode=mode, align_corners=False if mode == "trilinear" else None)
        in_first = in_channels_skip_connection * 3
        self.conv1 = ConvolutionalBlock(dimensions, in_first, in_channels_skip_connection, normalization=normalization,
                                        padding=padding, activation=activation, dilation=dilation)
        self.conv2 = ConvolutionalBlock(dimensions, in_channels_skip_connection, in_channels_skip_connection,
                                        normalization=normalization, padding=padding, activation=activation,
                                        dilation=dilation)

    def forward(self, skip, x, cat_buf=None, head=None):
        if cat_buf is not None and isinstance(self.upsample, mnn.Upsample):
            up = ops.upsample3d(x, self.upsample.size, self.upsample.scale_factor, self.upsample.mode,
                                self.upsample.align_corners, out=(cat_buf, skip.shape[1]))
            return self.conv2(self.conv1(ops.join_channels(cat_buf, [skip, up])), head=head)
        x = self.upsample(x)
        if skip.shape[2:] != x.shape[2:]:
            raise NotImplementedError("padding=False (centre-cropped skips) is not used by the reference")
        return self.conv2(self.conv1((skip, x)), head=head)


class Decoder(tnn.Module):
    def __init__(self, in_channels_skip_connection, dimensions, upsampling_type, num_decoding_blocks, normalization,
                 padding=0, activation="ReLU", initial_dilation=None):
        super().__init__()
        self.decoding_blocks = tnn.ModuleList()
        self.dilation = initial_dilation
        for _ in range(num_decoding_blocks):
            self.decoding_blocks.append(DecodingBlock(in_channels_skip_connection, dimensions, upsampling_type,
                                                      normalization, padding=padding, activation=activation,
                                                      dilation=self.dilation))
            in_channels_skip_connection //= 2
            if self.dilation is not None:
                self.dilation //= 2

    def forward(self, skips, x, cat_bufs=None, head=None):
        last = min(len(skips), len(self.decoding_blocks)) - 1
        for j, (skip, blk) in enumerate(zip(reversed(skips), self.decoding_blocks)):
            x = blk(skip, x, None if cat_bufs is None else cat_bufs[len(skips) - 1 - j], head if j == last else None)
        return x


class UNet(tnn.Module):
    def __init__(self, in_channels=1, out_classes=2, dimensions=2, num_encoding_blocks=5, out_channels_first_layer=64,
                 normalization=None, pooling_type="max", upsampling_type="conv", preactivation=False, residual=False,
                 padding=0, padding_mode="zeros", activation="ReLU", initial_dilation=None, dropout=0,
                 monte_carlo_dropout=0):
        super().__init__()
        if dimensions != 3:
            raise NotImplementedError("only dimensions=3 (the reference's configuration) is implemented")
        if preactivation or residual or dropout or padding_mode != "zeros":
            raise NotImplementedError("option not used by the reference and not implemented")
        if not padding:
            raise NotImplementedError("padding=False (valid convolutions + cropped skips) is not used by the reference")
        depth = num_encoding_blocks - 1
        self.encoder = Encoder(in_channels, out_channels_first_layer, dimensions, pooling_type, depth, normalization,
                               padding=padding, activation=activation, initial_dilation=initial_dilation)
        c = self.encoder.out_channels if depth > 0 else in_channels
        first = c if depth > 0 else out_channels_first_layer
        self.bottom_block = EncodingBlock(c, first, dimensions, normalization, pooling_type=None, padding=padding,
                                          activation=activation, dilation=self.encoder.dilation,
                                          is_first_block=depth == 0)
        skip_channels = out_channels_first_layer * 2 ** depth
        self.decoder = Decoder(skip_channels, dimensions, upsampling_type, depth, normalization, padding=padding,
                               activation=activation, initial_dilation=self.encoder.dilation)
        self.monte_carlo_layer = mnn.Dropout3d(p=monte_carlo_dropout) if monte_carlo_dropout else None
        self.shared_concat_buffers = False
        self.fused_head = True
        self.fused_pool = True
        self.classifier = ConvolutionalBlock(dimensions, 2 * out_channels_first_layer, out_classes, kernel_size=1,
                                             activation=None)

    def forward(self, x):
        cat_bufs = None
        if self.shared_concat_buffers and x.is_cuda and len(self.encoder.encoding_blocks) and all(
                isinstance(b.upsample, mnn.Upsample) for b in self.decoder.decoding_blocks):
            cat_bufs = []
            n, sp = x.shape[0], tuple(x.shape[2:])
            for blk in self.encoder.encoding_blocks:
                if any(s % 2 for s in sp):
                    cat_bufs = None
                    break
                cat_bufs.append(ops.new_cat_buffer(n, 3 * blk.out_channels, sp, x))
                sp = tuple(s // 2 for s in sp)
        clf = self.classifier
        mc = self.monte_carlo_layer
        mc = mc if (mc is not None and mc.training and mc.p > 0) else None
        head = clf.conv_layer if (self.fused_head and mc is None and x.is_cuda and clf.norm_layer is None
                                  and clf.activation_layer is None and clf.dropout_layer is None) else None
        skips, enc = self.encoder(x, cat_bufs, self.fused_pool)
        if not skips:
            x = self.bottom_block(enc, head=head)
        else:
            x = self.decoder(skips, self.bottom_block(enc), cat_bufs, head)
        if head is not None:
            return x
        return self.classifier(x if mc is None else mc(x))
```

Before: 69.11 volumes/s.

## Fuse first-layer 1-channel conv with activation in forward and backward

```diff
diff --git a/include/mri3d.h b/include/mri3d.h
--- a/include/mri3d.h
+++ b/include/mri3d.h
@@ -45,6 +45,17 @@
 
 int mri3d_conv3d_route(const Mri3dConvGeom* g, int32_t pass, int32_t stats, int32_t bias, int32_t split, int32_t second_ld,
                        int32_t align_x, int32_t align_y, char* name, size_t name_bytes);
+
+int32_t mri3d_conv_cin1_act_supported(const Mri3dConvGeom* g, int32_t a_ld, int32_t act, int32_t alpha_n, int32_t pass, int32_t align);
+size_t mri3d_conv_cin1_act_workspace_bytes(const Mri3dConvGeom* g, int32_t pass);
+int mri3d_conv_cin1_act_route(const Mri3dConvGeom* g, int32_t a_ld, int32_t act, int32_t alpha_n, int32_t pass, int32_t align,
+                              char* name, size_t name_bytes);
+int mri3d_conv_cin1_act_fwd(const Mri3dConvGeom* g, int32_t a_ld, int32_t act, int32_t alpha_n, float slope, const void* x,
+                            const void* w, const void* bias, const void* alpha, void* z, void* a, void* workspace, size_t ws_bytes,
+                            mri3d_stream_t stream);
+int mri3d_conv_cin1_act_bwd(const Mri3dConvGeom* g, int32_t da_ld, int32_t act, int32_t alpha_n, float slope, const void* x,
+                            const void* z, const void* da, const void* alpha, void* dw, void* dbias, void* dalpha, void* workspace,
+                            size_t ws_bytes, mri3d_stream_t stream);
 
 int32_t mri3d_conv3d_cat_supported(const Mri3dConvGeom* g, int32_t split, int32_t second_ld, int32_t pass);
 int32_t mri3d_conv3d_fwd_cat_stats_blocks(const Mri3dConvGeom* g, int32_t split, int32_t second_ld);
diff --git a/mri_epilepsy_diagnosis_amd/_lib.py b/mri_epilepsy_diagnosis_amd/_lib.py
--- a/mri_epilepsy_diagnosis_amd/_lib.py
+++ b/mri_epilepsy_diagnosis_amd/_lib.py
@@ -80,6 +80,11 @@
     "mri3d_conv3d_wgrad": (c_int32, [POINTER(ConvGeom), _P, _P, _P, _P, _P, c_size_t, _P]),
     "mri3d_conv3d_route": (c_int32, [POINTER(ConvGeom), c_int32, c_int32, c_int32, c_int32, c_int32, c_int32, c_int32, c_char_p, c_size_t]),
     "mri3d_conv3d_cat_supported": (c_int32, [POINTER(ConvGeom), c_int32, c_int32, c_int32]),
+    "mri3d_conv_cin1_act_supported": (c_int32, [POINTER(ConvGeom), c_int32, c_int32, c_int32, c_int32, c_int32]),
+    "mri3d_conv_cin1_act_workspace_bytes": (c_size_t, [POINTER(ConvGeom), c_int32]),
+    "mri3d_conv_cin1_act_route": (c_int32, [POINTER(ConvGeom), c_int32, c_int32, c_int32, c_int32, c_int32, c_char_p, c_size_t]),
+    "mri3d_conv_cin1_act_fwd": (c_int32, [POINTER(ConvGeom), c_int32, c_int32, c_int32, c_float, _P, _P, _P, _P, _P, _P, _P, c_size_t, _P]),
+    "mri3d_conv_cin1_act_bwd": (c_int32, [POINTER(ConvGeom), c_int32, c_int32, c_int32, c_float, _P, _P, _P, _P, _P, _P, _P, _P, c_size_t, _P]),
     "mri3d_conv3d_fwd_cat_stats_blocks": (c_int32, [POINTER(ConvGeom), c_int32, c_int32]),
     "mri3d_conv3d_fwd_cat": (c_int32, [POINTER(ConvGeom), _P, _P, c_int32, c_int32, _P, _P, _P, _P, _P, c_size_t, _P]),
     "mri3d_conv3d_dgrad_cat": (c_int32, [POINTER(ConvGeom), _P, _P, _P, _P, c_int32, c_int32, _P, c_size_t, _P]),
diff --git a/mri_epilepsy_diagnosis_amd/csrc/api.hip b/mri_epilepsy_diagnosis_amd/csrc/api.hip
--- a/mri_epilepsy_diagnosis_amd/csrc/api.hip
+++ b/mri_epilepsy_diagnosis_amd/csrc/api.hip
@@ -213,6 +213,63 @@
     case ConvBackend::mfma: return conv_mfma_wgrad(*g, x, dy, (float*)dw, (float*)dbias, workspace, ws_bytes, s);
     default: return conv_generic_wgrad(*g, x, dy, (float*)dw, (float*)dbias, workspace, ws_bytes, s);
     }
+}
+
+static bool cin1_act_ok(const Mri3dConvGeom* g, int32_t a_ld, int32_t act, int32_t alpha_n, int32_t pass, int32_t align, const char* who) {
+    if (!g || conv_check(g, who) != MRI3D_OK) return false;
+    if (!conv_cin1_act_supported(*g, a_ld, act, alpha_n, pass, align)) return false;
+    return pass == MRI3D_PASS_FWD || conv_backend(*g, MRI3D_PASS_WGRAD, false, 0, 0, align, align) == ConvBackend::generic;
+}
+
+extern "C" int32_t mri3d_conv_cin1_act_supported(const Mri3dConvGeom* g, int32_t a_ld, int32_t act, int32_t alpha_n, int32_t pass,
+                                                 int32_t align) {
+    return cin1_act_ok(g, a_ld, act, alpha_n, pass, align, "conv_cin1_act_supported") ? 1 : 0;
+}
+
+extern "C" size_t mri3d_conv_cin1_act_workspace_bytes(const Mri3dConvGeom* g, int32_t pass) {
+    if (!g || (pass != MRI3D_PASS_FWD && pass != MRI3D_PASS_WGRAD)) return 0;
+    return conv_cin1_act_workspace_bytes(*g, pass);
+}
+
+extern "C" int mri3d_conv_cin1_act_route(const Mri3dConvGeom* g, int32_t a_ld, int32_t act, int32_t alpha_n, int32_t pass,
+                                         int32_t align, char* name, size_t name_bytes) {
+    int rc = conv_check(g, "conv_cin1_act_route");
+    if (rc) return rc;
+    MRI3D_REQUIRE(name != nullptr && name_bytes >= 32, MRI3D_EINVAL, "conv_cin1_act_route: name buffer of at least 32 bytes required");
+    MRI3D_REQUIRE(pass == MRI3D_PASS_FWD || pass == MRI3D_PASS_WGRAD, MRI3D_EINVAL, "conv_cin1_act_route: pass %d", pass);
+    if (!cin1_act_ok(g, a_ld, act, alpha_n, pass, align, "conv_cin1_act_route")) {
+        snprintf(name, name_bytes, "none");
+        return MRI3D_OK;
+    }
+    MRI3D_REQUIRE(conv_cin1_act_route_name(*g, a_ld, act, alpha_n, pass, align, name, name_bytes), MRI3D_EINVAL,
+                  "conv_cin1_act_route: name buffer too small");
+    return MRI3D_OK;
+}
+
+extern "C" int mri3d_conv_cin1_act_fwd(const Mri3dConvGeom* g, int32_t a_ld, int32_t act, int32_t alpha_n, float slope, const void* x,
+                                       const void* w, const void* bias, const void* alpha, void* z, void* a, void* workspace,
+                                       size_t ws_bytes, mri3d_stream_t stream) {
+    int rc = conv_check(g, "conv_cin1_act_fwd");
+    if (rc) return rc;
+    MRI3D_REQUIRE(x && w && z && a, MRI3D_EINVAL, "conv_cin1_act_fwd: null pointer");
+    MRI3D_REQUIRE(act != MRI3D_ACT_PRELU || alpha, MRI3D_EINVAL, "conv_cin1_act_fwd: PReLU needs alpha");
+    MRI3D_REQUIRE(cin1_act_ok(g, a_ld, act, alpha_n, MRI3D_PASS_FWD, ptr_align(z, a, workspace), "conv_cin1_act_fwd"), MRI3D_ENOTSUP,
+                  "conv_cin1_act_fwd: geometry / activation / alignment not served (query mri3d_conv_cin1_act_supported)");
+    return conv_cin1_act_fwd(*g, a_ld, act, alpha_n, slope, (const float*)x, (const float*)w, (const float*)bias, (const float*)alpha,
+                             (float*)z, (float*)a, workspace, ws_bytes, static_cast<hipStream_t>(stream));
+}
+
+extern "C" int mri3d_conv_cin1_act_bwd(const Mri3dConvGeom* g, int32_t da_ld, int32_t act, int32_t alpha_n, float slope, const void* x,
+                                       const void* z, const void* da, const void* alpha, void* dw, void* dbias, void* dalpha,
+                                       void* workspace, size_t ws_bytes, mri3d_stream_t stream) {
+    int rc = conv_check(g, "conv_cin1_act_bwd");
+    if (rc) return rc;
+    MRI3D_REQUIRE(x && z && da && dw, MRI3D_EINVAL, "conv_cin1_act_bwd: null pointer");
+    MRI3D_REQUIRE(act != MRI3D_ACT_PRELU || alpha, MRI3D_EINVAL, "conv_cin1_act_bwd: PReLU needs alpha");
+    MRI3D_REQUIRE(cin1_act_ok(g, da_ld, act, alpha_n, MRI3D_PASS_WGRAD, ptr_align(z, da, workspace), "conv_cin1_act_bwd"), MRI3D_ENOTSUP,
+                  "conv_cin1_act_bwd: geometry / activation / alignment not served (query mri3d_conv_cin1_act_supported)");
+    return conv_cin1_act_bwd(*g, da_ld, act, alpha_n, slope, (const float*)x, (const float*)z, (const float*)da, (const float*)alpha,
+                             (float*)dw, (float*)dbias, (float*)dalpha, workspace, ws_bytes, static_cast<hipStream_t>(stream));
 }
 
 extern "C" int mri3d_conv3d_route(const Mri3dConvGeom* g, int32_t pass, int32_t stats, int32_t bias, int32_t split, int32_t second_ld,
diff --git a/mri_epilepsy_diagnosis_amd/csrc/conv_backends.h b/mri_epilepsy_diagnosis_amd/csrc/conv_backends.h
--- a/mri_epilepsy_diagnosis_amd/csrc/conv_backends.h
+++ b/mri_epilepsy_diagnosis_amd/csrc/conv_backends.h
@@ -16,6 +16,14 @@
 int conv_generic_wgrad(const Mri3dConvGeom& g, const void* x, const void* dy, float* dw, float* dbias, void* ws,
                        size_t ws_bytes, hipStream_t s);
 bool conv_generic_route_name(const Mri3dConvGeom& g, int pass, bool bias, int ax, int ay, char* name, size_t name_bytes);
+bool conv_cin1_act_supported(const Mri3dConvGeom& g, int a_ld, int act, int alpha_n, int pass, int align);
+size_t conv_cin1_act_workspace_bytes(const Mri3dConvGeom& g, int pass);
+bool conv_cin1_act_route_name(const Mri3dConvGeom& g, int a_ld, int act, int alpha_n, int pass, int align, char* name, size_t name_bytes);
+int conv_cin1_act_fwd(const Mri3dConvGeom& g, int a_ld, int act, int alpha_n, float slope, const float* x, const float* w,
+                      const float* bias, const float* alpha, float* z, float* a, void* ws, size_t ws_bytes, hipStream_t s);
+int conv_cin1_act_bwd(const Mri3dConvGeom& g, int da_ld, int act, int alpha_n, float slope, const float* x, const float* z,
+                      const float* da, const float* alpha, float* dw, float* dbias, float* dalpha, void* ws, size_t ws_bytes,
+                      hipStream_t s);
 
 bool conv_mfma_supported(const Mri3dConvGeom& g, int pass);
 size_t conv_mfma_workspace_bytes(const Mri3dConvGeom& g, int pass);
diff --git a/mri_epilepsy_diagnosis_amd/csrc/conv_generic.hip b/mri_epilepsy_diagnosis_amd/csrc/conv_generic.hip
--- a/mri_epilepsy_diagnosis_amd/csrc/conv_generic.hip
+++ b/mri_epilepsy_diagnosis_amd/csrc/conv_generic.hip
@@ -1080,6 +1080,275 @@
     }
 }
 
+struct Cin1Act {
+    const float* alpha;
+    int alpha_n, act;
+    float slope;
+};
+
+template <int CO>
+__global__ void __launch_bounds__(256)
+conv_cin1_act_fwd_kernel(Mri3dConvGeom g, const float* __restrict__ x, const float* __restrict__ wp, const float* __restrict__ bias,
+                         Cin1Act pa, float* __restrict__ z, float* __restrict__ a, int a_ld, int tilesD, int tilesH, int tilesW,
+                         int ntiles) {
+    constexpr int VPT = Cin1<CO>::VPT, TW = C1WQ * VPT, PW = TW + 4;
+    constexpr int Q = CO / 4;
+    constexpr int LS = VPT * CO + 4;
+    constexpr int RS = C1WQ * LS;
+    __shared__ __attribute__((aligned(16))) float xs[(C1D + 2) * (C1H + 2) * PW];
+    __shared__ __attribute__((aligned(16))) float wsh[27 * CO];
+    __shared__ __attribute__((aligned(16))) float turn[C1D][4 * RS];
+    const int tid = threadIdx.x;
+    for (int e = tid; e < 27 * CO; e += 256) wsh[e] = wp[e];
+    const int wq = tid % C1WQ, hl = (tid / C1WQ) % C1H, dl = tid / (C1WQ * C1H);
+    float bv[CO];
+#pragma unroll
+    for (int c = 0; c < CO; ++c) bv[c] = bias ? bias[c] : 0.f;
+    const int lane = tid & 63, tq = lane % Q, tv = lane / Q;
+    const int toff = (tv / VPT) * LS + (tv % VPT) * CO + tq * 4;
+    float al[4];
+#pragma unroll
+    for (int j = 0; j < 4; ++j) al[j] = (pa.act == MRI3D_ACT_PRELU) ? pa.alpha[pa.alpha_n == 1 ? 0 : tq * 4 + j] : pa.slope;
+    float sc = 1.f, sh = 0.f;
+    asm volatile("" : "+v"(sc), "+v"(sh));
+    float* tw = turn[dl];
+    for (int tile = blockIdx.x; tile < ntiles; tile += gridDim.x) {
+        int n, d0, h0, w0;
+        decode_tile(tile, tilesD, tilesH, tilesW, TW, n, d0, h0, w0);
+        __syncthreads();
+        cin1_stage<float, TW, C1D + 2>(xs, x + (int64_t)n * g.di * g.hi * g.wi * g.x_ld, g, d0 - 1, h0, w0, tid);
+        __syncthreads();
+        f32x2 acc[VPT][CO / 2];
+#pragma unroll
+        for (int v = 0; v < VPT; ++v)
+#pragma unroll
+            for (int c = 0; c < CO / 2; ++c) acc[v][c] = f32x2{bv[2 * c], bv[2 * c + 1]};
+#pragma unroll
+        for (int kd = 0; kd < 3; ++kd)
+#pragma unroll
+            for (int kh = 0; kh < 3; ++kh) {
+                const float* row = xs + ((dl + kd) * (C1H + 2) + hl + kh) * PW + wq * VPT;
+                float r[VPT + 2];
+#pragma unroll
+                for (int i = 0; i < VPT + 2; ++i) r[i] = row[i];
+                int woff = (kd * 3 + kh) * 3 * CO;
+                asm volatile("" : "+v"(woff));
+                __builtin_amdgcn_sched_barrier(0);
+                const float* wrow = wsh + woff;
+#pragma unroll
+                for (int kw = 0; kw < 3; ++kw) {
+                    const float* wt = wrow + kw * CO;
+#pragma unroll
+                    for (int c = 0; c < CO / 2; ++c) {
+                        const f32x2 wv = f32x2{wt[2 * c], wt[2 * c + 1]};
+#pragma unroll
+                        for (int v = 0; v < VPT; ++v)
+                            acc[v][c] = __builtin_elementwise_fma(f32x2{r[v + kw], r[v + kw]}, wv, acc[v][c]);
+                    }
+                }
+            }
+#pragma unroll
+        for (int v = 0; v < VPT; ++v)
+#pragma unroll
+            for (int c = 0; c < CO / 2; ++c) asm volatile("" : "+v"(acc[v][c]));
+        const int od = d0 + dl;
+#pragma unroll
+        for (int half = 0; half < 2; ++half) {
+            if ((hl >> 2) == half) {
+                float* dst = tw + (hl & 3) * RS + wq * LS;
+#pragma unroll
+                for (int v = 0; v < VPT; ++v)
+#pragma unroll
+                    for (int c = 0; c < CO; c += 4)
+                        *reinterpret_cast<float4*>(dst + v * CO + c) =
+                            make_float4(acc[v][c / 2].x, acc[v][c / 2].y, acc[v][c / 2 + 1].x, acc[v][c / 2 + 1].y);
+            }
+            __builtin_amdgcn_wave_barrier();
+#pragma unroll
+            for (int j = 0; j < 4; ++j) {
+                const float4 zq = *reinterpret_cast<const float4*>(tw + j * RS + toff);
+                const int oh = h0 + half * 4 + j, ow = w0 + tv;
+                if (od < g.dout && oh < g.ho && ow < g.wo) {
+                    const int64_t vox = (((int64_t)n * g.dout + od) * g.ho + oh) * g.wo + ow;
+                    stf4(z + vox * g.y_ld + tq * 4, zq);
+                    stf4(a + vox * a_ld + tq * 4,
+                         make_float4(apply_act(fmaf(zq.x, sc, sh), pa.act, al[0]), apply_act(fmaf(zq.y, sc, sh), pa.act, al[1]),
+                                     apply_act(fmaf(zq.z, sc, sh), pa.act, al[2]), apply_act(fmaf(zq.w, sc, sh), pa.act, al[3])));
+                }
+            }
+            __builtin_amdgcn_wave_barrier();
+        }
+    }
+}
+
+template <int CO>
+__global__ void __launch_bounds__(768)
+conv_cin1_act_bwd_kernel(Mri3dConvGeom g, const float* __restrict__ x, const float* __restrict__ z, const float* __restrict__ da,
+                         int da_ld, Cin1Act pa, float* __restrict__ part, float* __restrict__ bias_part,
+                         double* __restrict__ alpha_part, int tilesD, int tilesH, int tilesW, int ntiles, int nshares) {
+    constexpr int VPT = Cin1<CO>::VPT, TW = C1WQ * VPT, PW = TW + 4, NA = 9 * CO + CO;
+    constexpr int Q = CO / 4, LS = VPT * CO + 4, RS = C1WQ * LS, NROW = C1D * C1H, RPW = (NROW + 11) / 12;
+    __shared__ __attribute__((aligned(16))) float xs[(C1D + 2) * (C1H + 2) * PW];
+    __shared__ __attribute__((aligned(16))) float dzs[NROW * RS];
+    __shared__ float red[12][NA];
+    __shared__ double ared[12][CO];
+    const int kd = __builtin_amdgcn_readfirstlane((int)threadIdx.x >> 8);
+    const int tid = threadIdx.x & 255;
+    const int per_xcd = gridDim.x / 8;
+    const int share = (blockIdx.x % 8) * per_xcd + blockIdx.x / 8;
+    const int wq = tid % C1WQ, hl = (tid / C1WQ) % C1H, dl = tid / (C1WQ * C1H);
+    const int lane = tid & 63, wave = __builtin_amdgcn_readfirstlane((int)threadIdx.x >> 6);
+    const int tq = lane % Q, tv = lane / Q;
+    const int toff = (tv / VPT) * LS + (tv % VPT) * CO + tq * 4;
+    float al[4];
+#pragma unroll
+    for (int j = 0; j < 4; ++j)
+        al[j] = (pa.act == MRI3D_ACT_PRELU) ? pa.alpha[pa.alpha_n == 1 ? 0 : tq * 4 + j] : (pa.act == MRI3D_ACT_LEAKY ? pa.slope : 0.f);
+    f32x2 acc[3][3][CO / 2];
+    float bsum[CO];
+    double asum[4];
+#pragma unroll
+    for (int a = 0; a < 3; ++a)
+#pragma unroll
+        for (int b = 0; b < 3; ++b)
+#pragma unroll
+            for (int c = 0; c < CO / 2; ++c) acc[a][b][c] = f32x2{0.f, 0.f};
+#pragma unroll
+    for (int c = 0; c < CO; ++c) bsum[c] = 0.f;
+#pragma unroll
+    for (int j = 0; j < 4; ++j) asum[j] = 0.0;
+    const bool want_alpha = alpha_part != nullptr;
+    for (int tile = share; tile < ntiles; tile += nshares) {
+        int n, d0, h0, w0;
+        decode_tile(tile, tilesD, tilesH, tilesW, TW, n, d0, h0, w0);
+        float4 zq[RPW], dq[RPW];
+        bool ok[RPW];
+#pragma unroll
+        for (int i = 0; i < RPW; ++i) {
+            const int row = wave + 12 * i, od = d0 + row / C1H, oh = h0 + row % C1H, ow = w0 + tv;
+            ok[i] = row < NROW && od < g.dout && oh < g.ho && ow < g.wo;
+            zq[i] = dq[i] = make_float4(0.f, 0.f, 0.f, 0.f);
+            if (ok[i]) {
+                const int64_t vox = (((int64_t)n * g.dout + od) * g.ho + oh) * g.wo + ow;
+                zq[i] = ldf4(z + vox * g.y_ld + tq * 4);
+                dq[i] = ldf4(da + vox * da_ld + tq * 4);
+            }
+        }
+        __syncthreads();
+        cin1_stage<float, TW, C1D + 2, 768>(xs, x + (int64_t)n * g.di * g.hi * g.wi * g.x_ld, g, d0 - 1, h0, w0, (int)threadIdx.x);
+#pragma unroll
+        for (int i = 0; i < RPW; ++i) {
+            const int row = wave + 12 * i;
+            if (row < NROW) {
+                const float zv[4] = {zq[i].x, zq[i].y, zq[i].z, zq[i].w}, dv[4] = {dq[i].x, dq[i].y, dq[i].z, dq[i].w};
+                float du[4];
+#pragma unroll
+                for (int j = 0; j < 4; ++j) {
+                    const bool pos = zv[j] > 0.f;
+                    du[j] = ok[i] ? (pos ? dv[j] : dv[j] * al[j]) : 0.f;
+                    if (want_alpha) asum[j] += (pos || !ok[i]) ? 0.0 : (double)dv[j] * (double)zv[j];
+                }
+                *reinterpret_cast<float4*>(dzs + row * RS + toff) = make_float4(du[0], du[1], du[2], du[3]);
+            }
+        }
+        __syncthreads();
+        f32x2 gy[VPT][CO / 2];
+        {
+            const float* gp = dzs + (dl * C1H + hl) * RS + wq * LS;
+#pragma unroll
+            for (int v = 0; v < VPT; ++v)
+#pragma unroll
+                for (int c = 0; c < CO; c += 4) {
+                    const float4 q = *reinterpret_cast<const float4*>(gp + v * CO + c);
+                    gy[v][c / 2] = f32x2{q.x, q.y};
+                    gy[v][c / 2 + 1] = f32x2{q.z, q.w};
+                }
+        }
+#pragma unroll
+        for (int kh = 0; kh < 3; ++kh) {
+            const float* row = xs + ((dl + kd) * (C1H + 2) + hl + kh) * PW + wq * VPT;
+            float r[VPT + 2];
+#pragma unroll
+            for (int i = 0; i < VPT + 2; ++i) r[i] = row[i];
+#pragma unroll
+            for (int kw = 0; kw < 3; ++kw)
+#pragma unroll
+                for (int v = 0; v < VPT; ++v)
+#pragma unroll
+                    for (int c = 0; c < CO / 2; ++c)
+                        acc[kh][kw][c] = __builtin_elementwise_fma(f32x2{r[v + kw], r[v + kw]}, gy[v][c], acc[kh][kw][c]);
+        }
+        if (kd == 1) {
+#pragma unroll
+            for (int v = 0; v < VPT; ++v)
+#pragma unroll
+                for (int c = 0; c < CO / 2; ++c) { bsum[2 * c] += gy[v][c].x; bsum[2 * c + 1] += gy[v][c].y; }
+        }
+    }
+#pragma unroll
+    for (int a = 0; a < 3; ++a)
+#pragma unroll
+        for (int b = 0; b < 3; ++b)
+#pragma unroll
+            for (int c = 0; c < CO; ++c) {
+                const float vsum = wave_sum_dpp((c & 1) ? acc[a][b][c / 2].y : acc[a][b][c / 2].x);
+                if (lane == 0) red[wave][(a * 3 + b) * CO + c] = vsum;
+            }
+#pragma unroll
+    for (int c = 0; c < CO; ++c) {
+        const float vsum = wave_sum_dpp(bsum[c]);
+        if (lane == 0) red[wave][9 * CO + c] = vsum;
+    }
+    if (want_alpha) {
+#pragma unroll
+        for (int j = 0; j < 4; ++j) {
+            double v = asum[j];
+#pragma unroll
+            for (int m = 32; m >= Q; m >>= 1) v += __shfl_xor(v, m, 64);
+            if (lane < Q) ared[wave][lane * 4 + j] = v;
+        }
+    }
+    __syncthreads();
+    const int w0_ = 4 * kd;
+    if (tid < 9 * CO) {
+        const float t4 = (red[w0_][tid] + red[w0_ + 1][tid]) + (red[w0_ + 2][tid] + red[w0_ + 3][tid]);
+        part[((size_t)share * 27 + kd * 9 + tid / CO) * CO + tid % CO] = t4;
+    } else if (tid < NA && kd == 1 && bias_part) {
+        const int c = tid - 9 * CO;
+        bias_part[(size_t)share * CO + c] = (red[w0_][tid] + red[w0_ + 1][tid]) + (red[w0_ + 2][tid] + red[w0_ + 3][tid]);
+    }
+    if (want_alpha && (int)threadIdx.x < CO) {
+        double t = 0.0;
+#pragma unroll
+        for (int wv = 0; wv < 12; ++wv) t += ared[wv][tid];
+        alpha_part[(size_t)share * CO + tid] = t;
+    }
+}
+
+__global__ void __launch_bounds__(256)
+cin1_act_dalpha_kernel(const double* __restrict__ alpha_part, int nshares, int CO, int alpha_n, float* __restrict__ dalpha) {
+    __shared__ double r[256];
+    __shared__ float sums[16];
+    const int L = 256 / CO, c = threadIdx.x / L, ql = threadIdx.x % L;
+    double t = 0.0;
+    for (int q = ql; q < nshares; q += L) t += alpha_part[(size_t)q * CO + c];
+    r[threadIdx.x] = t;
+    __syncthreads();
+    if (ql == 0) {
+        t = 0.0;
+        for (int q = 0; q < L; ++q) t += r[c * L + q];
+        sums[c] = (float)t;
+    }
+    __syncthreads();
+    if (alpha_n > 1) {
+        if ((int)threadIdx.x < CO) dalpha[threadIdx.x] = (float)(double)sums[threadIdx.x];
+    } else if (threadIdx.x == 0) {
+        t = 0.0;
+        for (int q = 0; q < CO; ++q) t += (double)sums[q];
+        dalpha[0] = (float)t;
+    }
+}
+
 template <typename T>
 __global__ void __launch_bounds__(256)
 conv_c1c1_stencil_kernel(Mri3dConvGeom g, const T* __restrict__ x, int x_ld, const float* __restrict__ w, const float* __restrict__ bias,
@@ -1783,4 +2052,80 @@
     return check_launch(what);
 }
 
-}
+bool conv_cin1_act_supported(const Mri3dConvGeom& g, int a_ld, int act, int alpha_n, int pass, int align) {
+    if (pass != MRI3D_PASS_FWD && pass != MRI3D_PASS_WGRAD) return false;
+    if (g.dtype != MRI3D_F32 || !cin1_ok(g)) return false;
+    if (act != MRI3D_ACT_RELU && act != MRI3D_ACT_LEAKY && act != MRI3D_ACT_PRELU) return false;
+    if (act == MRI3D_ACT_PRELU && alpha_n != 1 && alpha_n != g.co) return false;
+    if (a_ld < g.co || a_ld % 4 != 0 || align < 16) return false;
+    return pass == MRI3D_PASS_FWD || g.co == 8;
+}
+
+struct Cin1ActPlan {
+    size_t part_floats, bias_floats, alpha_doubles;
+    size_t ws_bytes;
+};
+
+static Cin1ActPlan cin1_act_plan(const Mri3dConvGeom& g, int pass) {
+    Cin1ActPlan p{0, 0, 0, 0};
+    if (pass == MRI3D_PASS_FWD) {
+        p.ws_bytes = (size_t)27 * g.co * sizeof(float);
+        return p;
+    }
+    p.part_floats = (size_t)kCin1Shares * 27 * g.co, p.bias_floats = (size_t)kCin1Shares * g.co;
+    p.alpha_doubles = (size_t)kCin1Shares * g.co;
+    p.ws_bytes = (p.part_floats + p.bias_floats) * sizeof(float) + p.alpha_doubles * sizeof(double);
+    return p;
+}
+
+size_t conv_cin1_act_workspace_bytes(const Mri3dConvGeom& g, int pass) { return cin1_act_plan(g, pass).ws_bytes; }
+
+bool conv_cin1_act_route_name(const Mri3dConvGeom& g, int a_ld, int act, int alpha_n, int pass, int align, char* name, size_t name_bytes) {
+    const int len = conv_cin1_act_supported(g, a_ld, act, alpha_n, pass, align)
+                        ? snprintf(name, name_bytes, "cin1 act %s co%d", pass == MRI3D_PASS_FWD ? "fwd" : "bwd", g.co)
+                        : snprintf(name, name_bytes, "none");
+    return len > 0 && (size_t)len < name_bytes;
+}
+
+int conv_cin1_act_fwd(const Mri3dConvGeom& g, int a_ld, int act, int alpha_n, float slope, const float* x, const float* w,
+                      const float* bias, const float* alpha, float* z, float* a, void* ws, size_t ws_bytes, hipStream_t s) {
+    MRI3D_REQUIRE(conv_cin1_act_supported(g, a_ld, act, alpha_n, MRI3D_PASS_FWD, ptr_align(z, a, ws)), MRI3D_ENOTSUP,
+                  "conv_cin1_act_fwd: geometry / activation / alignment not served (query mri3d_conv_cin1_act_supported)");
+    const Cin1ActPlan p = cin1_act_plan(g, MRI3D_PASS_FWD);
+    MRI3D_REQUIRE(ws != nullptr && ws_bytes >= p.ws_bytes, MRI3D_EWORKSPACE, "conv_cin1_act_fwd: workspace %zu < %zu", ws_bytes, p.ws_bytes);
+    float* wp = static_cast<float*>(ws);
+    hipLaunchKernelGGL(repack_w_kernel, dim3(1), dim3(256), 0, s, w, wp, g.co, 1, 27, g.co, 0);
+    const C1Tiles t = cin1_tiles(g);
+    const int grid = std::min((int)t.ntiles, 256 * 8);
+    const Cin1Act pa{alpha, alpha_n, act, slope};
+    if (g.co == 8)
+        hipLaunchKernelGGL(conv_cin1_act_fwd_kernel<8>, dim3(grid), dim3(256), 0, s, g, x, wp, bias, pa, z, a, a_ld, t.tilesD, t.tilesH,
+                           t.tilesW, (int)t.ntiles);
+    else
+        hipLaunchKernelGGL(conv_cin1_act_fwd_kernel<16>, dim3(grid), dim3(256), 0, s, g, x, wp, bias, pa, z, a, a_ld, t.tilesD, t.tilesH,
+                           t.tilesW, (int)t.ntiles);
+    return check_launch("conv_cin1_act_fwd");
+}
+
+int conv_cin1_act_bwd(const Mri3dConvGeom& g, int da_ld, int act, int alpha_n, float slope, const float* x, const float* z,
+                      const float* da, const float* alpha, float* dw, float* dbias, float* dalpha, void* ws, size_t ws_bytes,
+                      hipStream_t s) {
+    MRI3D_REQUIRE(conv_cin1_act_supported(g, da_ld, act, alpha_n, MRI3D_PASS_WGRAD, ptr_align(z, da, ws)), MRI3D_ENOTSUP,
+                  "conv_cin1_act_bwd: geometry / activation / alignment not served (query mri3d_conv_cin1_act_supported)");
+    const Cin1ActPlan p = cin1_act_plan(g, MRI3D_PASS_WGRAD);
+    MRI3D_REQUIRE(ws != nullptr && ws_bytes >= p.ws_bytes, MRI3D_EWORKSPACE, "conv_cin1_act_bwd: workspace %zu < %zu", ws_bytes, p.ws_bytes);
+    float* part = static_cast<float*>(ws);
+    float* bias_part = dbias ? part + p.part_floats : nullptr;
+    double* alpha_part = (dalpha && act == MRI3D_ACT_PRELU) ? reinterpret_cast<double*>(part + p.part_floats + p.bias_floats) : nullptr;
+    const C1Tiles t = cin1_tiles(g);
+    const Cin1Act pa{alpha, alpha_n, act, slope};
+    hipLaunchKernelGGL(conv_cin1_act_bwd_kernel<8>, dim3(kCin1Shares), dim3(768), 0, s, g, x, z, da, da_ld, pa, part, bias_part,
+                       alpha_part, t.tilesD, t.tilesH, t.tilesW, (int)t.ntiles, kCin1Shares);
+    hipLaunchKernelGGL(wgrad_reduce_kernel, dim3(cdiv(g.co * 27 + g.co, 8)), dim3(256), 0, s, part, bias_part, dw, dbias, kCin1Shares,
+                       27, 1, g.co, 1, g.co);
+    if (alpha_part)
+        hipLaunchKernelGGL(cin1_act_dalpha_kernel, dim3(1), dim3(256), 0, s, alpha_part, kCin1Shares, g.co, alpha_n, dalpha);
+    return check_launch("conv_cin1_act_bwd");
+}
+
+}
diff --git a/mri_epilepsy_diagnosis_amd/nn.py b/mri_epilepsy_diagnosis_amd/nn.py
--- a/mri_epilepsy_diagnosis_amd/nn.py
+++ b/mri_epilepsy_diagnosis_amd/nn.py
@@ -165,8 +165,23 @@
                        (x,))
 
 
-def conv_norm_act(conv, norm, act, x, out=None, head=None, pool=None):
-    wants = (isinstance(norm, tnn.modules.batchnorm._BatchNorm) and (norm.training or norm.running_mean is None)
+def fused_conv_act(conv, act, x):
+    if not (isinstance(conv, Conv3d) and conv.padding_mode == "zeros" and conv.groups == 1 and not isinstance(conv.padding, str)
+            and tuple(conv.kernel_size) == (3, 3, 3) and tuple(conv.stride) == (1, 1, 1) and tuple(conv.padding) == (1, 1, 1)
+            and tuple(conv.dilation) == (1, 1, 1) and torch.is_tensor(x)):
+        return None
+    kind, alpha, slope = _act_spec(act)
+    if kind is None or not ops.conv3d_act_supported(x, conv.weight, kind, alpha):
+        return None
+    return ops.conv3d_act(x, conv.weight, conv.bias, alpha, kind, slope)
+
+
+def conv_norm_act(conv, norm, act, x, out=None, head=None, pool=None, fused_first=True):
+    if fused_first and norm is None and out is None and head is None and pool is None:
+        a = fused_conv_act(conv, act, x)
+        if a is not None:
+            return a
+    wants =(isinstance(norm, tnn.modules.batchnorm._BatchNorm) and (norm.training or norm.running_mean is None)
              and ops.sync_batchnorm_reducer() is None and isinstance(conv, Conv3d) and conv.padding_mode == "zeros"
              and conv.groups == 1 and not isinstance(conv.padding, str))
     if isinstance(x, (tuple, list)):
diff --git a/mri_epilepsy_diagnosis_amd/ops.py b/mri_epilepsy_diagnosis_amd/ops.py
--- a/mri_epilepsy_diagnosis_amd/ops.py
+++ b/mri_epilepsy_diagnosis_amd/ops.py
@@ -679,6 +679,116 @@
 
 def conv3d(x, weight, bias=None, stride=1, padding=0, dilation=1, bn_stats=False):
     return _apply_with_bn_stats(_Conv3dFn, bn_stats, _autocast_in(x), weight, bias, _triple(stride), _triple(padding), _triple(dilation))
+
+
+
+
+def conv_cin1_act_route(g, a_ld, act_code, alpha_n, pass_, align=16):
+    name = ctypes.create_string_buffer(64)
+    check(_lib.lib().mri3d_conv_cin1_act_route(ctypes.byref(g), a_ld, act_code, alpha_n, pass_, align, name, 64), "conv_cin1_act_route")
+    return name.value.decode()
+
+
+def _cin1_act_alpha_n(act_code, alpha):
+    return 1 if act_code != ACT_PRELU else (alpha.numel() if alpha is not None else 0)
+
+
+def conv3d_act_supported(x, weight, act, alpha=None, out=None):
+    if not (torch.is_tensor(x) and x.dim() == 5 and x.dtype == torch.float32 and not x.requires_grad):
+        return False
+    if _autocast_dtype is not None or act not in ("relu", "leaky_relu", "prelu"):
+        return False
+    if weight.dim() != 5 or tuple(weight.shape[2:]) != (3, 3, 3) or weight.shape[1] != x.shape[1] or weight.dtype != torch.float32:
+        return False
+    if act == "prelu" and (alpha is None or alpha.dtype != torch.float32):
+        return False
+    x_ld = _pitch_of(x)
+    g = _conv_geom(x.shape, weight.shape, _ONE, _ONE, _ONE, x_ld=x.shape[1] if x_ld is None else x_ld)
+    act_code = _ACT_CODES[act]
+    z_ld = a_ld = g.co
+    if out is not None:
+        z_ld, a_ld = _pitch_of(out[0]), _pitch_of(out[1])
+        if z_ld is None or a_ld is None:
+            return False
+        g.y_ld = z_ld
+    align = 16 if out is None else _ptr_align(*out)
+    return bool(_lib.lib().mri3d_conv_cin1_act_supported(ctypes.byref(g), a_ld, act_code, _cin1_act_alpha_n(act_code, alpha), PASS_FWD, align))
+
+
+def _cin1_act_tag(kind, g):
+    return "conv3d_act_%s 1->%d @%dx%dx%d n%d" % (kind, g.co, g.dout, g.ho, g.wo, g.n)
+
+
+class _Conv3dActFn(torch.autograd.Function):
+
+    @staticmethod
+    def forward(ctx, x, weight, bias, alpha, act, slope, out):
+        _require_device(x)
+        _require_param(weight, bias, alpha)
+        L = _lib.lib()
+        x, x_ld = _nd(x)
+        w = weight.contiguous()
+        g = _conv_geom(x.shape, w.shape, _ONE, _ONE, _ONE, x_ld=x_ld)
+        shape = (g.n, g.co, g.dout, g.ho, g.wo)
+        z, a = (_new(shape, x), _new(shape, x)) if out is None else out
+        if tuple(z.shape) != shape or tuple(a.shape) != shape or z.dtype != x.dtype or a.dtype != x.dtype:
+            raise RuntimeError("conv3d_act(out=): two float32 tensors of shape %s expected" % (shape,))
+        g.y_ld, a_ld = _pitch_of(z), _pitch_of(a)
+        if g.y_ld is None or a_ld is None:
+            raise RuntimeError("conv3d_act(out=): the output tensors must be NDHWC in memory")
+        act_code = _ACT_CODES[act]
+        prelu = act_code == ACT_PRELU
+        alpha_n = _cin1_act_alpha_n(act_code, alpha)
+        _launch(L.mri3d_conv_cin1_act_fwd, lambda: _cin1_act_tag("fwd", g),
+                lambda: {"flops": _conv_work(g, "fwd")["flops"], "bytes": 4.0 * (x.numel() + 2 * z.numel())},
+                L.mri3d_conv_cin1_act_workspace_bytes(ctypes.byref(g), PASS_FWD), x.device,
+                g, a_ld, act_code, alpha_n, float(slope), x, w, bias, alpha if prelu else None, z, a)
+        ctx.save_for_backward(x, w, z, alpha if prelu else None)
+        ctx.geom, ctx.act, ctx.slope = g, (act_code, alpha_n), float(slope)
+        ctx.params, ctx.has_bias = (weight, bias, alpha if prelu else None), bias is not None
+        return a
+
+    @staticmethod
+    def backward(ctx, da):
+        L = _lib.lib()
+        x, w, z, alpha = ctx.saved_tensors
+        g0 = ctx.geom
+        act_code, alpha_n = ctx.act
+        if da.dtype != z.dtype:
+            raise RuntimeError("conv3d_act backward: gradient dtype %s does not match activation dtype %s" % (da.dtype, z.dtype))
+        if ctx.needs_input_grad[0]:
+            raise RuntimeError("conv3d_act: no data gradient (ops.conv3d_act_supported declines an input that requires one)")
+        weight, bias, alpha_p = ctx.params
+        if not any(p is not None and ctx.needs_input_grad[1 + i] for i, p in enumerate(ctx.params)):
+            return None, None, None, None, None, None, None
+        da, da_ld = _nd(da)
+        csinks, cgrads = _grad_slots(ctx, (w, bias), 1, (weight, bias), all_written=True)
+        asinks, agrads = _grad_slots(ctx, (alpha,), 3, (alpha_p,))
+        dw, db = cgrads
+        dalpha = agrads[0]
+        g = _repitched(g0, g0.x_ld, g0.y_ld)
+        if L.mri3d_conv_cin1_act_supported(ctypes.byref(g), da_ld, act_code, alpha_n, PASS_WGRAD, _ptr_align(z, da)):
+            _launch(L.mri3d_conv_cin1_act_bwd, lambda: _cin1_act_tag("bwd", g),
+                    lambda: {"flops": _conv_work(g, "wgrad")["flops"], "bytes": 4.0 * (x.numel() + 2 * z.numel())},
+                    L.mri3d_conv_cin1_act_workspace_bytes(ctypes.byref(g), PASS_WGRAD), x.device,
+                    g, da_ld, act_code, alpha_n, ctx.slope, x, z, da, alpha, dw, db, dalpha)
+        else:
+            zd = z if g0.y_ld == g0.co else z.contiguous(memory_format=CL3D)
+            dz = _new(zd.shape, zd)
+            ng = NormGeom(g0.n, g0.dout * g0.ho * g0.wo, g0.co, g0.co, da_ld, 0, act_code, alpha_n, ctx.slope, 0.0, 0, F32)
+            ws = _workspace(L.mri3d_norm_workspace_bytes(ctypes.byref(ng)), x.device)
+            with _timed(lambda: "norm_act_bwd c%d vox%d n%d" % (ng.c, ng.vox, ng.n), lambda: {"flops": 0.0, "bytes": 20.0 * zd.numel()}):
+                check(L.mri3d_norm_act_bwd(ctypes.byref(ng), 0, _ptr(zd), _ptr(da), None, None, None, None, _ptr(alpha), _ptr(dz), None,
+                                           None, _ptr(dalpha), _ptr(ws), ws.numel(), _stream()), "norm_act_bwd")
+            _conv_wgrad(_repitched(g0, g0.x_ld, g0.co), x, dz, w, db is not None, dw, db)
+        return (None, *_grad_slots_done(ctx, cgrads, csinks, 1, (weight, bias)), *_grad_slots_done(ctx, agrads, asinks, 3, (alpha_p,)),
+                None, None, None)
+
+
+def conv3d_act(x, weight, bias=None, alpha=None, act="prelu", slope=0.01, out=None):
+    if not conv3d_act_supported(x, weight, act, alpha, out):
+        raise RuntimeError("conv3d_act: not served for this input, kernel or activation (ask conv3d_act_supported)")
+    return _Conv3dActFn.apply(x, weight, bias, alpha, act, slope, out)
 
 
 
diff --git a/mri_epilepsy_diagnosis_amd/unet/unet.py b/mri_epilepsy_diagnosis_amd/unet/unet.py
--- a/mri_epilepsy_diagnosis_amd/unet/unet.py
+++ b/mri_epilepsy_diagnosis_amd/unet/unet.py
@@ -32,8 +32,8 @@
         self.dropout_layer = None
         self.block = tnn.Sequential(*[m for m in (conv, norm, act) if m is not None])
 
-    def forward(self, x, out=None, head=None, pool=None):
-        return mnn.conv_norm_act(self.conv_layer, self.norm_layer, self.activation_layer, x, out, head, pool)
+    def forward(self, x, out=None, head=None, pool=None, fused_first=True):
+        return mnn.conv_norm_act(self.conv_layer, self.norm_layer, self.activation_layer, x, out, head, pool, fused_first)
 
 
 class EncodingBlock(tnn.Module):
@@ -55,12 +55,12 @@
                 raise NotImplementedError("only max pooling is used by the reference")
             self.downsample = mnn.MaxPool3d(kernel_size=2)
 
-    def forward(self, x, skip_out=None, head=None, fused_pool=True):
+    def forward(self, x, skip_out=None, head=None, fused_pool=True, fused_first=True):
         if self.downsample is None:
-            return self.conv2(self.conv1(x), skip_out, head)
+            return self.conv2(self.conv1(x, fused_first=fused_first), skip_out, head)
         if fused_pool and skip_out is None and isinstance(self.downsample, mnn.MaxPool3d):
-            return self.conv2(self.conv1(x), pool=self.downsample)
-        x = self.conv2(self.conv1(x), skip_out)
+            return self.conv2(self.conv1(x, fused_first=fused_first), pool=self.downsample)
+        x = self.conv2(self.conv1(x, fused_first=fused_first), skip_out)
         return self.downsample.forward_with_skip(x)
 
     @property
@@ -85,10 +85,10 @@
             if self.dilation is not None:
                 self.dilation *= 2
 
-    def forward(self, x, cat_bufs=None, fused_pool=True):
+    def forward(self, x, cat_bufs=None, fused_pool=True, fused_first=True):
         skips = []
         for i, blk in enumerate(self.encoding_blocks):
-            x, skip = blk(x, None if cat_bufs is None else (cat_bufs[i], 0), fused_pool=fused_pool)
+            x, skip = blk(x, None if cat_bufs is None else (cat_bufs[i], 0), fused_pool=fused_pool, fused_first=fused_first)
             skips.append(skip)
         return skips, x
 
@@ -173,6 +173,7 @@
         self.shared_concat_buffers = False
         self.fused_head = True
         self.fused_pool = True
+        self.fused_first = True
         self.classifier = ConvolutionalBlock(dimensions, 2 * out_channels_first_layer, out_classes, kernel_size=1,
                                              activation=None)
 
@@ -193,9 +194,9 @@
         mc = mc if (mc is not None and mc.training and mc.p > 0) else None
         head = clf.conv_layer if (self.fused_head and mc is None and x.is_cuda and clf.norm_layer is None
                                   and clf.activation_layer is None and clf.dropout_layer is None) else None
-        skips, enc = self.encoder(x, cat_bufs, self.fused_pool)
+        skips, enc = self.encoder(x, cat_bufs, self.fused_pool, self.fused_first)
         if not skips:
-            x = self.bottom_block(enc, head=head)
+            x = self.bottom_block(enc, head=head, fused_first=self.fused_first)
         else:
             x = self.decoder(skips, self.bottom_block(enc), cat_bufs, head)
         if head is not None:
```

Result: faster. 69.99 volumes/s (median of 6 runs) (+1.3%).
